# jac0626/Neighbor-Aware-Reinforcement-Learning-Fosters-Cooperation-in-Spatial-Public-Goods-Games-

Measured on AMD Instinct MI355X. Metric: agent-steps/sec (L×L×iters×replicas) + achieved HBM GB/s, L=200, higher is better.
Workload: dtype f64

## Files before the change

include/spgg_abi.h:

```cpp
#ifndef SPGG_ABI_H
#define SPGG_ABI_H

#include <stdint.h>

#ifdef __cplusplus
extern "C" {
#endif

#define SPGG_ABI_VERSION 17

#define SPGG_OK 0
#define SPGG_E_ARG (-1)
#define SPGG_E_STATE (-2)
#define SPGG_E_HIP (-3)

#define SPGG_GEN_ERR_SPIN 1u
#define SPGG_STEP_ERR_BARRIER 2u

#define SPGG_CLUSTERS_MAX_PASSES 32

#define SPGG_STATE_REPUTATION 0
#define SPGG_STATE_ACTION 1

#define SPGG_ALG_QLEARNING 0
#define SPGG_ALG_SARSA 1
#define SPGG_ALG_EXPECTED_SARSA 2
#define SPGG_ALG_DOUBLE_Q 3

#define SPGG_RNG_INJECT 0
#define SPGG_RNG_MT19937 1
#define SPGG_RNG_PHILOX 2

enum {
  SPGG_ST_NCOOP = 0,
  SPGG_ST_SUMP = 1,
  SPGG_ST_SUMP_C = 2,
  SPGG_ST_SUMP_D = 3,
  SPGG_ST_SUMR = 4,
  SPGG_ST_SW_CD = 5,
  SPGG_ST_SW_DC = 6,
  SPGG_ST_SUM_WPP = 7,
  SPGG_ST_SUM_WRR = 8,
  SPGG_ST_SUM_REW_C = 9,
  SPGG_ST_SUM_REW_D = 10,
  SPGG_ST_SUM_RATIO_C = 11,
  SPGG_ST_GC0 = 12,
  SPGG_ST_NMD_POS = 18,
  SPGG_ST_NMD_POS2 = 19,
  SPGG_ST_SUM_PCT = 20,
  SPGG_ST_SUMQ = 21,
  SPGG_ST_SUMQ_C = 25,
  SPGG_ST_SUMQ_D = 29,
  SPGG_ST_GMAX = 33,
  SPGG_NSTAT = 34
};

typedef struct spgg_ctx spgg_ctx;

typedef struct {
  int32_t device;
  int32_t n_rep;
  int32_t L;
  int32_t second_order;
  int32_t state_mode;
  int32_t rng_mode;
  int32_t iterations;
  int32_t rep_int8;
  int32_t algorithm;
  int32_t batch_reps;
} spgg_config;

typedef struct {
  double rc;
  double cost;
  double norm_min;
  double norm_den;
  double w_p;
  double w_rep;
  double alpha;
  double gamma;
  double diag_alpha;
  double diag_gamma;
  double kappa;
  double lambda_eps;
  double rep_gain_c;
  double neg_delta_r_d;
  double r_min;
  double r_max;
  uint64_t seed;
  uint64_t stream_id;
  double pay_c[6];
  double pay_d[6];
  double rep_unit;
  int32_t rk_gain, rk_loss, rk_min, rk_max;
  double norm_rcp;
} spgg_rep_params;

typedef struct {
  uint8_t* S[2];
  void* R[2];
  double* Q;
  double* pub[2];
  double* md;
  float* atd;
  uint32_t* draws;
  int64_t draw_slot_stride;
  uint32_t* mt_state;
  uint32_t* mt_snap;
  int64_t mt_snap_stride;
  double* eps;
  double* stats;
  int32_t* stop_iter;
} spgg_buffers;

int spgg_abi_version(void);
const char* spgg_build_id(void);
int spgg_draw_planes(int32_t algorithm);
const char* spgg_last_error(const spgg_ctx* ctx);

int spgg_create(spgg_ctx** out, const spgg_config* cfg);
int spgg_set_params(spgg_ctx* ctx, const spgg_rep_params* params);
int spgg_bind(spgg_ctx* ctx, const spgg_buffers* bufs);

int spgg_step(spgg_ctx* ctx, int32_t t0, int32_t n_steps, void* hip_stream);

int spgg_step_groups(spgg_ctx* const* ctxs, void* const* hip_streams, int32_t n_ctx, int32_t t0,
                     int32_t n_steps);

int spgg_flush(spgg_ctx* ctx, int32_t t_last, void* hip_stream);

int spgg_status(const spgg_ctx* ctx, uint32_t* flags);

int spgg_history_finalize(spgg_ctx* ctx, int32_t t_last, void* hip_stream);

int spgg_draw(spgg_ctx* ctx, int32_t t, void* hip_stream);
int spgg_draw_range(spgg_ctx* ctx, int32_t t0, int32_t t1, void* hip_stream);

int spgg_draw_layout(const spgg_ctx* ctx, int32_t* slots, int64_t* words_per_rep, int32_t* snap_slots);

int spgg_mt_chains(const spgg_ctx* ctx, int32_t* chains, int32_t* per_chain);

int spgg_mt_jump_poly(int64_t e, uint32_t* out624);

int spgg_stream_create(int32_t device, void** hip_stream);
int spgg_stream_destroy(void* hip_stream);

int spgg_set_draw_stream(spgg_ctx* ctx, void* hip_stream);

int spgg_payoff(spgg_ctx* ctx, int32_t t, double* out, void* hip_stream);

int spgg_clusters_max_side(const spgg_ctx* ctx, int32_t* side);
int spgg_clusters(spgg_ctx* ctx, int32_t t, int32_t periodic, int32_t* sizes, int32_t* rec,
                  int64_t rec_stride, void* hip_stream);

int spgg_pub_doubles(const spgg_ctx* ctx, int64_t* per_rep);

int spgg_stat_stripes(const spgg_ctx* ctx, int32_t* stripes);

int spgg_persistent(const spgg_ctx* ctx, int32_t* on, int32_t* capacity);

int spgg_tile_shape(const spgg_ctx* ctx, int32_t* tw, int32_t* th);

int spgg_destroy(spgg_ctx* ctx);

#ifdef __cplusplus
}
#endif
#endif
```

neighbor-aware-reinforcement-learning-fosters-cooperation-in-spatial-public-goods-games-_amd/_lib.py:

```python
from __future__ import annotations

import ctypes
import os
import threading

PKG_DIR = os.path.dirname(os.path.abspath(__file__))
LIB_PATH = os.path.join(PKG_DIR, "libspgg_hip.so")

ABI_VERSION = 17
OK, E_ARG, E_STATE, E_HIP = 0, -1, -2, -3
GEN_ERR_SPIN = 1
CLUSTERS_MAX_PASSES = 32
STATE_REPUTATION, STATE_ACTION = 0, 1
RNG_INJECT, RNG_MT19937, RNG_PHILOX = 0, 1, 2
RNG_MODES = {"inject": RNG_INJECT, "mt19937": RNG_MT19937, "philox": RNG_PHILOX}
ALG_QLEARNING, ALG_SARSA, ALG_EXPECTED_SARSA, ALG_DOUBLE_Q = 0, 1, 2, 3
ALGORITHMS = {"qlearning": ALG_QLEARNING, "sarsa": ALG_SARSA, "expected_sarsa": ALG_EXPECTED_SARSA,
              "double_qlearning": ALG_DOUBLE_Q}
DRAW_PLANES = {ALG_QLEARNING: 2, ALG_SARSA: 6, ALG_EXPECTED_SARSA: 2, ALG_DOUBLE_Q: 3}

ST_NCOOP, ST_SUMP, ST_SUMP_C, ST_SUMP_D, ST_SUMR = 0, 1, 2, 3, 4
ST_SW_CD, ST_SW_DC, ST_SUM_WPP, ST_SUM_WRR = 5, 6, 7, 8
ST_SUM_REW_C, ST_SUM_REW_D, ST_SUM_RATIO_C = 9, 10, 11
ST_GC0, ST_NMD_POS, ST_NMD_POS2, ST_SUM_PCT = 12, 18, 19, 20
ST_SUMQ, ST_SUMQ_C, ST_SUMQ_D, ST_GMAX = 21, 25, 29, 33
NSTAT = 34

EXPORTED = ("spgg_abi_version", "spgg_build_id", "spgg_last_error", "spgg_create", "spgg_set_params",
            "spgg_bind", "spgg_step", "spgg_step_groups", "spgg_flush", "spgg_draw", "spgg_payoff", "spgg_tile_shape",
            "spgg_destroy", "spgg_draw_planes", "spgg_pub_doubles", "spgg_stat_stripes",
            "spgg_history_finalize", "spgg_draw_layout", "spgg_set_draw_stream", "spgg_draw_range",
            "spgg_mt_chains", "spgg_mt_jump_poly", "spgg_stream_create", "spgg_stream_destroy",
            "spgg_status", "spgg_persistent", "spgg_clusters", "spgg_clusters_max_side")
TEST_EXPORTED = ("spgg_test_set_error",)


class Config(ctypes.Structure):
    _fields_ = [("device", ctypes.c_int32), ("n_rep", ctypes.c_int32), ("L", ctypes.c_int32),
                ("second_order", ctypes.c_int32), ("state_mode", ctypes.c_int32),
                ("rng_mode", ctypes.c_int32), ("iterations", ctypes.c_int32),
                ("rep_int8", ctypes.c_int32), ("algorithm", ctypes.c_int32),
                ("batch_reps", ctypes.c_int32)]


class RepParams(ctypes.Structure):
    _fields_ = [(name, ctypes.c_double) for name in (
        "rc", "cost", "norm_min", "norm_den", "w_p", "w_rep", "alpha", "gamma",
        "diag_alpha", "diag_gamma", "kappa", "lambda_eps", "rep_gain_c", "neg_delta_r_d",
        "r_min", "r_max")] + [("seed", ctypes.c_uint64), ("stream_id", ctypes.c_uint64),
                              ("pay_c", ctypes.c_double * 6), ("pay_d", ctypes.c_double * 6),
                              ("rep_unit", ctypes.c_double), ("rk_gain", ctypes.c_int32),
                              ("rk_loss", ctypes.c_int32), ("rk_min", ctypes.c_int32),
                              ("rk_max", ctypes.c_int32), ("norm_rcp", ctypes.c_double)]


class Buffers(ctypes.Structure):
    _fields_ = [("S", ctypes.c_void_p * 2), ("R", ctypes.c_void_p * 2), ("Q", ctypes.c_void_p),
                ("pub", ctypes.c_void_p * 2), ("md", ctypes.c_void_p), ("atd", ctypes.c_void_p),
                ("draws", ctypes.c_void_p), ("draw_slot_stride", ctypes.c_int64),
                ("mt_state", ctypes.c_void_p), ("mt_snap", ctypes.c_void_p), ("mt_snap_stride", ctypes.c_int64),
                ("eps", ctypes.c_void_p),
                ("stats", ctypes.c_void_p), ("stop_iter", ctypes.c_void_p)]


class SpggError(RuntimeError):
    pass


_libs = {}
_lock = threading.Lock()


def load(path: str | None = None):
    with _lock:
        p = path or os.environ.get("SPGG_LIB") or LIB_PATH
        if p in _libs:
            return _libs[p]
        if not os.path.exists(p):
            raise SpggError(f"{p} is not built; run `python -c 'import __graft_entry__ as g; g.build()'`")
        lib = ctypes.CDLL(p)
        vp, i32 = ctypes.c_void_p, ctypes.c_int32
        lib.spgg_abi_version.restype = ctypes.c_int
        lib.spgg_abi_version.argtypes = []
        lib.spgg_last_error.restype = ctypes.c_char_p
        lib.spgg_last_error.argtypes = [vp]
        lib.spgg_create.restype = ctypes.c_int
        lib.spgg_create.argtypes = [ctypes.POINTER(vp), ctypes.POINTER(Config)]
        lib.spgg_set_params.restype = ctypes.c_int
        lib.spgg_set_params.argtypes = [vp, ctypes.POINTER(RepParams)]
        lib.spgg_bind.restype = ctypes.c_int
        lib.spgg_bind.argtypes = [vp, ctypes.POINTER(Buffers)]
        lib.spgg_step.restype = ctypes.c_int
        lib.spgg_step.argtypes = [vp, i32, i32, vp]
        lib.spgg_step_groups.restype = ctypes.c_int
        lib.spgg_step_groups.argtypes = [ctypes.POINTER(vp), ctypes.POINTER(vp), i32, i32, i32]
        lib.spgg_flush.restype = ctypes.c_int
        lib.spgg_flush.argtypes = [vp, i32, vp]
        lib.spgg_history_finalize.restype = ctypes.c_int
        lib.spgg_history_finalize.argtypes = [vp, i32, vp]
        lib.spgg_draw.restype = ctypes.c_int
        lib.spgg_draw.argtypes = [vp, i32, vp]
        lib.spgg_draw_range.restype = ctypes.c_int
        lib.spgg_draw_range.argtypes = [vp, i32, i32, vp]
        lib.spgg_payoff.restype = ctypes.c_int
        lib.spgg_payoff.argtypes = [vp, i32, vp, vp]
        lib.spgg_tile_shape.restype = ctypes.c_int
        lib.spgg_tile_shape.argtypes = [vp, ctypes.POINTER(i32), ctypes.POINTER(i32)]
        lib.spgg_clusters.restype = ctypes.c_int
        lib.spgg_clusters.argtypes = [vp, i32, i32, vp, vp, ctypes.c_int64, vp]
        lib.spgg_clusters_max_side.restype = ctypes.c_int
        lib.spgg_clusters_max_side.argtypes = [vp, ctypes.POINTER(i32)]
        lib.spgg_persistent.restype = ctypes.c_int
        lib.spgg_persistent.argtypes = [vp, ctypes.POINTER(i32), ctypes.POINTER(i32)]
        lib.spgg_destroy.restype = ctypes.c_int
        lib.spgg_destroy.argtypes = [vp]
        lib.spgg_draw_planes.restype = ctypes.c_int
        lib.spgg_draw_planes.argtypes = [i32]
        lib.spgg_stat_stripes.restype = ctypes.c_int
        lib.spgg_stat_stripes.argtypes = [vp, ctypes.POINTER(ctypes.c_int32)]
        lib.spgg_pub_doubles.restype = ctypes.c_int
        lib.spgg_pub_doubles.argtypes = [vp, ctypes.POINTER(ctypes.c_int64)]
        lib.spgg_draw_layout.restype = ctypes.c_int
        lib.spgg_draw_layout.argtypes = [vp, ctypes.POINTER(i32), ctypes.POINTER(ctypes.c_int64), ctypes.POINTER(i32)]
        lib.spgg_mt_chains.restype = ctypes.c_int
        lib.spgg_mt_chains.argtypes = [vp, ctypes.POINTER(i32), ctypes.POINTER(i32)]
        lib.spgg_mt_jump_poly.restype = ctypes.c_int
        lib.spgg_mt_jump_poly.argtypes = [ctypes.c_int64, vp]
        lib.spgg_stream_create.restype = ctypes.c_int
        lib.spgg_stream_create.argtypes = [i32, ctypes.POINTER(vp)]
        lib.spgg_stream_destroy.restype = ctypes.c_int
        lib.spgg_stream_destroy.argtypes = [vp]
        lib.spgg_set_draw_stream.restype = ctypes.c_int
        lib.spgg_set_draw_stream.argtypes = [vp, vp]
        lib.spgg_status.restype = ctypes.c_int
        lib.spgg_status.argtypes = [vp, ctypes.POINTER(ctypes.c_uint32)]
        lib.spgg_test_set_error.restype = ctypes.c_int
        lib.spgg_test_set_error.argtypes = [vp, ctypes.c_uint32]
        lib.spgg_build_id.restype = ctypes.c_char_p
        lib.spgg_build_id.argtypes = []
        v = lib.spgg_abi_version()
        if v != ABI_VERSION:
            raise SpggError(f"libspgg_hip ABI {v} != expected {ABI_VERSION}")
        if p == LIB_PATH:
            from . import build as B
            if os.path.exists(B.SRC[0]):
                want, have = B.build_id(), lib.spgg_build_id().decode()
                if want != have:
                    raise SpggError(f"{p} was built from other sources (build id {have}, sources {want}); "
                                    "rebuild: python -c 'import __graft_entry__ as g; g.build()'")
        _libs[p] = lib
        return lib


def check(rc: int, ctx=None, what: str = "", lib=None):
    if rc != OK:
        lib = lib or load()
        detail = (lib.spgg_last_error(ctx) or b"").decode()
        raise SpggError(f"{what} failed (rc={rc}): {detail}")
```

neighbor-aware-reinforcement-learning-fosters-cooperation-in-spatial-public-goods-games-_amd/csrc/spgg_kernels.hip:

```cpp
#include <hip/hip_runtime.h>

#include <algorithm>
#include <numeric>
#include <type_traits>
#include <cstdio>
#include <cstdlib>
#include <cstring>
#include <new>
#include <string>
#include <thread>
#include <vector>

#include "spgg_abi.h"
#include "spgg_test.h"
#include "spgg_device.h"
#include "spgg_mt.h"
#include "spgg_clusters.h"

using namespace spgg;

#ifndef SPGG_ABLATE
#define SPGG_ABLATE 0
#endif
#ifndef SPGG_PRIO
#define SPGG_PRIO 0
#endif
#ifndef SPGG_QNT
#define SPGG_QNT 0
#endif
#ifndef SPGG_QSTORE
#define SPGG_QSTORE 0
#endif

#ifndef SPGG_TU
#define SPGG_TU (-1)
#endif
#define SPGG_TU_HAS_ALG(k) (SPGG_TU == -1 || SPGG_TU == (k))
#define SPGG_TU_HAS_HOST (SPGG_TU == -1 || SPGG_TU == 9)

namespace spgg_impl {

struct TileArgs {
  const uint8_t* S_in;
  uint8_t* S_out;
  const void* R_in;
  void* R_out;
  double* Q;
  double* md;
  const double* pub_in;
  double* pub_out;
  float* atd;
  const uint32_t* draws;
  int draw_words;
  int planes;
  const double* eps;
  double* stats;
  int* stop_iter;
  const spgg_rep_params* params;
  const int2* ring;
  int L, n, TW, TH, tiles_x, tiles_per_rep, n_rep, slots;
  int PB;
  int ring_max;
  int stripes;
  int rep_stride;
};

struct LaunchCfg {
  int m2, as, rq, rng, twc, total_tiles;
  int apt;
  size_t lds_bytes;
};

struct PersistArgs {
  uint8_t* S[2];
  void* R[2];
  double* pub[2];
  const uint32_t* draws0;
  long long draw_stride;
  int draw_slots;
  int t_end;
  uint32_t* bar;
  int shards;
  uint32_t base;
  uint32_t* err;
  uint32_t* err_host;
};
constexpr int kBarWords = 16;

template <int ALG>
void launch_alg(const LaunchCfg& lc, const TileArgs& a, int t, int fin, hipStream_t s,
                const PersistArgs* pa = nullptr);
template <int ALG>
int persist_blocks_per_cu(const LaunchCfg& lc);

constexpr int apt_of(int alg) { return (alg == SPGG_ALG_DOUBLE_Q ? 512 : 1024) / kBlock; }
constexpr int js_of(bool m2) { return kBlock == 256 ? (m2 ? 8 : 7) : 4; }
constexpr int jr_of() { return kBlock == 256 ? 6 : 3; }
constexpr int ring_per_thread(bool m2) { return kBlock == 256 && m2 ? 2 : 1; }
constexpr int qw_of(int alg) { return alg == SPGG_ALG_DOUBLE_Q ? 8 : 4; }
constexpr int pf_of(int alg) { return alg == SPGG_ALG_DOUBLE_Q ? 5 : 3; }

__host__ __device__ inline int pub_slots(int TW, int TH, int HA) {
  return 2 * HA * TW + (TH > 2 * HA ? (TH - 2 * HA) * 2 * HA : 0);
}
__host__ __device__ inline bool is_border(int r, int c, int th, int tw, int HA) {
  return r < HA || r >= th - HA || c < HA || c >= tw - HA;
}
__host__ __device__ inline int border_slot(int r, int c, int th, int tw, int HA) {
  if (r < HA) return r * tw + c;
  if (r >= th - HA) return (r - th + 2 * HA) * tw + c;
  const int cc = c < HA ? c : c - tw + 2 * HA;
  return 2 * HA * tw + (r - HA) * 2 * HA + cc;
}
__host__ __device__ inline int border_slot_or_none(int r, int c, int th, int tw, int HA) {
  const bool top = r < HA, bot = r >= th - HA;
  const bool left = c < HA, right = c >= tw - HA;
  const int band = (top ? r : r - th + 2 * HA) * tw + c;
  const int side = 2 * HA * tw + (r - HA) * 2 * HA + (left ? c : c - tw + 2 * HA);
  return (top || bot) ? band : ((left || right) ? side : -1);
}

__host__ __device__ inline void ring_cell(int k, int th, int tw, int HA, int* ay, int* ax) {
  const int aw = tw + 2 * HA, band = HA * aw;
  if (k < band) {
    *ay = k / aw;
    *ax = k - *ay * aw;
  } else if (k < 2 * band) {
    const int k2 = k - band;
    *ay = HA + th + k2 / aw;
    *ax = k2 - (k2 / aw) * aw;
  } else {
    const int k3 = k - 2 * band;
    *ay = HA + k3 / (2 * HA);
    const int cc = k3 - (k3 / (2 * HA)) * (2 * HA);
    *ax = cc < HA ? cc : tw + cc;
  }
}

}

using spgg_impl::TileArgs;

namespace {


struct LdsLayout {
  int sw, sh, aw, ah;
  int off_Rew, off_R, off_Rn, off_S, off_D, off_A, off_PC, off_DR, off_DP, bytes;
};

constexpr int kDrawSlots = 6;

constexpr int kPcPitch = 64;

__host__ __device__ inline LdsLayout lds_layout(int tw, int th, int HS, int HA, int rsz, bool dword_rows = false,
                                                bool draws = false) {
  LdsLayout l;
  l.sw = tw + 2 * HS; l.sh = th + 2 * HS;
  l.aw = tw + 2 * HA; l.ah = th + 2 * HA;
  if (dword_rows) l.sw = l.aw = (tw + 2 * HS + 3 + 3) / 4 * 4;
  const int na = l.aw * l.ah;
  int off = (12 + kWaves * 64) * 8;
  l.off_Rew = off;  off += ((na * 8 + 15) / 16) * 16;
  l.off_R = off;    off += ((na * rsz + 15) / 16) * 16;
  l.off_Rn = off;   off += ((na * rsz + 15) / 16) * 16;
  l.off_S = off;    off += ((l.sw * l.sh + 15) / 16) * 16;
  l.off_D = off;    off += ((l.sw * l.sh + kPcPitch + 15) / 16) * 16;
  l.off_A = off;    off += ((na + 15) / 16) * 16;
  l.off_PC = off;   off += (l.ah + 2) * kPcPitch;
  off = (off + 15) / 16 * 16;
  l.off_DR = off;   off += draws ? l.ah * kDrawSlots * 2 * 4 : 0;
  l.off_DP = off;   off += draws ? l.ah * 2 * 2 * 4 : 0;
  l.bytes = off;
  return l;
}

template <typename T>
__device__ __forceinline__ T* at(T* base, uint32_t i) {
  using B = typename std::conditional<std::is_const<T>::value, const char, char>::type;
  return reinterpret_cast<T*>(reinterpret_cast<B*>(base) + (size_t)(i * (uint32_t)sizeof(T)));
}

#ifndef SPGG_PERSIST_PLAIN
#define SPGG_PERSIST_PLAIN 0
#endif
#ifndef SPGG_PERSIST_STAGGER
#define SPGG_PERSIST_STAGGER 0
#endif
#ifndef SPGG_PERSIST_NORECOMP
#define SPGG_PERSIST_NORECOMP 0
#endif
template <bool SC1, typename T>
__device__ __forceinline__ T hload(const T* p) {
  if constexpr (SC1 && !SPGG_PERSIST_PLAIN) return __hip_atomic_load(const_cast<T*>(p), __ATOMIC_RELAXED, __HIP_MEMORY_SCOPE_AGENT);
  else return *p;
}
template <bool SC1, typename T>
__device__ __forceinline__ void hstore(T* p, T v) {
  if constexpr (SC1 && !SPGG_PERSIST_PLAIN) __hip_atomic_store(p, v, __ATOMIC_RELAXED, __HIP_MEMORY_SCOPE_AGENT);
  else *p = v;
}

template <bool RQ>
using RStore = typename std::conditional<RQ, int8_t, double>::type;
template <bool RQ>
using RVal = typename std::conditional<RQ, int, double>::type;

template <bool RQ, typename PT>
__device__ __forceinline__ RVal<RQ> rep_next(RVal<RQ> r, int act, const PT& p) {
  if constexpr (RQ) {
    const int k = r + (act == 0 ? p.rk_gain : -p.rk_loss);
    return min(max(k, p.rk_min), p.rk_max);
  } else {
    const double x = r + (act == 0 ? p.rep_gain_c : p.neg_delta_r_d);
    return fmin(fmax(x, p.r_min), p.r_max);
  }
}

template <bool M2>
__device__ __forceinline__ int rep_state_lds(const int8_t* R, int c, int w) {
  int acc = R[c] + R[c - w] + R[c + w] + R[c - 1] + R[c + 1];
  if constexpr (M2)
    acc += R[c - 2 * w] + R[c + 2 * w] + R[c - 2] + R[c + 2] + R[c - w - 1] + R[c - w + 1] + R[c + w - 1] +
           R[c + w + 1];
  return acc > 0 ? 1 : 0;
}

template <bool M2>
__device__ __forceinline__ int rep_state_lds(const double* R, int c, int w) {
  double acc = 0.0;
  acc += R[c];
  acc += R[c - w];
  acc += R[c + w];
  acc += R[c - 1];
  acc += R[c + 1];
  if constexpr (M2) {
    acc += R[c - 2 * w];
    acc += R[c + 2 * w];
    acc += R[c - 2];
    acc += R[c + 2];
    acc += R[c - w - 1];
    acc += R[c - w + 1];
    acc += R[c + w - 1];
    acc += R[c + w + 1];
  }
  return acc >= rep_threshold(M2) ? 1 : 0;
}

__device__ __forceinline__ double pending_nu(uint8_t b, double md, double kappa, double lam_den, double lam_rcp) {
  const double lam = div_uniform(kappa * md, lam_den, lam_rcp);
  return ((b >> 2) & 1) ? lam : -lam;
}

__device__ __forceinline__ int pending_entry(uint8_t b) { return ((b >> 1) & 1) * 2 + (b & 1); }

template <int K, typename T>
__device__ __forceinline__ void wave_partials(T (&v)[K], double* red, int base, int tid) {
  transpose_level<K, 32, K, T>(v, tid & 63);
  const int lane = tid & 63, wave = tid >> 6;
  constexpr int per = 64 / K;
  if ((lane & (per - 1)) == 0) red[wave * 64 + base + lane / per] = (double)v[0];
}

__device__ __forceinline__ int wrap1(int x, int L, bool tiny) {
  if (tiny) return wrap(x, L);
  x += x < 0 ? L : 0;
  x -= x >= L ? L : 0;
  return x;
}

template <typename T>
using StageReg = typename std::conditional<(sizeof(T) < 4), int, T>::type;

template <int J, typename T>
__device__ __forceinline__ void stage_region(T* dst, int pitch, const T* src, int h, int w, int y0, int x0,
                                             int L, bool tiny, uint8_t* dbit = nullptr) {
  const int total = h * w;
  const int tid = threadIdx.x;
  const int dr = kBlock / w, dc = kBlock - (kBlock / w) * w;
  int r = tid / w, c = tid - (tid / w) * w;
  StageReg<T> buf[J];
  int di[J];
#pragma unroll
  for (int j = 0; j < J; ++j) {
// ... 149 lines not shown
#define T_AT(t, o) (*reinterpret_cast<const double*>((t) + (o)))
__device__ __forceinline__ double payoff_pc(const uint8_t* pc, int ry, int rx, const double* tb, double norm_min,
                                            double norm_den, double norm_rcp) {
  const uint8_t* p = pc + ry * kPcPitch + rx + 1;
  const char* t = reinterpret_cast<const char*>(tb);
  const uint32_t x0 = p[kPcPitch], x1 = p[0], x2 = p[2 * kPcPitch], x3 = p[kPcPitch - 1], x4 = p[kPcPitch + 1];
  double tot = T_AT(t, x0);
  tot = tot + T_AT(t, x1);
  tot = tot + T_AT(t, x2);
  tot = tot + T_AT(t, x3);
  tot = tot + T_AT(t, x4);
  return div_uniform(tot - norm_min, norm_den, norm_rcp);
}

#undef T_AT

__device__ __forceinline__ double rcp_diag(double x) {
  double r = __builtin_amdgcn_rcp(x);
  r = __builtin_fma(r, __builtin_fma(-x, r, 1.0), r);
  r = __builtin_fma(r, __builtin_fma(-x, r, 1.0), r);
  return r;
}

constexpr uint64_t stat_bytes(int a, int b, int c, int d, int e, int f, int g, int h) {
  return (uint64_t)(uint8_t)a | (uint64_t)(uint8_t)b << 8 | (uint64_t)(uint8_t)c << 16 | (uint64_t)(uint8_t)d << 24 |
         (uint64_t)(uint8_t)e << 32 | (uint64_t)(uint8_t)f << 40 | (uint64_t)(uint8_t)g << 48 |
         (uint64_t)(uint8_t)h << 56;
}


enum { ALG_Q = SPGG_ALG_QLEARNING, ALG_SARSA = SPGG_ALG_SARSA, ALG_ES = SPGG_ALG_EXPECTED_SARSA,
       ALG_DQ = SPGG_ALG_DOUBLE_Q };

__device__ __forceinline__ int greedy2(double v0, double v1) { return v0 >= v1 ? 0 : 1; }

__device__ __forceinline__ double mean2(double x, double y) { return (x + y) * 0.5; }

__device__ __forceinline__ double expected_q(double v0, double v1, double eps) {
  const double po = eps * 0.5;
  const double pgr = (1.0 - eps) + po;
  const int g = greedy2(v0, v1);
  return (g == 0 ? pgr : po) * v0 + (g == 1 ? pgr : po) * v1;
}

__device__ __forceinline__ int draw_bit(const TileArgs& a, int rep, int g, int p) {
  const uint32_t w = *at(a.draws, (uint32_t)(rep * a.draw_words + (g >> 5) * a.planes + p));
  return (int)((w >> (g & 31)) & 1u);
}

template <int RNG>
__device__ __forceinline__ void draw_pair(const TileArgs& a, int rep, int g, int t, uint32_t key, uint64_t thr,
                                          int k, int* ex, int* rbt) {
  if constexpr (RNG == SPGG_RNG_PHILOX) {
#if SPGG_ABLATE & 1
    *ex = ((g * 2654435761u + t + k) >> 7) % 50 == 0; *rbt = (g ^ t ^ k) & 1;
#else
    philox_draw(g, t + (k << 26), key, thr, ex, rbt);
#endif
  } else {
    *ex = draw_bit(a, rep, g, 2 * k);
    *rbt = draw_bit(a, rep, g, 2 * k + 1);
  }
}

__device__ __forceinline__ void staged_draw(const uint2* sDP, int ry, int rx, int* ex, int* rbt) {
  const uint2 w = sDP[ry * 2 + (rx >> 5)];
  *ex = (int)((w.x >> (rx & 31)) & 1u);
  *rbt = (int)((w.y >> (rx & 31)) & 1u);
}

template <int RNG>
__device__ __forceinline__ int draw_table1(const TileArgs& a, int rep, int g, int t, uint32_t key) {
  if constexpr (RNG == SPGG_RNG_PHILOX) {
    int ex, rbt;
    philox_draw(g, t + (1 << 26), key, 1ull << 52, &ex, &rbt);
    return ex;
  } else {
    return draw_bit(a, rep, g, 2);
  }
}

typedef double vd2 __attribute__((ext_vector_type(2)));

template <int QB>
__device__ __forceinline__ void load_q(const double* Qr, uint32_t n, uint32_t agent, double (&q)[4],
                                       double (&qb)[QB ? 4 : 1]) {
  const vd2* q0 = at(reinterpret_cast<const vd2*>(Qr), agent * (QB ? 2 : 1));
  const vd2* q1 = at(reinterpret_cast<const vd2*>(Qr), (n + agent) * (QB ? 2 : 1));
#if SPGG_QNT & 1
  const vd2 q01 = __builtin_nontemporal_load(q0), q23 = __builtin_nontemporal_load(q1);
#else
  const vd2 q01 = q0[0], q23 = (SPGG_ABLATE & 4096) ? q01 : q1[0];
#endif
  q[0] = q01.x; q[1] = q01.y; q[2] = q23.x; q[3] = q23.y;
  if constexpr (QB) {
    const vd2 b01 = q0[1], b23 = q1[1];
    qb[0] = b01.x; qb[1] = b01.y; qb[2] = b23.x; qb[3] = b23.y;
  }
}

template <int QB>
__device__ __forceinline__ void store_q(double* Qr, uint32_t n, uint32_t agent, const double (&q)[4],
                                        const double (&qb)[QB ? 4 : 1], uint32_t rows = 3u) {
  vd2* q0 = at(reinterpret_cast<vd2*>(Qr), agent * (QB ? 2 : 1));
  vd2* q1 = at(reinterpret_cast<vd2*>(Qr), (n + agent) * (QB ? 2 : 1));
#if SPGG_QNT & 2
  if constexpr (!QB) {
    if (rows & 1u) __builtin_nontemporal_store(vd2{q[0], q[1]}, q0);
    if (rows & 2u) __builtin_nontemporal_store(vd2{q[2], q[3]}, q1);
    return;
  }
#endif
  if (rows & 1u) {
    q0[0] = vd2{q[0], q[1]};
    if constexpr (QB) q0[1] = vd2{qb[0], qb[1]};
  }
  if (rows & 2u) {
    q1[0] = vd2{q[2], q[3]};
    if constexpr (QB) q1[1] = vd2{qb[2], qb[3]};
  }
}

template <int QB>
__device__ __forceinline__ void select_row(const double (&q)[4], const double (&qb)[QB ? 4 : 1], int s,
                                           double* v0, double* v1) {
  if constexpr (QB) {
    const double m00 = mean2(q[0], qb[0]), m01 = mean2(q[1], qb[1]);
    const double m10 = mean2(q[2], qb[2]), m11 = mean2(q[3], qb[3]);
    *v0 = s ? m10 : m00;
    *v1 = s ? m11 : m01;
  } else {
    uint32_t a0, a1, b0, b1;
    asm("v_cmp_ne_u32_e32 vcc, 0, %4\n\t"
        "v_cndmask_b32_e32 %0, %5, %6, vcc\n\t"
        "v_cndmask_b32_e32 %1, %7, %8, vcc\n\t"
        "v_cndmask_b32_e32 %2, %9, %10, vcc\n\t"
        "v_cndmask_b32_e32 %3, %11, %12, vcc"
        : "=&v"(a0), "=&v"(a1), "=&v"(b0), "=&v"(b1)
        : "v"(s), "v"(__double2loint(q[0])), "v"(__double2loint(q[2])), "v"(__double2hiint(q[0])),
          "v"(__double2hiint(q[2])), "v"(__double2loint(q[1])), "v"(__double2loint(q[3])),
          "v"(__double2hiint(q[1])), "v"(__double2hiint(q[3]))
        : "vcc");
    *v0 = __hiloint2double((int)a1, (int)a0);
    *v1 = __hiloint2double((int)b1, (int)b0);
  }
}

template <typename PT>
__device__ __forceinline__ float diag_td_dq(const double (&q)[4], const double (&qb)[4], int e, int sn, double rew,
                                            const PT& pg) {
  const double m00 = mean2(q[0], qb[0]), m01 = mean2(q[1], qb[1]);
  const double m10 = mean2(q[2], qb[2]), m11 = mean2(q[3], qb[3]);
  const double m0 = sn ? m10 : m00, m1 = sn ? m11 : m01;
  const double td2 = (rew + pg.diag_gamma * max_f64(m0, m1)) - mean2(q_get(q, e), q_get(qb, e));
  return (float)fabs(pg.diag_alpha * td2);
}

template <int ALG, int RNG, typename PT>
__device__ __forceinline__ float td_update(const TileArgs& a, const PT& pg, int rep, int g, int t,
                                           uint32_t key, double eps, uint64_t eps53, bool diag, double rew,
                                           int so, int act, int sn, double (&q)[4],
                                           double (&qb)[ALG == ALG_DQ ? 4 : 1], double* rn0, double* rn1) {
  const double alpha = pg.alpha, gamma = pg.gamma, dgamma = pg.diag_gamma;
  const int e = so * 2 + act;
  if constexpr (ALG == ALG_DQ) {
    double x[4] = {q[0], q[1], q[2], q[3]}, y[4] = {qb[0], qb[1], qb[2], qb[3]};
    const int up1 = draw_table1<RNG>(a, rep, g, t, key);
    const double qc1 = q_get(x, e), qc2 = q_get(y, e);
    const double y0 = y[0], y1 = y[1], y2 = y[2], y3 = y[3];
// ... 98 lines not shown
  return v;
}

#ifndef SPGG_BAR_DEBUG
#define SPGG_BAR_DEBUG 0
#endif
constexpr uint32_t kBarrierPolls = 1u << 21;

__device__ __forceinline__ bool replica_barrier(const spgg_impl::PersistArgs& pa, int rep, int tile,
                                                int tiles_per_rep, uint32_t k,
                                                unsigned long long* arrive_stamp = nullptr) {
  __shared__ int bar_ok;
  asm volatile("s_waitcnt vmcnt(0)" ::: "memory");
  __syncthreads();
  if (arrive_stamp && threadIdx.x == 0) *arrive_stamp = __builtin_amdgcn_s_memrealtime();
  if (threadIdx.x < 64) {
    const int lane = threadIdx.x, S = pa.shards;
    uint32_t* ctr = pa.bar + (size_t)rep * S * spgg_impl::kBarWords;
    if (lane == 0)
      __hip_atomic_fetch_add(ctr + (tile % S) * spgg_impl::kBarWords, 1u, __ATOMIC_RELAXED,
                             __HIP_MEMORY_SCOPE_AGENT);
    const int j = lane < S ? lane : 0;
    const uint32_t want = (uint32_t)((tiles_per_rep - j + S - 1) / S) * (pa.base + k);
    bool ok = false;
    for (uint32_t poll = 0; poll < kBarrierPolls; ++poll) {
      const uint32_t have = __hip_atomic_load(ctr + j * spgg_impl::kBarWords, __ATOMIC_RELAXED,
                                              __HIP_MEMORY_SCOPE_AGENT);
      const uint32_t err = __hip_atomic_load(pa.err, __ATOMIC_RELAXED, __HIP_MEMORY_SCOPE_AGENT);
      if (__builtin_amdgcn_readfirstlane(err) != 0) break;
      if (__all((int32_t)(have - want) >= 0)) {
        ok = true;
        break;
      }
      __builtin_amdgcn_s_sleep(2);
    }
    if (!ok && lane == 0) {
      atomicOr(pa.err, (uint32_t)SPGG_STEP_ERR_BARRIER);
      __hip_atomic_fetch_or(pa.err_host, (uint32_t)SPGG_STEP_ERR_BARRIER, __ATOMIC_RELAXED, __HIP_MEMORY_SCOPE_SYSTEM);
    }
#if SPGG_BAR_DEBUG
    if (!ok) {
      const uint32_t have = __hip_atomic_load(ctr + j * spgg_impl::kBarWords, __ATOMIC_RELAXED, __HIP_MEMORY_SCOPE_AGENT);
      if ((int32_t)(have - want) < 0)
        printf("spgg barrier: rep %d tile %d k %u shard %d have %u want %u base %u\n", rep, tile, k, j, have, want,
               pa.base);
    }
#endif
    if (lane == 0) bar_ok = ok ? 1 : 0;
  }
  __syncthreads();
  return bar_ok != 0;
}

#ifndef SPGG_STAMPS
#define SPGG_STAMPS 0
#endif
#if SPGG_STAMPS
#ifndef SPGG_STAMP_T
#define SPGG_STAMP_T 30
#endif
constexpr int kStampWG = 8192, kStampSlots = 12;
__device__ unsigned long long spgg_stamps[kStampWG * kStampSlots];
#define STAMP(k)                                                                            \
  do {                                                                                      \
    if (t == SPGG_STAMP_T && tid == 0 && stamp_id < kStampWG)                               \
      spgg_stamps[stamp_id * kStampSlots + (k)] = __builtin_amdgcn_s_memrealtime();         \
  } while (0)
#else
#define STAMP(k) \
  do {           \
  } while (0)
#endif
constexpr int min_waves(bool m2, int rng, int twc, int alg) {
#ifdef SPGG_MIN_WAVES
  return SPGG_MIN_WAVES;
#else
#ifdef SPGG_MT_MIN_WAVES
  if (!m2 && rng == SPGG_RNG_MT19937 && twc > 0 && alg != SPGG_ALG_DOUBLE_Q) return SPGG_MT_MIN_WAVES;
#endif
  return (!m2 && rng == SPGG_RNG_PHILOX && twc > 0 && alg != SPGG_ALG_DOUBLE_Q) ? 4 : 1;
#endif
}

template <bool M2, bool AS, bool RQ, int RNG, int APT, int TWC, int ALG, bool PERSIST>
__device__ __forceinline__ void step_impl(const TileArgs& a0, const int t0, const int fin_only,
                                          const spgg_impl::PersistArgs& pa) {
  static_assert(!PERSIST || TWC > 0, "persistent launches use the compile-time-width kernels");
  using RT = RStore<RQ>;
  constexpr int HA = M2 ? 2 : 1;
  constexpr int HS = HA + 2;
  constexpr int QB = ALG == ALG_DQ ? 1 : 0;
  constexpr int QW = QB ? 8 : 4;
  constexpr int PF = spgg_impl::pf_of(ALG);
  constexpr bool RECOMP = ALG != ALG_SARSA && APT == spgg_impl::apt_of(ALG) && !(PERSIST && SPGG_PERSIST_NORECOMP);
  constexpr bool CARRY = PERSIST && !SPGG_PERSIST_NORECOMP;
  extern __shared__ __attribute__((aligned(16))) unsigned char smem[];

  const int total = a0.n_rep * a0.tiles_per_rep;
  const int per_xcd = (total + 7) / 8;
  const int logical = (blockIdx.x & 7) * per_xcd + (blockIdx.x >> 3);
  if (logical >= total) return;
  if (SPGG_ABLATE & 64) return;
  const int lrep = logical / a0.tiles_per_rep;
  const int tile = logical - lrep * a0.tiles_per_rep;
  const int rep = a0.rep_stride > 1 ? (int)(((uint32_t)lrep * (uint32_t)a0.rep_stride) % (uint32_t)a0.n_rep) : lrep;
#if SPGG_STAMPS
  const int stamp_id = (int)a0.params[rep].stream_id * a0.tiles_per_rep + tile;
#endif

  const int L = a0.L, n = a0.n;
  const bool tiny = TWC ? false : L < 8;
  const int tyi = tile / a0.tiles_x, txi = tile - (tile / a0.tiles_x) * a0.tiles_x;
  const int y0 = tyi * a0.TH, x0 = txi * a0.TW;
  const int th = min(a0.TH, L - y0), tw = TWC ? TWC : min(a0.TW, L - x0);
  constexpr bool DSTAGE = RNG != SPGG_RNG_PHILOX && TWC > 0;
  const LdsLayout ly = TWC ? lds_layout(TWC, a0.TH, HS, HA, (int)sizeof(RT), true, DSTAGE)
                           : lds_layout(tw, th, HS, HA, (int)sizeof(RT));
  double* tab = reinterpret_cast<double*>(smem);
  double* red = tab + 12;
  double* sRew = reinterpret_cast<double*>(smem + ly.off_Rew);
  RT* sR = reinterpret_cast<RT*>(smem + ly.off_R);
  RT* sRn = reinterpret_cast<RT*>(smem + ly.off_Rn);
  uint8_t* sS = smem + ly.off_S;
  uint8_t* sD = smem + ly.off_D;
  uint8_t* sA = smem + ly.off_A;
  uint8_t* sPC = smem + ly.off_PC;
  uint8_t* sPP = smem + ly.bytes;
  uint32_t* sDR = reinterpret_cast<uint32_t*>(smem + ly.off_DR);
  uint2* sDP = reinterpret_cast<uint2*>(smem + ly.off_DP);
  const size_t rb = (size_t)rep * n;
  double* Qr = a0.Q + rb * QW;
  double* mdr = a0.md + rb;
  float* atdr = a0.atd + rb;
  const int aw = tw + 2 * HA, ah = th + 2 * HA;

  int rc[APT];
  unsigned vbits = 0;
  double q[APT][4];
  double qb[APT][QB ? 4 : 1];
  double md_own[APT];
  float atd_own[APT];
  const int n_own = th * tw;
  const uint32_t g00 = (uint32_t)(y0 * L + x0);
  auto agent_of = [&](int rcu) { return g00 + __umul24((uint32_t)(rcu >> 16), (uint32_t)L) + ((rcu >> 8) & 0xff); };
  bool stored = false;
  int t = t0;
  for (;; ++t) {
  TileArgs a = a0;
  if constexpr (PERSIST) {
    const int cur = (t - 1) & 1, nxt = t & 1;
    a.S_in = pa.S[cur];
    a.S_out = pa.S[nxt];
    a.R_in = pa.R[cur];
    a.R_out = pa.R[nxt];
    a.pub_in = pa.pub[cur];
    a.pub_out = pa.pub[nxt];
    if (pa.draws0) a.draws = pa.draws0 + (size_t)((t - 1) % pa.draw_slots) * pa.draw_stride;
  }
  const bool first = !PERSIST || t == t0;
  int tid = threadIdx.x;
  if constexpr (PERSIST) asm volatile("" : "+v"(tid));
  const uint8_t* Sin = a.S_in + rb;
  uint8_t* Sout = a.S_out + rb;
  const RT* Rin = reinterpret_cast<const RT*>(a.R_in) + rb;
  RT* Rout = reinterpret_cast<RT*>(a.R_out) + rb;
  const bool pending = t > 1;
  STAMP(0);
#if SPGG_PRIO
  if constexpr (!PERSIST) __builtin_amdgcn_s_setprio(SPGG_PRIO);
#endif
#if SPGG_STAMPS
  if (t == SPGG_STAMP_T && tid == 0 && stamp_id < kStampWG) {
    unsigned hw, xcc;
    asm volatile("s_getreg_b32 %0, hwreg(HW_REG_HW_ID)" : "=s"(hw));
    asm volatile("s_getreg_b32 %0, hwreg(HW_REG_XCC_ID)" : "=s"(xcc));
    spgg_stamps[stamp_id * kStampSlots + 8] = hw;
    spgg_stamps[stamp_id * kStampSlots + 9] = xcc;
  }
#endif

  if (!first) {
#pragma unroll
    for (int u = 0; u < APT; ++u) rc[u] &= ~0xff;
  } else {
    const int dr = kBlock / tw, dc = kBlock - (kBlock / tw) * tw;
    int r = tid / tw, c = tid - (tid / tw) * tw;
#pragma unroll
    for (int u = 0; u < APT; ++u) {
      const int k = tid + u * kBlock;
      const bool own = k < n_own;
      rc[u] = own ? (r << 16) | (c << 8) : (TWC ? (tid & 1) << 8 : 0);
      vbits |= own ? 1u << u : 0u;
      const uint32_t g = own ? g00 + __umul24((uint32_t)r, (uint32_t)L) + (uint32_t)c : g00 + (TWC ? (tid & 1) : 0);
      if (SPGG_ABLATE & 512) {
#pragma unroll
        for (int k = 0; k < 4; ++k) q[u][k] = (double)((g + k) & 15) * 1e-3;
        if constexpr (QB) for (int k = 0; k < 4; ++k) qb[u][QB ? k : 0] = q[u][k];
        md_own[u] = 0.0;
        atd_own[u] = 0.f;
      } else {
        load_q<QB>(Qr, (uint32_t)n, g, q[u], qb[u]);
      }
      r += dr;
      c += dc;
      if (c >= tw) {
        c -= tw;
        ++r;
      }
    }
  }
  constexpr int RP = spgg_impl::ring_per_thread(M2);
  const int ring = aw * ah - n_own;
  int2 re[RP];
  {
    const int2* rtab = a.ring + (size_t)tile * a.ring_max;
#pragma unroll
    for (int j = 0; j < RP; ++j) re[j] = *at(rtab, (uint32_t)min(tid + j * kBlock, ring - 1));
  }
  constexpr int JRR = (25 + 2 * HA + kWaves - 1) / kWaves;
  constexpr int JSF = spgg_impl::js_of(M2), JRF = spgg_impl::jr_of();
  constexpr int DWS = (TWC + 2 * HS + 3 + 3) / 4, DWR = (TWC + 2 * HA + 3 + 3) / 4;
  constexpr int JSD = (25 + 2 * HS + kBlock / DWS - 1) / (kBlock / DWS);
  constexpr int JRD = (25 + 2 * HA + kBlock / DWR - 1) / (kBlock / DWR);
  const int soffS = TWC ? ((x0 - HS) & 3) : 0, soffR = TWC && RQ ? ((x0 - HA) & 3) : 0;
  uint8_t* sSv = sS + soffS;
  uint8_t* sDv = sD + soffS;
  RT* sRv = sR + soffR;
  DwordWindow<JSD, DWS> winS;
  DwordWindow<JRD, DWR> winRd;
  RowWindow<JRR, TWC + 2 * HA, RT> winR;
  if constexpr (TWC > 0) {
    winS.template load<PERSIST>(Sin, th + 2 * HS, y0 - HS, (x0 - HS) & ~3, L, tid);
    if constexpr (!AS) {
      if constexpr (RQ) winRd.template load<PERSIST>(Rin, ah, y0 - HA, (x0 - HA) & ~3, L, tid);
      else winR.template load<PERSIST>(Rin, ah, y0 - HA, x0 - HA, L, tid);
    }
  }

  if (!(SPGG_ABLATE & 512) && !RECOMP && (first || !CARRY)) {
    const bool ni_rec = __builtin_amdgcn_readfirstlane((int)(a.params[rep].kappa != 0.0)) != 0;
#pragma unroll
    for (int u = 0; u < APT; ++u) {
      const uint32_t g = ni_rec ? agent_of(rc[u]) : 0u;
      md_own[u] = (SPGG_ABLATE & 8192) ? 0.0 : *at(mdr, g);
      atd_own[u] = (SPGG_ABLATE & 256) ? 0.f : *at(atdr, g);
    }
  }
  const uint32_t xA = wrap_once(x0 - HA, L);
  const int a_len = min(aw, L - (int)xA);
  uint32_t dw0 = 0, dw1 = 0;
  if constexpr (DSTAGE) {
    const int i = min(tid, ah * kDrawSlots - 1), ry = i / kDrawSlots, sl = i - ry * kDrawSlots;
    const uint32_t gy = wrap_once(y0 - HA + ry, L);
    const uint32_t grp = min((gy * (uint32_t)L + (sl < 3 ? xA : 0u)) / 32u + (uint32_t)(sl % 3),
                             (uint32_t)(a.draw_words / a.planes - 1));
    const uint32_t wi = (uint32_t)rep * a.draw_words + grp * a.planes;
    dw0 = *at(a.draws, wi);
    dw1 = *at(a.draws, wi + 1);
  }
  const int st = first ? a.stop_iter[rep] : 0;
  const bool dead = st != 0 && st < t;
  const spgg_rep_params& pg = a.params[rep];
  __shared__ spgg_rep_params hps;
  static_assert(sizeof(spgg_rep_params) % 8 == 0, "spgg_rep_params: whole 8-byte words");
  constexpr int kParamWords = (int)(sizeof(spgg_rep_params) / 8);
  constexpr int kPayWord = (int)(offsetof(spgg_rep_params, pay_c) / 8);
  const uint64_t pword = *at(reinterpret_cast<const uint64_t*>(&pg),
                             (uint32_t)(tid < kParamWords ? tid
                                        : tid < kParamWords + 6 ? kPayWord + 5 - (tid - kParamWords)
                                        : kPayWord + 17 - min(tid - kParamWords, 11)));
  const spgg_rep_params& hp = hps;
  const double kappa = pg.kappa, w_p = pg.w_p, w_rep = pg.w_rep;
  const size_t stripe_len = (size_t)a.slots * SPGG_NSTAT;
  const double* rrow = a.stats + (size_t)rep * a.stripes * stripe_len;
  double* srow = a.stats + ((size_t)rep * a.stripes + tile % a.stripes) * stripe_len;
  bool stop_now = false;
  double gmax_prev = 0.0;
  if constexpr (PERSIST) {
    const int lane = tid & 63, k = lane < a.stripes ? lane : 0;
    const double ncv = hload<true>(rrow + k * stripe_len + (size_t)t * SPGG_NSTAT + SPGG_ST_NCOOP);
    const double gmv = pending ? hload<true>(rrow + k * stripe_len + (size_t)(t - 1) * SPGG_NSTAT + SPGG_ST_GMAX) : 0.0;
    const double nc = uniform_f64(wave_sum(lane < a.stripes ? ncv : 0.0));
    stop_now = (nc == 0.0) || (nc == (double)n);
    gmax_prev = uniform_f64(max_f64(wave_max(gmv), 0.0));
  } else {
    if (!fin_only) {
      double nc = 0.0;
      for (int k = 0; k < a.stripes; ++k) nc += rrow[k * stripe_len + (size_t)t * SPGG_NSTAT + SPGG_ST_NCOOP];
      stop_now = (nc == 0.0) || (nc == (double)n);
    }
    if (pending)
      for (int k = 0; k < a.stripes; ++k)
        gmax_prev = fmax(gmax_prev, rrow[k * stripe_len + (size_t)(t - 1) * SPGG_NSTAT + SPGG_ST_GMAX]);
  }
  const bool acting = !fin_only && !stop_now;
  const double lam_den = uniform_f64(pending ? gmax_prev + pg.lambda_eps : 1.0);
  const double lam_rcp = uniform_f64(1.0 / lam_den);
  const double eps_t = a.eps[(size_t)rep * a.slots + t];
  const double eps_prev = ALG == ALG_ES && pending ? a.eps[(size_t)rep * a.slots + t - 1] : 0.0;
  const uint64_t eps53 = uniform_u64(u53_threshold(eps_t));
  const uint32_t pkey = (uint32_t)pg.seed ^ (uint32_t)(pg.seed >> 32) * 0x85EBCA6Bu ^
                        (uint32_t)pg.stream_id * 0xC2B2AE35u;

  if (tid < kParamWords) reinterpret_cast<uint64_t*>(&hps)[tid] = pword;
  else if (tid < kParamWords + 12) reinterpret_cast<uint64_t*>(tab)[tid - kParamWords] = pword;
  if constexpr (TWC > 0) {
    winS.store(sS, ly.sw, th + 2 * HS, sD, tid);
    if constexpr (!AS) {
      if constexpr (RQ) winRd.store(reinterpret_cast<uint8_t*>(sR), ly.aw, ah, nullptr, tid);
      else winR.template store<(TWC + 2 * HS + 6) / 4 * 4>(sR, ah, nullptr, tid);
    }
  } else {
    stage_region<JSF>(sS, ly.sw, Sin, th + 2 * HS, tw + 2 * HS, y0 - HS, x0 - HS, L, tiny, sD);
    if (!AS) stage_region<JRF>(sR, ly.aw, Rin, ah, aw, y0 - HA, x0 - HA, L, tiny);
  }
  if constexpr (DSTAGE) {
    if (tid < ah * kDrawSlots) {
      sDR[tid * 2] = dw0;
      sDR[tid * 2 + 1] = dw1;
    }
  }
  if (dead) return;
  if (stop_now && tile == 0 && tid == 0) a.stop_iter[rep] = t;
  double rv[RP][PF];
  {
    const double* pin = a.pub_in + (size_t)rep * a.tiles_per_rep * PF * a.PB;
#pragma unroll
    for (int j = 0; j < RP; ++j)
#pragma unroll
      for (int f = 0; f < PF; ++f) rv[j][f] = hload<PERSIST>(at(pin, (uint32_t)(re[j].y + f * a.PB)));
  }
  __syncthreads();
  STAMP(1);
#if SPGG_PRIO
  if constexpr (!PERSIST) __builtin_amdgcn_s_setprio(0);
#endif
  if (SPGG_ABLATE & 128) {
#pragma unroll
    for (int u = 0; u < APT; ++u) {
      const int r = rc[u] >> 16, c = (rc[u] >> 8) & 0xff;
      store_q<QB>(Qr, (uint32_t)n, agent_of(rc[u]), q[u], qb[u]);
      if (!RECOMP) {
        *at(mdr, agent_of(rc[u])) = md_own[u];
        *at(atdr, agent_of(rc[u])) = atd_own[u];
      }
      *at(Sout, agent_of(rc[u])) = sSv[(r + HS) * ly.sw + (c + HS)];
      if (!AS) *at(Rout, agent_of(rc[u])) = sRv[(r + HA) * ly.aw + (c + HA)];
    }
    return;
  }
  if (!fin_only) {
    if constexpr (TWC > 0) build_plus_counts_dw<(TWC + 2 * HA + 2 + 3) / 4>(sPC, sD, ly.sw, ah + 2, soffS, tid);
    else build_plus_counts(sPC, sDv, ly.sw, ah + 2, tid);
  }
  const bool rec_prev = RECOMP && pending && kappa != 0.0;
  if (rec_prev) {
    if constexpr (TWC > 0) build_plus_counts_prev_dw<(TWC + 2 * HA + 2 + 3) / 4>(sPP, sS, ly.sw, ah + 2, soffS, tid);
    else build_plus_counts_prev(sPP, sSv, ly.sw, ah + 2, tid);
    __syncthreads();
    const int dr = kBlock / aw, dc = kBlock - (kBlock / aw) * aw;
    int ry = tid / aw, rx = tid - (tid / aw) * aw;
    for (int k = tid; k < aw * ah; k += kBlock) {
      const uint8_t b = sSv[(ry + (HS - HA)) * ly.sw + (rx + (HS - HA))];
      const double P = payoff_pc(sPP, ry, rx, tab + (((b >> 3) & 1) ? 6 : 0), hp.norm_min, hp.norm_den, hp.norm_rcp);
      const double rr = (b & 1) ? 0.0 : 0.5;
      const double wpp = w_p * P, wrr = w_rep * rr;
      sRew[ry * ly.aw + rx] = wpp + wrr;
      ry += dr;
      rx += dc;
      if (rx >= aw) {
        rx -= aw;
        ++ry;
      }
    }
    __syncthreads();
  }
  if constexpr (DSTAGE) {
    if (!fin_only && tid < ah * 2) {
      const int ry = tid >> 1, r0 = (tid & 1) * 32;
      const uint32_t gyL = wrap_once(y0 - HA + ry, L) * (uint32_t)L;
      const int offA = (int)((gyL + xA) & 31u), offB = (int)(gyL & 31u);
      const uint32_t* W = sDR + ry * kDrawSlots * 2;
      auto bits32 = [&](int slot0, int bitpos, int p) {
        const int w = bitpos >> 5;
        const uint32_t lo = W[(slot0 + min(w, 2)) * 2 + p], hi = W[(slot0 + min(w + 1, 2)) * 2 + p];
        return __builtin_amdgcn_alignbit(hi, lo, (uint32_t)(bitpos & 31));
      };
      uint32_t out[2] = {0u, 0u};
#pragma unroll
      for (int p = 0; p < 2; ++p) {
        if (r0 < a_len) out[p] = bits32(0, offA + r0, p);
        if (a_len < r0 + 32) {
          const int rs = max(r0, a_len), sh = rs - r0;
          const uint32_t mB = ~0u << sh;
          out[p] = (out[p] & ~mB) | ((bits32(3, offB + rs - a_len, p) << sh) & mB);
        }
      }
      sDP[ry * 2 + (r0 >> 5)] = make_uint2(out[0], out[1]);
    }
  }

  float pct_t1 = 0.f;
  uint32_t ni_rows = 0;
  {
    double v[8];
    float pct = 0.f;
#pragma unroll
    for (int k = 0; k < 8; ++k) v[k] = 0.0;
    uint8_t sb[APT];
#pragma unroll
    for (int u = 0; u < APT; ++u) {
      const int r = rc[u] >> 16, c = (rc[u] >> 8) & 0xff;
      sb[u] = sSv[(r + HS) * ly.sw + (c + HS)];
      rc[u] |= (AS ? 0 : ((sb[u] >> 4) & 1) << 1) | ((sb[u] & 1) << 3);
    }
    if (pending) {
#pragma unroll
      for (int u = 0; u < APT; ++u) {
        const double vmu = (vbits >> u) & 1 ? 1.0 : 0.0;
        const uint8_t b = sb[u];
        const int e = pending_entry(b);
        if (kappa != 0.0) {
          double mdp;
          float atdv;
          if constexpr (RECOMP) {
            const int r = rc[u] >> 16, c = (rc[u] >> 8) & 0xff;
            const int ca = (r + HA) * ly.aw + (c + HA);
            mdp = prev_max_diff<M2>(sRew, ca, ly.aw);
            atdv = prev_diag_td<ALG>(q[u], qb[u], e, (b >> 4) & 1, sRew[ca], hp, eps_prev);
          } else {
            mdp = md_own[u];
            atdv = atd_own[u];
          }
          const double nu = pending_nu(b, mdp, kappa, lam_den, lam_rcp);
#pragma unroll
          for (int k = 0; k < 4; ++k) {
            const double m = e == k ? 1.0 : 0.0;
            q[u][k] = __builtin_fma(m, nu, q[u][k]);
            if constexpr (QB) qb[u][k] = __builtin_fma(m, nu, qb[u][QB ? k : 0]);
          }
          ni_rows |= (1u << (e >> 1)) << (2 * u);
          const float anu = fabsf((float)nu);
          pct = (SPGG_ABLATE & 32768) ? 0.f : __builtin_fmaf(anu * __builtin_amdgcn_rcpf((atdv + anu) + 1e-8f), (float)vmu, pct);
        }
        const double cm = ((b >> 3) & 1) ? 0.0 : vmu;
#pragma unroll
        for (int e2 = 0; e2 < 4; ++e2) {
          const double qv = QB ? mean2(q[u][e2], qb[u][QB ? e2 : 0]) : q[u][e2];
          v[e2] = __builtin_fma(qv, vmu, v[e2]);
          v[4 + e2] = __builtin_fma(qv, cm, v[4 + e2]);
        }
      }
    }
    wave_partials<8>(v, red, 0, tid);
    pct_t1 = pct;
  }
  if (!acting) {
#pragma unroll
    for (int u = 0; u < APT; ++u) store_q<QB>(Qr, (uint32_t)n, agent_of(rc[u]), q[u], qb[u]);
    stored = true;
  }
  double* sRec = reinterpret_cast<double*>(smem + ly.bytes);
#pragma unroll
  for (int j = 0; j < RP; ++j) {
    const int k = tid + j * kBlock;
    if (k < ring) {
#pragma unroll
      for (int f = 0; f < PF; ++f) sRec[k * PF + f] = rv[j][f];
    }
  }
  STAMP(2);
  __syncthreads();

  uint32_t cw0 = 0, cw1 = 0;
  constexpr bool PAIRED = RNG == SPGG_RNG_PHILOX && TWC > 0 && APT % 2 == 0 && !(SPGG_ABLATE & 1);
  uint32_t pbits[APT];
  {
    double va[4] = {0.0, 0.0, 0.0, 0.0};
    RVal<RQ> rsum = 0;
#pragma unroll
    for (int u = 0; u < APT; ++u) {
      if (fin_only) continue;
      const int r = rc[u] >> 16, c = (rc[u] >> 8) & 0xff;
      const uint32_t one = (vbits >> u) & 1;
      const double vmu = one ? 1.0 : 0.0;
      const int cs = (r + HS) * ly.sw + (c + HS);
      const int ca = (r + HA) * ly.aw + (c + HA);
      const int s_t = (rc[u] >> 3) & 1;
      const double P = payoff_pc(sPC, r + HA, c + HA, tab + (s_t ? 6 : 0), hp.norm_min, hp.norm_den,
                                 hp.norm_rcp);
      const RVal<RQ> r_t = AS ? hload<PERSIST>(at(Rin, agent_of(rc[u]))) : sRv[ca];
      if constexpr (RQ) rsum += one ? r_t : 0;
      else rsum = __builtin_fma(r_t, vmu, rsum);
      if (!acting) continue;
      if constexpr (PAIRED) {
        if (u % 2 == 0) {
          const bool odd = tid & 1;
          const uint2 w = philox_block((int)agent_of(rc[odd ? u + 1 : u]), t, pkey);
          const uint32_t keep = odd ? w.y : w.x, recv = partner<1>(odd ? w.x : w.y);
          pbits[u] = odd ? recv : keep;
          pbits[u + 1] = odd ? keep : recv;
        }
      }
      int so;
      if constexpr (AS) so = s_t == 0 ? 1 : 0;
      else so = (rc[u] >> 1) & 1;
      int ex, rbt;
      if constexpr (PAIRED) philox_decide(pbits[u], eps53, &ex, &rbt);
      else if constexpr (DSTAGE) staged_draw(sDP, r + HA, c + HA, &ex, &rbt);
      else draw_pair<RNG>(a, rep, agent_of(rc[u]), t, pkey, eps53, 0, &ex, &rbt);
      double qs0, qs1;
      select_row<QB>(q[u], qb[u], so, &qs0, &qs1);
      const int act = ex ? rbt : greedy2(qs0, qs1);
      const RVal<RQ> rn = rep_next<RQ>(r_t, act, hp);
      const double rr = act == 0 ? 0.5 : 0.0;
      const double wpp = w_p * P, wrr = w_rep * rr;
      const double rew = wpp + wrr;
      sA[ca] = (uint8_t)act;
      sRn[ca] = (RT)rn;
      sRew[ca] = rew;
      rc[u] |= act | (AS ? so << 1 : 0);
      cw0 += (s_t == 0 && act == 1) ? one : 0u;
      cw1 += act == 0 ? one : 0u;
      const double am = act ? 0.0 : vmu;
      va[1] = __builtin_fma(rew, am, va[1]);
      if (w_rep != 0.0) va[2] = __builtin_fma(fabs(wrr) * rcp_diag(fabs(rew) + 1e-9), am, va[2]);
    }
    va[0] = (double)rsum;
    va[3] = (double)pct_t1;
    if (!(SPGG_ABLATE & (8 | 65536))) wave_partials<4>(va, red, 16, tid);
  }
  STAMP(3);

  if (acting && !(SPGG_ABLATE & 4)) {
#pragma unroll
    for (int j = 0; j < RP; ++j) {
      const int k = tid + j * kBlock;
      if (k >= ring) break;
      int ay, ax;
      spgg_impl::ring_cell(k, th, tw, HA, &ay, &ax);
      const int g = re[j].x;
      const int cs = (ay + (HS - HA)) * ly.sw + (ax + (HS - HA));
      const uint8_t b = sSv[cs];
      const double* rec = sRec + k * PF;
      double v0 = rec[0], v1 = rec[1], w0 = 0.0, w1 = 0.0;
      if constexpr (QB) {
        w0 = rec[QB ? 2 : 0];
        w1 = rec[QB ? 3 : 0];
      }
      if (pending && kappa != 0.0) {
        const int e = pending_entry(b);
        if ((e >> 1) == ((b >> 4) & 1)) {
          const double nu = pending_nu(b, rec[PF - 1], kappa, lam_den, lam_rcp);
          if (e & 1) v1 = v1 + nu; else v0 = v0 + nu;
          if constexpr (QB) {
            if (e & 1) w1 = w1 + nu; else w0 = w0 + nu;
          }
        }
      }
      const double P = payoff_pc(sPC, ay, ax, tab + ((b & 1) ? 6 : 0), hp.norm_min, hp.norm_den, hp.norm_rcp);
      const RVal<RQ> r_t = AS ? RVal<RQ>(0) : RVal<RQ>(sRv[ay * ly.aw + ax]);
      int ex, rbt;
      if constexpr (DSTAGE) staged_draw(sDP, ay, ax, &ex, &rbt);
      else draw_pair<RNG>(a, rep, g, t, pkey, eps53, 0, &ex, &rbt);
      const int act = ex ? rbt : (QB ? greedy2(mean2(v0, w0), mean2(v1, w1)) : greedy2(v0, v1));
      const RVal<RQ> rn = rep_next<RQ>(r_t, act, hp);
      const double rr = act == 0 ? 0.5 : 0.0;
      const int ca = ay * ly.aw + ax;
      sA[ca] = (uint8_t)act;
      sRn[ca] = (RT)rn;
      const double wpp = w_p * P, wrr = w_rep * rr;
      sRew[ca] = wpp + wrr;
    }
  }
  __syncthreads();
  STAMP(4);

  double bmax = 0.0;
  uint32_t gcn = 0, nmd2 = 0;
  if (acting) {
    double* pout = a.pub_out + (size_t)(rep * a.tiles_per_rep + tile) * PF * a.PB;
    const uint64_t bsw = *at(reinterpret_cast<const uint64_t*>(a.ring + (size_t)a.tiles_per_rep * a.ring_max),
                             (uint32_t)(((th != a.TH ? 2 : 0) + (tw != a.TW ? 1 : 0)) * kBlock + tid));
    const bool ni_on = __builtin_amdgcn_readfirstlane((int)(kappa != 0.0)) != 0;
    const bool diag_on = ni_on && !RECOMP;
#pragma unroll
    for (int u = 0; u < APT; ++u) {
      const int r = rc[u] >> 16, c = (rc[u] >> 8) & 0xff;
      const int ca = (r + HA) * ly.aw + (c + HA);
      const uint32_t one = (vbits >> u) & 1;
      const int act = rc[u] & 1, so = (rc[u] >> 1) & 1;
      const double rew = sRew[ca];
      int sn;
      if constexpr (AS) sn = act == 0 ? 1 : 0;
      else sn = rep_state_lds<M2>(sRn, ca, ly.aw);
      double rn0, rn1;
      const float atd = td_update<ALG, RNG>(a, hp, rep, agent_of(rc[u]), t, pkey, eps_t, eps53, diag_on, rew, so,
                                            act, sn, q[u], qb[u], &rn0, &rn1);
      if constexpr (CARRY) atd_own[u] = atd;
      else if (diag_on && !(SPGG_ABLATE & (256 | 2048))) *at(atdr, agent_of(rc[u])) = atd;
      if (!PERSIST && !(SPGG_ABLATE & 2048)) {
        uint32_t rows = ((ni_rows >> (2 * u)) & 3u) | (1u << so);
#if SPGG_QSTORE == 1
        rows = 3u;
#elif SPGG_QSTORE == 2
        rows |= (uint32_t)__shfl_xor((int)rows, 1);
        rows |= (uint32_t)__shfl_xor((int)rows, 2);
        rows |= (uint32_t)__shfl_xor((int)rows, 4);
#elif SPGG_QSTORE == 3
        if constexpr (TWC > 0 && TWC % 2 == 0) rows |= partner<1>(rows);
#elif SPGG_QSTORE == 4
        if constexpr (TWC > 0 && TWC % 8 == 0) {
          rows |= partner<1>(rows);
          rows |= partner<2>(rows);
          rows |= partner<4>(rows);
        }
#endif
        store_q<QB>(Qr, (uint32_t)n, agent_of(rc[u]), q[u], qb[u], rows);
      }
      const int w = ly.aw;
      constexpr int KN = M2 ? 12 : 4;
      const int nb[12] = {ca - w, ca + w, ca - 1, ca + 1,
                          ca - 2 * w, ca + 2 * w, ca - 2, ca + 2,
                          ca - w - 1, ca - w + 1, ca + w - 1, ca + w + 1};
      double rw[KN];
      int an[KN];
#pragma unroll
      for (int kk = 0; kk < KN; ++kk) {
        rw[kk] = sRew[nb[kk]];
        an[kk] = sA[nb[kk]];
      }
      double md = rw[0] - rew;
      int abest = an[0], ks = 0;
#pragma unroll
      for (int kk = 1; kk < KN; ++kk) {
        const double d = rw[kk] - rew;
        const bool better = d > md;
        md = max_f64(md, d);
        abest = better ? an[kk] : abest;
        if constexpr (M2) ks = better ? kk : ks;
      }
      const int dp = abest == act ? 1 : 0;
      const double mdp = max_f64(md, 0.0);
      bmax = max_f64(bmax, mdp);
      if constexpr (CARRY) md_own[u] = mdp;
      else if (ni_on && !RECOMP && !(SPGG_ABLATE & (2048 | 8192))) *at(mdr, agent_of(rc[u])) = mdp;
      hstore<PERSIST>(at(Sout, agent_of(rc[u])), (uint8_t)((rc[u] & 0xff) | (dp << 2) | (sn << 4)));
      hstore<PERSIST>(at(Rout, agent_of(rc[u])), (RT)sRn[ca]);
      const int bslot = (int)(int16_t)(uint16_t)(bsw >> (16 * u));
      if (bslot >= 0) {
        double* rec = pout + bslot;
        hstore<PERSIST>(rec, rn0);
        hstore<PERSIST>(rec + a.PB, rn1);
        if constexpr (QB) {
          hstore<PERSIST>(rec + 2 * a.PB, sn ? qb[u][QB ? 2 : 0] : qb[u][0]);
          hstore<PERSIST>(rec + 3 * a.PB, sn ? qb[u][QB ? 3 : 0] : qb[u][QB ? 1 : 0]);
        }
        if (ni_on) hstore<PERSIST>(rec + (PF - 1) * a.PB, mdp);
      }
      const int nd = act + an[0] + an[1] + an[2] + an[3];
      gcn += one << (4 * nd);
      if (md > 0.0) {
        cw1 += one << 16;
        if (M2 && ks >= 4) nmd2 += one;
      }
    }
  }
  STAMP(5);
  if (!(SPGG_ABLATE & (8 | 131072))) {
    uint32_t cw[8] = {cw0,
                      cw1,
                      nmd2 | ((gcn & 0xfu) << 16),
                      ((gcn >> 4) & 0xfu) | (((gcn >> 8) & 0xfu) << 16),
                      ((gcn >> 12) & 0xfu) | (((gcn >> 16) & 0xfu) << 16),
                      (gcn >> 20) & 0xfu,
                      0u,
                      0u};
    wave_partials<8>(cw, red, 24, tid);
  }
  {
    const double wm = wave_max(bmax);
    if ((tid & 63) == 0) red[(tid >> 6) * 64 + 12] = wm;
  }
  if (SPGG_ABLATE & 16) {
    if (tid == 0 && tile == 0 && acting) srow[(size_t)(t + 1) * SPGG_NSTAT] = n / 2;
    return;
  }
  __syncthreads();
  STAMP(6);

  if ((SPGG_ABLATE & (8 | 131072)) && tid == 0 && tile == 0 && acting) srow[(size_t)(t + 1) * SPGG_NSTAT] = n / 2;
  if ((SPGG_ABLATE & 16392) == 16392 && tid == 40 && acting) {
    double bm = 0.0;
#pragma unroll
    for (int w = 0; w < kWaves; ++w) bm = max_f64(bm, red[w * 64 + 12]);
    if (bm > 0.0)
      atomicMax(reinterpret_cast<unsigned long long*>(&srow[(size_t)t * SPGG_NSTAT + SPGG_ST_GMAX]),
                (unsigned long long)__double_as_longlong(bm));
  }
  if (tid < 64 && !(SPGG_ABLATE & 8)) {
    int slot = -1, k = -1, src = 12, src_c = -1;
    bool counter = false;
    if (tid < 13) {
      if (pending) {
        slot = t - 1;
        if (tid < 4) { k = SPGG_ST_SUMQ + tid; src = tid; }
        else if (tid < 8) { k = SPGG_ST_SUMQ_C + tid - 4; src = tid; }
        else if (tid == 8) { k = SPGG_ST_SUM_PCT; src = 16 + 3; }
        else { k = SPGG_ST_SUMQ_D + tid - 9; src = tid - 9; src_c = tid - 5; }
      }
    } else if (tid >= 16 && tid < 16 + 14 && !fin_only) {
      const int j = tid - 16;
      constexpr uint64_t km0 = stat_bytes(SPGG_ST_SUMR, SPGG_ST_SUM_REW_C, SPGG_ST_SUM_RATIO_C, SPGG_ST_SW_CD,
                                          -1, SPGG_ST_NCOOP, SPGG_ST_NMD_POS, SPGG_ST_NMD_POS2);
      constexpr uint64_t km1 = stat_bytes(SPGG_ST_GC0, SPGG_ST_GC0 + 1, SPGG_ST_GC0 + 2, SPGG_ST_GC0 + 3,
                                          SPGG_ST_GC0 + 4, SPGG_ST_GC0 + 5, -1, -1);
      k = (int)(int8_t)(uint8_t)((j < 8 ? km0 : km1) >> (8 * (j & 7)));
      counter = j >= 3;
      src = counter ? 24 + ((j - 3) >> 1) : 16 + j;
      const bool start_val = j == 0;
      if ((acting || start_val) && k >= 0) slot = (j == 5) ? t + 1 : t;
    }
    if ((SPGG_ABLATE & 131072) && tid >= 19 && tid <= 29) slot = -1;
    const int sc = src_c >= 0 ? src_c : src;
    double x[kWaves], y[kWaves];
#pragma unroll
    for (int w = 0; w < kWaves; ++w) {
      x[w] = red[w * 64 + src];
      y[w] = red[w * 64 + sc];
    }
    const double rep_unit = hp.rep_unit;
    if (tid == 40 && acting) {
      double bm = 0.0;
#pragma unroll
      for (int w = 0; w < kWaves; ++w) bm = max_f64(bm, x[w]);
      if (bm > 0.0)
        atomicMax(reinterpret_cast<unsigned long long*>(&srow[(size_t)t * SPGG_NSTAT + SPGG_ST_GMAX]),
                  (unsigned long long)__double_as_longlong(bm));
    }
    if (slot >= 0) {
      const int j = tid - 16;
      double tot0 = 0.0, tot1 = 0.0;
#pragma unroll
      for (int w = 0; w < kWaves; ++w) {
        tot0 += x[w];
        tot1 += y[w];
      }
      double val = src_c >= 0 ? tot0 - tot1 : tot0;
      if (counter) val = (double)(((unsigned long long)tot0 >> (16 * ((j - 3) & 1))) & 0xffffu);
      if (RQ && k == SPGG_ST_SUMR) val *= rep_unit;
      if (k == SPGG_ST_SUM_PCT || k == SPGG_ST_SUM_RATIO_C) val *= 100.0;
      if (val != 0.0 && (!(SPGG_ABLATE & 2) || k == SPGG_ST_NCOOP))
        atomicAdd(&srow[(size_t)slot * SPGG_NSTAT + k], val);
    }
  }
  STAMP(7);
  if constexpr (!PERSIST) {
    break;
  } else {
    if (!acting || t == pa.t_end) break;
    unsigned long long* arrive = nullptr;
#if SPGG_STAMPS
    if (t == SPGG_STAMP_T && stamp_id < kStampWG) arrive = &spgg_stamps[stamp_id * kStampSlots + 10];
#endif
    if (!replica_barrier(pa, rep, tile, a0.tiles_per_rep, (uint32_t)(t - t0 + 1), arrive)) {
      stored = true;
      break;
    }
    STAMP(11);
#if SPGG_PERSIST_STAGGER
    for (int z = 0; z < ((blockIdx.x >> 3) & 3) * SPGG_PERSIST_STAGGER; ++z) __builtin_amdgcn_s_sleep(16);
#endif
  }
  }
  if constexpr (PERSIST) {
    if (!stored) {
      const bool ni_rec = __builtin_amdgcn_readfirstlane((int)(a0.params[rep].kappa != 0.0)) != 0;
#pragma unroll
      for (int u = 0; u < APT; ++u) {
        store_q<QB>(Qr, (uint32_t)n, agent_of(rc[u]), q[u], qb[u]);
        if (CARRY && !RECOMP && ni_rec) {
          *at(mdr, agent_of(rc[u])) = md_own[u];
          *at(atdr, agent_of(rc[u])) = atd_own[u];
        }
      }
    }
  }
}

template <bool M2, bool AS, bool RQ, int RNG, int APT, int TWC, int ALG>
__global__ __launch_bounds__(kBlock, min_waves(M2, RNG, TWC, ALG)) void spgg_step_kernel(TileArgs a, int t,
                                                                                         int fin_only) {
  step_impl<M2, AS, RQ, RNG, APT, TWC, ALG, false>(a, t, fin_only, spgg_impl::PersistArgs{});
}

template <bool M2, bool AS, bool RQ, int RNG, int APT, int TWC, int ALG>
__global__ __launch_bounds__(kBlock, 4) void spgg_persist_kernel(TileArgs a, int t0, spgg_impl::PersistArgs pa) {
  step_impl<M2, AS, RQ, RNG, APT, TWC, ALG, true>(a, t0, 0, pa);
}

template <bool M2, bool AS, bool RQ, int ALG>
__global__ __launch_bounds__(kBlock) void spgg_publish_init_kernel(TileArgs a) {
  using RT = RStore<RQ>;
  constexpr int HA = M2 ? 2 : 1;
  constexpr int QB = ALG == ALG_DQ ? 1 : 0;
  constexpr int PF = spgg_impl::pf_of(ALG);
  const int rep = blockIdx.y;
  const int g = blockIdx.x * kBlock + threadIdx.x;
  const int L = a.L;
  const int y = g / L, x = g - (g / L) * L;
  const size_t rb = (size_t)rep * a.n;
  uint8_t* S = a.S_out;
  __shared__ int gc1[6];
  if (threadIdx.x < 6) gc1[threadIdx.x] = 0;
  __syncthreads();
  if (g < a.n) {
    const uint8_t* s = S + rb;
    const int d = (s[g] & 1) + (s[wrap(y - 1, L) * L + x] & 1) + (s[wrap(y + 1, L) * L + x] & 1) +
                  (s[y * L + wrap(x - 1, L)] & 1) + (s[y * L + wrap(x + 1, L)] & 1);
    atomicAdd(&gc1[d], 1);
  }
  __syncthreads();
  if (threadIdx.x < 6 && gc1[threadIdx.x] != 0)
    atomicAdd(&a.stats[(size_t)rep * a.stripes * a.slots * SPGG_NSTAT + SPGG_ST_GC0 + threadIdx.x],
              (double)gc1[threadIdx.x]);
  if (g >= a.n) return;
  int s1;
  if constexpr (AS) {
    s1 = (S[rb + g] & 1) ? 0 : 1;
  } else {
    const RT* R = reinterpret_cast<const RT*>(a.R_in) + rb;
    const int ym = wrap(y - 1, L), yp = wrap(y + 1, L), xm = wrap(x - 1, L), xp = wrap(x + 1, L);
    RT cell[13];
    cell[0] = R[y * L + x]; cell[1] = R[ym * L + x]; cell[2] = R[yp * L + x];
    cell[3] = R[y * L + xm]; cell[4] = R[y * L + xp];
    int nc = 5;
    if constexpr (M2) {
      const int yM = wrap(y - 2, L), yP = wrap(y + 2, L), xM = wrap(x - 2, L), xP = wrap(x + 2, L);
      cell[5] = R[yM * L + x]; cell[6] = R[yP * L + x]; cell[7] = R[y * L + xM]; cell[8] = R[y * L + xP];
      cell[9] = R[ym * L + xm]; cell[10] = R[ym * L + xp]; cell[11] = R[yp * L + xm]; cell[12] = R[yp * L + xp];
      nc = 13;
    }
    if constexpr (RQ) {
      int acc = 0;
      for (int i = 0; i < nc; ++i) acc += cell[i];
      s1 = acc > 0 ? 1 : 0;
    } else {
      double acc = 0.0;
      for (int i = 0; i < nc; ++i) acc += cell[i];
      s1 = acc >= rep_threshold(M2) ? 1 : 0;
    }
  }
  S[rb + g] = (uint8_t)((S[rb + g] & 0x0f) | (s1 << 4));
  const int ty = y / a.TH, tx = x / a.TW;
  const int r = y - ty * a.TH, c = x - tx * a.TW;
  const int th = min(a.TH, L - ty * a.TH), tw = min(a.TW, L - tx * a.TW);
  if (!spgg_impl::is_border(r, c, th, tw, HA)) return;
  constexpr int QH = QB ? 4 : 2;
  const double* Q = a.Q + rb * 2 * QH + ((size_t)s1 * a.n + g) * QH;
  double* rec = a.pub_out + (size_t)(rep * a.tiles_per_rep + ty * a.tiles_x + tx) * PF * a.PB +
                spgg_impl::border_slot(r, c, th, tw, HA);
  rec[0] = Q[0];
  rec[a.PB] = Q[1];
  if constexpr (QB) {
    rec[2 * a.PB] = Q[2];
    rec[3 * a.PB] = Q[3];
  }
  rec[(PF - 1) * a.PB] = 0.0;
}

}

namespace spgg_impl {

template <bool M2, bool AS, bool RQ, int RNG, int ALG>
const void* persist_fn_t(const LaunchCfg& lc) {
  constexpr int APT = apt_of(ALG);
  if constexpr (APT > 2) {
    if (lc.apt == 2 && lc.twc == 20)
      return reinterpret_cast<const void*>(&spgg_persist_kernel<M2, AS, RQ, RNG, 2, 20, ALG>);
  }
  if (lc.apt == APT && lc.twc == 40)
    return reinterpret_cast<const void*>(&spgg_persist_kernel<M2, AS, RQ, RNG, APT, 40, ALG>);
  return nullptr;
}

template <int ALG>
const void* persist_fn(const LaunchCfg& lc) {
  if (lc.rng == SPGG_RNG_INJECT) return nullptr;
  const bool ph = lc.rng == SPGG_RNG_PHILOX;
#define SPGG_PF(X, Y, Z)                                                                             \
  if (lc.m2 == X && lc.as == Y && lc.rq == Z)                                                        \
    return ph ? persist_fn_t<X, Y, Z, SPGG_RNG_PHILOX, ALG>(lc) : persist_fn_t<X, Y, Z, SPGG_RNG_MT19937, ALG>(lc);
  SPGG_PF(0, 0, 0) SPGG_PF(0, 0, 1) SPGG_PF(0, 1, 0) SPGG_PF(0, 1, 1)
  SPGG_PF(1, 0, 0) SPGG_PF(1, 0, 1) SPGG_PF(1, 1, 0) SPGG_PF(1, 1, 1)
#undef SPGG_PF
  return nullptr;
}

template <int ALG>
int persist_blocks_per_cu(const LaunchCfg& lc) {
  const void* f = persist_fn<ALG>(lc);
  int nb = 0;
  if (!f || hipOccupancyMaxActiveBlocksPerMultiprocessor(&nb, f, kBlock, lc.lds_bytes) != hipSuccess) return 0;
  return nb;
}

template <bool M2, bool AS, bool RQ, int RNG, int ALG>
void launch_t(const LaunchCfg& lc, const TileArgs& a, int t, int fin, hipStream_t s) {
  constexpr int APT = apt_of(ALG);
  const dim3 grid(((lc.total_tiles + 7) / 8) * 8);
  if (lc.apt == 1) {
    hipLaunchKernelGGL((spgg_step_kernel<M2, AS, RQ, RNG, 1, 0, ALG>), grid, dim3(kBlock), lc.lds_bytes, s, a, t,
                       fin);
    return;
  }
  if constexpr (APT > 2) {
    if (lc.apt == 2) {
      if (lc.twc == 20)
        hipLaunchKernelGGL((spgg_step_kernel<M2, AS, RQ, RNG, 2, 20, ALG>), grid, dim3(kBlock), lc.lds_bytes, s, a,
                           t, fin);
      else
        hipLaunchKernelGGL((spgg_step_kernel<M2, AS, RQ, RNG, 2, 0, ALG>), grid, dim3(kBlock), lc.lds_bytes, s, a,
                           t, fin);
      return;
    }
  }
#ifndef SPGG_NO_TWC
  if (lc.twc == 40)
    hipLaunchKernelGGL((spgg_step_kernel<M2, AS, RQ, RNG, APT, 40, ALG>), grid, dim3(kBlock), lc.lds_bytes, s, a,
                       t, fin);
  else
#endif
    hipLaunchKernelGGL((spgg_step_kernel<M2, AS, RQ, RNG, APT, 0, ALG>), grid, dim3(kBlock), lc.lds_bytes, s, a,
                       t, fin);
}

template <bool M2, bool AS, bool RQ, int ALG>
void launch_rng(const LaunchCfg& lc, const TileArgs& a, int t, int fin, hipStream_t s) {
  if (t == 0) {
    const dim3 grid((a.n + kBlock - 1) / kBlock, a.n_rep);
    hipLaunchKernelGGL((spgg_publish_init_kernel<M2, AS, RQ, ALG>), grid, dim3(kBlock), 0, s, a);
    return;
  }
  if (lc.rng == SPGG_RNG_PHILOX) launch_t<M2, AS, RQ, SPGG_RNG_PHILOX, ALG>(lc, a, t, fin, s);
  else launch_t<M2, AS, RQ, SPGG_RNG_MT19937, ALG>(lc, a, t, fin, s);
}

template <bool M2, bool AS, int ALG>
void launch_rq(const LaunchCfg& lc, const TileArgs& a, int t, int fin, hipStream_t s) {
  if (lc.rq) launch_rng<M2, AS, true, ALG>(lc, a, t, fin, s);
  else launch_rng<M2, AS, false, ALG>(lc, a, t, fin, s);
}

template <int ALG>
void launch_alg(const LaunchCfg& lc, const TileArgs& a, int t, int fin, hipStream_t s, const PersistArgs* pa) {
  if (pa) {
    const void* f = persist_fn<ALG>(lc);
    if (!f) return;
    TileArgs ka = a;
    int kt = t;
    PersistArgs kp = *pa;
    void* args[] = {&ka, &kt, &kp};
    (void)hipLaunchKernel(f, dim3(((lc.total_tiles + 7) / 8) * 8), dim3(kBlock), args, lc.lds_bytes, s);
    return;
  }
  if (lc.m2) {
    if (lc.as) launch_rq<true, true, ALG>(lc, a, t, fin, s);
    else launch_rq<true, false, ALG>(lc, a, t, fin, s);
  } else {
    if (lc.as) launch_rq<false, true, ALG>(lc, a, t, fin, s);
    else launch_rq<false, false, ALG>(lc, a, t, fin, s);
  }
}

#define SPGG_LAUNCH_INST(k, name)                                                                   \
  template void launch_alg<name>(const LaunchCfg&, const TileArgs&, int, int, hipStream_t, const PersistArgs*); \
  template int persist_blocks_per_cu<name>(const LaunchCfg&);
#define SPGG_LAUNCH_EXTERN(k, name)                                                                 \
  extern template void launch_alg<name>(const LaunchCfg&, const TileArgs&, int, int, hipStream_t,   \
                                        const PersistArgs*);                                        \
  extern template int persist_blocks_per_cu<name>(const LaunchCfg&);
#if SPGG_TU_HAS_ALG(0)
#if SPGG_STAMPS
}
extern "C" int spgg_stamps_read(void* dst, size_t bytes) {
  return (int)hipMemcpyFromSymbol(dst, HIP_SYMBOL(spgg_stamps), bytes < sizeof(spgg_stamps) ? bytes : sizeof(spgg_stamps));
}
namespace spgg_impl {
#endif
SPGG_LAUNCH_INST(0, SPGG_ALG_QLEARNING)
#else
SPGG_LAUNCH_EXTERN(0, SPGG_ALG_QLEARNING)
#endif
#if SPGG_TU_HAS_ALG(1)
SPGG_LAUNCH_INST(1, SPGG_ALG_SARSA)
#else
SPGG_LAUNCH_EXTERN(1, SPGG_ALG_SARSA)
#endif
#if SPGG_TU_HAS_ALG(2)
SPGG_LAUNCH_INST(2, SPGG_ALG_EXPECTED_SARSA)
#else
SPGG_LAUNCH_EXTERN(2, SPGG_ALG_EXPECTED_SARSA)
#endif
#if SPGG_TU_HAS_ALG(3)
SPGG_LAUNCH_INST(3, SPGG_ALG_DOUBLE_Q)
#else
SPGG_LAUNCH_EXTERN(3, SPGG_ALG_DOUBLE_Q)
#endif

}

#if SPGG_TU_HAS_HOST
namespace {

__device__ __forceinline__ uint32_t mt_temper(uint32_t y) {
  y ^= (y >> 11);
  y ^= (y << 7) & 0x9d2c5680u;
  y ^= (y << 15) & 0xefc60000u;
  y ^= (y >> 18);
  return y;
}

using spgg_mt::mt_next;

constexpr uint32_t kTemperBit0 = 0x20444009u;

__host__ __device__ inline int draw_planes(int alg) {
  return alg == SPGG_ALG_SARSA ? 6 : alg == SPGG_ALG_DOUBLE_Q ? 3 : 2;
}
__host__ __device__ inline int64_t draw_mt_words(int64_t n, int planes) { return n * (planes / 2 * 3 + (planes & 1) * 2); }
__host__ __device__ inline uint32_t plane_word0(uint32_t n, int p) { return n * (uint32_t)(p / 2 * 3 + (p & 1) * 2); }
__host__ __device__ inline int64_t draw_words_of(int n, int alg) {
  return (int64_t)((n + 63) / 64) * 2 * draw_planes(alg);
}

#ifndef SPGG_GEN_OUT
#define SPGG_GEN_OUT 3
#endif
constexpr int kGenOut = SPGG_GEN_OUT;
constexpr int kGenSPW = 4;
constexpr int kGenPub = 4;

constexpr int kGenU = 4;
constexpr int kGenThreads = 64 * (1 + kGenOut);
constexpr int kMtBlock = 227;
constexpr int kGenPitch = kMtBlock;
#ifndef SPGG_GEN_NB
#define SPGG_GEN_NB 16
#endif
constexpr int kGenNB = SPGG_GEN_NB;
static_assert(kGenNB == 16 || kGenNB == 8, "the block loop is unrolled kGenNB times");
static_assert(kGenNB % kGenPub == 0, "publication period divides the unrolled block loop");
static_assert(kGenU * kGenOut * 128 - 1 < (kGenNB - kGenPub) * kMtBlock + 1, "output waves' progress");
constexpr int kGenRingWords = kGenPitch * kGenNB;
constexpr int kGenRing = kGenRingWords + kGenPitch;
constexpr uint32_t kGenDoneAbort = (0xffffffffu - 624u) / kMtBlock;
constexpr uint32_t kGenSpinMax = 1u << 23;
#ifndef SPGG_GEN_SLEEP_OUT
#define SPGG_GEN_SLEEP_OUT 1
#endif
#ifndef SPGG_GEN_SLEEP_REC
#define SPGG_GEN_SLEEP_REC 2
#endif

__host__ __device__ constexpr int gen_slot_base(int s) { return s == 0 ? 0 : s == 1 ? 169 : s == 2 ? 58 : 122; }
__host__ __device__ constexpr int gen_slot_len(int s) { return s == 0 ? 58 : s == 1 ? 58 : s == 2 ? 64 : 47; }
__device__ __forceinline__ int gen_position(int s, int lane) {
  return gen_slot_base(s) + (lane < gen_slot_len(s) ? lane : lane - gen_slot_len(s));
}
// ... 176 lines not shown
      if (lane == 0) key[624] = key_pos;
    }
    return;
  }
  const int ow = wave - 1;
  const uint64_t thr_half = u53_threshold(0.5);
  const int nchunk = (g.n + 63) / 64;
  uint32_t kpos = pos0;
  uint32_t seen = 624;
  const uint32_t lane_off = (uint32_t)(((lane >> 1) * kGenOut * 2 + (lane & 1)) * planes);
  const uint64_t tail = (g.n & 63) ? (1ull << (g.n & 63)) - 1ull : ~0ull;
  for (int t = t0; t <= t1; ++t) {
    const uint64_t thr = u53_threshold(g.eps[(size_t)rep * g.eps_slots + t]);
    uint32_t* rec_out = g.draws + (size_t)((t - 1) % g.draw_slots) * g.draw_stride + (size_t)rep * g.draw_words;
    for (int p = 0; p < planes; ++p) {
      const bool dbl = (p & 1) == 0;
      const uint64_t th = (g.alg == SPGG_ALG_DOUBLE_Q && p == 2) ? thr_half : thr;
      const uint32_t th_hi = __builtin_amdgcn_readfirstlane((uint32_t)(th >> 26));
      const uint32_t th_lo = __builtin_amdgcn_readfirstlane((uint32_t)th & ((1u << 26) - 1u));
      const uint32_t base = kpos + plane_word0((uint32_t)g.n, p);
      auto chunks = [&](auto dbl_c) -> bool {
        constexpr bool dbl = decltype(dbl_c)::value;
        constexpr uint32_t wmul = dbl ? 2u : 1u;
        constexpr uint32_t cstep = 64u * wmul * kGenOut;
        static_assert(cstep * kGenU < (uint32_t)kGenRingWords, "a batch stays within one turn of the ring");
        const uint32_t wlane = wmul * (uint32_t)lane;
        uint32_t first = base + 64u * wmul * (uint32_t)ow;
        uint32_t rpos = gen_word_pos(first);
        for (int c = ow; c < nchunk; c += kGenOut * kGenU) {
          const int nb = min(kGenU, (nchunk - 1 - c) / kGenOut + 1);
          const int cl = c + (nb - 1) * kGenOut;
          const uint32_t last = first + cstep * (uint32_t)(nb - 1) + wmul * (uint32_t)min(64, g.n - 64 * cl) - 1u;
          LDS_ST(gen_need[ow][lane], first);
          if (seen <= last) {
            uint32_t spin = 0;
            for (; seen <= last && spin < kGenSpinMax; ++spin) {
              seen = 624u + kMtBlock * __builtin_amdgcn_readfirstlane(LDS_LD(gen_done[0]));
              if (seen <= last) __builtin_amdgcn_s_sleep(SPGG_GEN_SLEEP_OUT);
            }
            if (seen <= last) {
              gen_fail(g);
              LDS_ST(gen_need[ow][lane], 0xffffffffu);
              return false;
            }
          }
          GEN_FENCE();
          uint32_t rp[kGenU], x[kGenU];
#pragma unroll
          for (int u = 0; u < kGenU; ++u) {
            rp[u] = u == 0 ? rpos : rp[u - 1] + cstep;
            if (u > 0) rp[u] -= rp[u] >= (uint32_t)kGenRingWords ? (uint32_t)kGenRingWords : 0u;
            x[u] = ring[rp[u] + wlane];
          }
          uint32_t val = 0;
#pragma unroll
          for (int u = 0; u < kGenU; ++u) {
            if (u < nb) {
              bool flag;
              if (dbl) {
                const uint32_t ah = mt_temper(x[u]) >> 5;
                flag = ah < th_hi;
                if (ah == th_hi) flag = (mt_temper(ring[rp[u] + wlane + 1]) >> 6) < th_lo;
              } else {
                flag = (__builtin_popcount(x[u] & kTemperBit0) & 1) != 0;
              }
              const uint64_t bits = __builtin_amdgcn_ballot_w64(flag) & (c + u * kGenOut == nchunk - 1 ? tail : ~0ull);
              val = lane == 2 * u ? (uint32_t)bits : lane == 2 * u + 1 ? (uint32_t)(bits >> 32) : val;
            }
          }
          rpos += cstep * (uint32_t)nb;
          rpos -= rpos >= (uint32_t)kGenRingWords ? (uint32_t)kGenRingWords : 0u;
          if (lane < 2 * nb) *at(rec_out, (uint32_t)(2 * c * planes + p) + lane_off) = val;
          first += cstep * (uint32_t)nb;
        }
        return true;
      };
      if (!(dbl ? chunks(std::true_type{}) : chunks(std::false_type{}))) return;
    }
    kpos += W;
  }
  LDS_ST(gen_need[ow][lane], 0xffffffffu);
}

__global__ void spgg_set_err_kernel(uint32_t* err, uint32_t flags) {
  if (threadIdx.x == 0) atomicOr(err, flags);
}

__global__ void spgg_mt_final_kernel(GenArgs g, int t_last) {
  const int rep = blockIdx.x;
  const int st = g.stop_iter[rep];
  const int src = st ? st - 1 : t_last;
  const uint32_t* sn = g.snap + (size_t)(src % g.snap_slots) * g.snap_stride + (size_t)rep * 625;
  uint32_t* key = g.key_out + (size_t)rep * 625;
  for (int i = threadIdx.x; i < 625; i += blockDim.x) key[i] = sn[i];
}

__global__ __launch_bounds__(kBlock) void spgg_history_finalize_kernel(double* stats, const int* stop_iter,
                                                                       const spgg_rep_params* params, int n,
                                                                       int slots, int stripes, int t_last) {
  const int rep = blockIdx.y;
  const int t = blockIdx.x * kBlock + threadIdx.x + 1;
  const int st = stop_iter[rep];
  const int last = st ? st : t_last, m = st ? st - 1 : t_last;
  if (t > last || t + 1 >= slots) return;
  const size_t stripe_len = (size_t)slots * SPGG_NSTAT;
  const double* rec = stats + (size_t)rep * stripes * stripe_len;
  auto total = [&](int slot, int k) {
    double v = 0.0;
    for (int sp = 0; sp < stripes; ++sp) v += rec[sp * stripe_len + (size_t)slot * SPGG_NSTAT + k];
    return v;
  };
  const spgg_rep_params& p = params[rep];
  double praw = 0.0, praw_c = 0.0;
#pragma unroll
  for (int d = 0; d <= 5; ++d) {
    const double gc = total(t - 1, SPGG_ST_GC0 + d);
    praw_c += gc * ((5 - d) * p.pay_c[5 - d]);
    praw += gc * ((5 - d) * p.pay_c[5 - d] + d * p.pay_d[5 - d]);
  }
  const double nc = total(t, SPGG_ST_NCOOP);
  const double sump = (praw - n * p.norm_min) / p.norm_den;
  const double sump_c = (praw_c - nc * p.norm_min) / p.norm_den;
  double* out = stats + (size_t)rep * stripes * stripe_len + (size_t)t * SPGG_NSTAT;
  out[SPGG_ST_SUMP] = sump;
  out[SPGG_ST_SUMP_C] = sump_c;
  out[SPGG_ST_SUMP_D] = sump - sump_c;
  if (t <= m) {
    const double nc1 = total(t + 1, SPGG_ST_NCOOP);
    const double wpp = p.w_p * sump;
    const double wrr = nc1 * (p.w_rep * 0.5);
    out[SPGG_ST_SUM_WPP] = wpp;
    out[SPGG_ST_SUM_WRR] = wrr;
    out[SPGG_ST_SUM_REW_D] = (wpp + wrr) - total(t, SPGG_ST_SUM_REW_C);
    out[SPGG_ST_SW_DC] = total(t, SPGG_ST_SW_CD) + nc1 - nc;
  }
}

__global__ __launch_bounds__(kBlock) void spgg_payoff_kernel(const uint8_t* S, const spgg_rep_params* params,
                                                             double* out, int L, int n) {
  __shared__ double tab[12];
  const int rep = blockIdx.y;
  if (threadIdx.x < 12)
    tab[threadIdx.x] = threadIdx.x < 6 ? params[rep].pay_c[threadIdx.x] : params[rep].pay_d[threadIdx.x - 6];
  __syncthreads();
  const int idx = blockIdx.x * kBlock + threadIdx.x;
  if (idx >= n) return;
  const uint8_t* s = S + (size_t)rep * n;
  const int i = idx / L, j = idx - (idx / L) * L;
  const int im1 = wrap(i - 1, L), ip1 = wrap(i + 1, L), im2 = wrap(i - 2, L), ip2 = wrap(i + 2, L);
  const int jm1 = wrap(j - 1, L), jp1 = wrap(j + 1, L), jm2 = wrap(j - 2, L), jp2 = wrap(j + 2, L);
#define CO(r, c) ((s[(r) * L + (c)] & 1) ? 0 : 1)
  Cells13 c;
  c.c00 = CO(i, j); c.cm0 = CO(im1, j); c.cp0 = CO(ip1, j); c.c0m = CO(i, jm1); c.c0p = CO(i, jp1);
  c.cmm = CO(im1, jm1); c.cmp = CO(im1, jp1); c.cpm = CO(ip1, jm1); c.cpp = CO(ip1, jp1);
  c.cM0 = CO(im2, j); c.cP0 = CO(ip2, j); c.c0M = CO(i, jm2); c.c0P = CO(i, jp2);
#undef CO
  out[(size_t)rep * n + idx] = payoff13(c, tab, params[rep].norm_min, params[rep].norm_den, params[rep].norm_rcp);
}

}

struct spgg_ctx {
  spgg_config cfg{};
  spgg_buffers buf{};
  bool bound = false;
  bool params_set = false;
  int gen_chunk = 8, draw_slots = 16, snap_slots = 25;
  int chains = 1, per_chain = 8, jump_levels = 0;
  uint32_t* d_parts[2] = {nullptr, nullptr};
  uint32_t* d_keybuf[2] = {nullptr, nullptr};
  uint32_t* d_run_pos0 = nullptr;
  uint32_t* d_polys = nullptr;
  int64_t draw_words = 0;
  hipStream_t gen_stream = nullptr;
  bool own_gen_stream = false;
  hipEvent_t gen_done[2] = {nullptr, nullptr}, step_done[2] = {nullptr, nullptr}, gen_idle = nullptr;
  hipEvent_t caller_ready = nullptr;
  uint32_t* d_err = nullptr;
  volatile uint32_t* h_err = nullptr;
  int gen_upto = 0;
  std::vector<spgg_rep_params> params_host;
  bool params_moved = false;
  spgg_rep_params* d_params = nullptr;
  int2* d_ring = nullptr;
  int ring_max = 0;
  int n = 0;
  int TW = 0, TH = 0, tiles_x = 0, tiles_per_rep = 0, apt = 4, PB = 0;
  int stripes = 1;
  int rep_stride = 1;
  size_t lds_bytes = 0;
  bool persist = false;
  int persist_capacity = 0;
  uint32_t* d_bar = nullptr;
  uint32_t bar_base = 0;
  std::string err;
};

namespace {

int twc_of(const spgg_config& cfg, int TW, int TH) {
  if (TW == 40 && cfg.L % 40 == 0 && cfg.L >= 120 && TH <= 25) return 40;
  if (TW == 20 && cfg.L % 20 == 0 && cfg.L >= 60 && TH <= 25 && cfg.algorithm != SPGG_ALG_DOUBLE_Q) return 20;
  return 0;
}

thread_local std::string g_create_err;

int fail(spgg_ctx* c, int code, const std::string& msg) {
  if (c) c->err = msg;
  return code;
}

int create_fail(int code, const std::string& msg) {
  g_create_err = msg;
  return code;
}

int hip_check(spgg_ctx* c, hipError_t e, const char* what) {
  if (e == hipSuccess) return SPGG_OK;
  return fail(c, SPGG_E_HIP, std::string(what) + ": " + hipGetErrorString(e));
}

const char* tuning_env(const char* name) {
  const char* on = getenv("SPGG_TUNING");
  return on && !strcmp(on, "1") ? getenv(name) : nullptr;
}

constexpr long long kSmallBatchTiles = 128;
constexpr long long kTwoPerThreadTiles = 800;

constexpr double kGenRateMargin = 2.0;

void choose_mt_chains(spgg_ctx* c) {
  const spgg_config& cfg = c->cfg;
  const long long W = draw_mt_words(c->n, draw_planes(cfg.algorithm));
  int chains = 1, per = 8;
  const long long batch = cfg.batch_reps > 0 ? cfg.batch_reps : cfg.n_rep;
  if (W >= 4096) {
    const double gen_ns = W / 227.0 * 200.0;
    const double step_ns = std::max(8000.0, (double)batch * c->n * 0.015);
    const double need = kGenRateMargin * gen_ns / step_ns;
    while (chains < 256 && chains < need) chains *= 2;
    if (chains > 1)
      per = (int)std::max((1000000 + W - 1) / W, (long long)((128 + chains - 1) / chains));
    const double rec = draw_words_of(c->n, cfg.algorithm) * 4.0 * batch;
    while (chains > 1 && 2.0 * chains * per * rec > 512e6) {
      if (per > 1) per = std::max(1, per / 2);
      else chains /= 2;
    }
  }
  if (const char* e = tuning_env("SPGG_MT_CHAINS")) {
    int v = atoi(e), p2 = 1;
    while (p2 < 256 && p2 < v) p2 *= 2;
    chains = W >= 624 ? std::max(1, p2) : 1;
  }
  if (const char* e = tuning_env("SPGG_MT_PER_CHAIN")) per = std::max(1, std::min(4096, atoi(e)));
  if (chains == 1)
    if (const char* e = tuning_env("SPGG_MT_CHUNK")) per = std::max(1, std::min(256, atoi(e)));
  per = (int)std::max(1LL, std::min((long long)per, ((1LL << 31) - (1LL << 16)) / W));
  c->chains = chains;
  c->per_chain = per;
  c->gen_chunk = chains * per;
  c->jump_levels = 0;
  while ((1 << c->jump_levels) < chains) ++c->jump_levels;
  if (chains > 1) {
    const uint64_t D = (uint64_t)per * (uint64_t)W;
    const int J = c->jump_levels;
    try {
      std::thread([D, J] {
        uint32_t tmp[624];
        for (int j = 0; j <= J; ++j) spgg_mt::jump_poly((D << j) - 1, tmp);
      }).detach();
    } catch (...) {
    }
  }
}

// ... 63 lines not shown
  }
  if (rmax > spgg_impl::ring_per_thread(c->cfg.second_order != 0) * kBlock)
    return fail(c, SPGG_E_ARG, "tile ring exceeds the kernel's ring cells per thread");
  c->ring_max = rmax;
  int rc = hip_check(c, hipMalloc(&c->d_ring, tab.size() * sizeof(int2)), "hipMalloc(ring)");
  if (rc) return rc;
  return hip_check(c, hipMemcpy(c->d_ring, tab.data(), tab.size() * sizeof(int2), hipMemcpyHostToDevice),
                   "hipMemcpy(ring)");
}

TileArgs make_args(const spgg_ctx* c, int t) {
  TileArgs a{};
  if (t == 0) {
    a.S_out = c->buf.S[0];
    a.R_in = c->buf.R[0];
    a.pub_out = c->buf.pub[0];
  } else {
    const int cur = (t - 1) & 1, nxt = t & 1;
    a.S_in = c->buf.S[cur];    a.S_out = c->buf.S[nxt];
    a.R_in = c->buf.R[cur];    a.R_out = c->buf.R[nxt];
    a.pub_in = c->buf.pub[cur];  a.pub_out = c->buf.pub[nxt];
  }
  a.Q = c->buf.Q;
  a.md = c->buf.md;
  a.atd = c->buf.atd;
  a.draws = c->buf.draws ? c->buf.draws + (size_t)((t >= 1 ? t - 1 : 0) % c->draw_slots) * c->buf.draw_slot_stride
                         : nullptr;
  a.draw_words = (int)c->draw_words;
  a.planes = draw_planes(c->cfg.algorithm);
  a.eps = c->buf.eps;
  a.stats = c->buf.stats;
  a.stop_iter = c->buf.stop_iter;
  a.params = c->d_params;
  a.L = c->cfg.L;
  a.n = c->n;
  a.TW = c->TW;
  a.TH = c->TH;
  a.tiles_x = c->tiles_x;
  a.tiles_per_rep = c->tiles_per_rep;
  a.n_rep = c->cfg.n_rep;
  a.slots = c->cfg.iterations + 2;
  a.PB = c->PB;
  a.ring = c->d_ring;
  a.ring_max = c->ring_max;
  a.stripes = c->stripes;
  a.rep_stride = c->rep_stride;
  return a;
}

spgg_impl::LaunchCfg launch_cfg(const spgg_ctx* c) {
  spgg_impl::LaunchCfg lc;
  lc.m2 = c->cfg.second_order != 0;
  lc.as = c->cfg.state_mode == SPGG_STATE_ACTION;
  lc.rq = c->cfg.rep_int8 != 0;
  lc.rng = c->cfg.rng_mode;
  lc.twc = twc_of(c->cfg, c->TW, c->TH);
  lc.apt = c->apt;
  lc.total_tiles = c->cfg.n_rep * c->tiles_per_rep;
  lc.lds_bytes = c->lds_bytes;
  return lc;
}

void launch_step(const spgg_ctx* c, int t, int fin, hipStream_t s, const spgg_impl::PersistArgs* pa = nullptr) {
  const TileArgs a = make_args(c, t);
  const spgg_impl::LaunchCfg lc = launch_cfg(c);
  switch (c->cfg.algorithm) {
    case SPGG_ALG_SARSA: spgg_impl::launch_alg<SPGG_ALG_SARSA>(lc, a, t, fin, s, pa); break;
    case SPGG_ALG_EXPECTED_SARSA: spgg_impl::launch_alg<SPGG_ALG_EXPECTED_SARSA>(lc, a, t, fin, s, pa); break;
    case SPGG_ALG_DOUBLE_Q: spgg_impl::launch_alg<SPGG_ALG_DOUBLE_Q>(lc, a, t, fin, s, pa); break;
    default: spgg_impl::launch_alg<SPGG_ALG_QLEARNING>(lc, a, t, fin, s, pa); break;
  }
}

int persist_blocks(const spgg_ctx* c) {
  const spgg_impl::LaunchCfg lc = launch_cfg(c);
  switch (c->cfg.algorithm) {
    case SPGG_ALG_SARSA: return spgg_impl::persist_blocks_per_cu<SPGG_ALG_SARSA>(lc);
    case SPGG_ALG_EXPECTED_SARSA: return spgg_impl::persist_blocks_per_cu<SPGG_ALG_EXPECTED_SARSA>(lc);
    case SPGG_ALG_DOUBLE_Q: return spgg_impl::persist_blocks_per_cu<SPGG_ALG_DOUBLE_Q>(lc);
    default: return spgg_impl::persist_blocks_per_cu<SPGG_ALG_QLEARNING>(lc);
  }
}

int err_word_init(spgg_ctx* c) {
  int rc = SPGG_OK;
  if (!c->d_err) {
    rc = hip_check(c, hipMalloc(&c->d_err, 4), "hipMalloc(err)");
    if (!rc) rc = hip_check(c, hipMemset(c->d_err, 0, 4), "hipMemset(err)");
  }
  if (!rc && !c->h_err) {
    void* h = nullptr;
    rc = hip_check(c, hipHostMalloc(&h, 4, hipHostMallocMapped), "hipHostMalloc(err)");
    if (!rc) {
      c->h_err = static_cast<volatile uint32_t*>(h);
      *c->h_err = 0;
    }
  }
  return rc;
}

int persist_lazy_init(spgg_ctx* c) {
  int rc = err_word_init(c);
  if (rc || c->d_bar) return rc;
  const size_t bytes = (size_t)c->cfg.n_rep * c->stripes * spgg_impl::kBarWords * 4;
  rc = hip_check(c, hipMalloc(&c->d_bar, bytes), "hipMalloc(barrier counters)");
  if (!rc) rc = hip_check(c, hipMemset(c->d_bar, 0, bytes), "hipMemset(barrier counters)");
  return rc;
}

void launch_persist(spgg_ctx* c, int t, int t1, hipStream_t s) {
  if (t == 1) {
    (void)hipMemsetAsync(c->d_bar, 0, (size_t)c->cfg.n_rep * c->stripes * spgg_impl::kBarWords * 4, s);
    c->bar_base = 0;
  }
  spgg_impl::PersistArgs pa{};
  for (int i = 0; i < 2; ++i) {
    pa.S[i] = c->buf.S[i];
    pa.R[i] = c->buf.R[i];
    pa.pub[i] = c->buf.pub[i];
  }
  pa.draws0 = c->cfg.rng_mode == SPGG_RNG_PHILOX ? nullptr : c->buf.draws;
  pa.draw_stride = c->buf.draw_slot_stride;
  pa.draw_slots = c->draw_slots;
  pa.t_end = t1;
  pa.bar = c->d_bar;
  pa.shards = c->stripes;
  pa.base = c->bar_base;
  pa.err = c->d_err;
  void* hd = nullptr;
  pa.err_host = hipHostGetDevicePointer(&hd, (void*)c->h_err, 0) == hipSuccess ? static_cast<uint32_t*>(hd)
                                                                                 : const_cast<uint32_t*>(c->h_err);
  launch_step(c, t, 0, s, &pa);
  c->bar_base += (uint32_t)(t1 - t);
}

GenArgs gen_args(const spgg_ctx* c, int q = -1) {
  GenArgs g{};
  g.key_in = q <= 0 ? c->buf.mt_state : c->d_keybuf[q & 1];
  g.key_out = q < 0 ? c->buf.mt_state : c->d_keybuf[(q + 1) & 1];
  g.parts = q < 0 ? nullptr : c->d_parts[q & 1];
  g.run_pos0 = c->d_run_pos0;
  g.chains = q < 0 ? 1 : c->chains;
  g.per_chain = q < 0 ? c->gen_chunk : c->per_chain;
  g.snap = c->buf.mt_snap;
  g.snap_stride = c->buf.mt_snap_stride;
  g.snap_slots = c->snap_slots;
  g.draws = c->buf.draws;
  g.draw_stride = c->buf.draw_slot_stride;
  g.draw_slots = c->draw_slots;
  g.draw_words = (int)c->draw_words;
  g.eps = c->buf.eps;
  g.eps_slots = c->cfg.iterations + 2;
  g.stop_iter = c->buf.stop_iter;
  g.err = c->d_err;
  g.n = c->n;
  g.alg = c->cfg.algorithm;
  return g;
}

void launch_gen(const spgg_ctx* c, int t0, int t1, int skip_stopped, hipStream_t s, int q = -1) {
  const GenArgs g = gen_args(c, q);
  hipLaunchKernelGGL(spgg_mt_gen_kernel, dim3(c->cfg.n_rep * g.chains), dim3(kGenThreads), 0, s, g, t0, t1,
                     skip_stopped);
}

hipError_t make_stream(hipStream_t* s, bool gen) {
  const char* e = tuning_env(gen ? "SPGG_GEN_STREAM_MODE" : "SPGG_STREAM_MODE");
  const int mode = e ? atoi(e) : gen ? 0 : 2;
  if (mode == 1 || mode == 4) {
    int lo = 0, hi = 0;
    if (hipDeviceGetStreamPriorityRange(&lo, &hi) == hipSuccess)
      return hipStreamCreateWithPriority(s, hipStreamNonBlocking, mode == 1 ? hi : lo);
  } else if (mode == 2 || mode == 3) {
    int dev = 0, cus = 0;
    hipError_t r = hipGetDevice(&dev);
    if (r == hipSuccess) r = hipDeviceGetAttribute(&cus, hipDeviceAttributeMultiprocessorCount, dev);
    if (r == hipSuccess && cus > 0) {
      const char* st = tuning_env("SPGG_GEN_CU_STRIDE");
      const int stride = std::max(2, st ? atoi(st) : 8);
      std::vector<uint32_t> mask((cus + 31) / 32, 0u);
      for (int i = 0; i < cus; ++i)
        if (mode == 2 || ((i % stride == 0) == gen)) mask[i / 32] |= 1u << (i % 32);
      return hipExtStreamCreateWithCUMask(s, (uint32_t)mask.size(), mask.data());
    }
  }
  return hipStreamCreateWithFlags(s, hipStreamNonBlocking);
}

int mt_lazy_init(spgg_ctx* c) {
  if (c->gen_done[0] && c->h_err) return SPGG_OK;
  int rc = SPGG_OK;
  if (!c->gen_stream) {
    rc = hip_check(c, make_stream(&c->gen_stream, true), "hipStreamCreate(gen)");
    if (rc) return rc;
    c->own_gen_stream = true;
  }
  for (int i = 0; i < 2 && !rc; ++i) {
    rc = hip_check(c, hipEventCreateWithFlags(&c->gen_done[i], hipEventDisableTiming), "hipEventCreate");
    if (!rc) rc = hip_check(c, hipEventCreateWithFlags(&c->step_done[i], hipEventDisableTiming), "hipEventCreate");
  }
  if (!rc) rc = hip_check(c, hipEventCreateWithFlags(&c->gen_idle, hipEventDisableTiming), "hipEventCreate");
  if (!rc) rc = hip_check(c, hipEventCreateWithFlags(&c->caller_ready, hipEventDisableTiming), "hipEventCreate");
  if (!rc) rc = err_word_init(c);
  if (rc || c->chains == 1) return rc;
  const size_t R = c->cfg.n_rep, win = R * c->chains * spgg_mt::kSplits * 624;
  for (int i = 0; i < 2 && !rc; ++i) {
    rc = hip_check(c, hipMalloc(&c->d_parts[i], win * 4), "hipMalloc(mt parts)");
    if (!rc) rc = hip_check(c, hipMalloc(&c->d_keybuf[i], R * 625 * 4), "hipMalloc(mt keys)");
  }
  if (!rc) rc = hip_check(c, hipMalloc(&c->d_run_pos0, R * 4), "hipMalloc(mt pos)");
  if (!rc) rc = hip_check(c, hipMalloc(&c->d_polys, (size_t)(c->jump_levels + 1) * 624 * 4), "hipMalloc(mt polys)");
  if (rc) return rc;
  const uint64_t W = (uint64_t)draw_mt_words(c->n, draw_planes(c->cfg.algorithm));
  std::vector<uint32_t> polys((size_t)(c->jump_levels + 1) * 624);
  for (int j = 0; j <= c->jump_levels; ++j) {
    spgg_mt::jump_poly(((uint64_t)c->per_chain * W << j) - 1, polys.data() + (size_t)j * 624);
    bool nz = false;
    for (int i = 0; i < 624; ++i) nz |= polys[(size_t)j * 624 + i] != 0;
    if (!nz) return fail(c, SPGG_E_STATE, "MT19937 jump polynomial unavailable");
  }
  return hip_check(c, hipMemcpy(c->d_polys, polys.data(), polys.size() * 4, hipMemcpyHostToDevice),
                   "hipMemcpy(mt polys)");
}

void enqueue_gen_chunk(spgg_ctx* c, int q) {
  const int K = c->gen_chunk;
  const int t0 = q * K + 1, t1 = std::min((q + 1) * K, c->cfg.iterations);
  const int J = c->jump_levels, R = c->cfg.n_rep;
  if (q >= 2) (void)hipStreamWaitEvent(c->gen_stream, c->step_done[q & 1], 0);
  if (c->chains > 1 && q == 0) {
    spgg_mt::launch_seed(c->buf.mt_state, c->d_run_pos0, c->d_parts[J & 1], R, c->chains, c->gen_stream);
    for (int j = 0; j < J; ++j)
      spgg_mt::launch_jump(c->d_parts[(J - j) & 1], c->d_parts[(J - j - 1) & 1], c->d_polys + (size_t)j * 624, R,
                           c->chains, j, nullptr, c->gen_stream);
  }
  launch_gen(c, t0, t1, 1, c->gen_stream, c->chains > 1 ? q : -1);
  (void)hipEventRecord(c->gen_done[q & 1], c->gen_stream);
  (void)hipMemcpyAsync((void*)c->h_err, c->d_err, 4, hipMemcpyDeviceToHost, c->gen_stream);
  if (c->chains > 1 && t1 < c->cfg.iterations)
    spgg_mt::launch_jump(c->d_parts[q & 1], c->d_parts[(q + 1) & 1], c->d_polys + (size_t)J * 624, R, c->chains, -1,
                         c->buf.stop_iter, c->gen_stream);
  c->gen_upto = t1;
}

}

#ifndef SPGG_TIMING
#define SPGG_TIMING 0
#endif

#ifndef SPGG_BUILD_ID
#define SPGG_BUILD_ID "unversioned"
#endif

extern "C" {

int spgg_abi_version(void) { return SPGG_ABI_VERSION; }

static const char kBuildTag[] = "spgg-build:" SPGG_BUILD_ID;
const char* spgg_build_id(void) { return kBuildTag + 11; }

int spgg_draw_planes(int32_t algorithm) {
  if (algorithm < SPGG_ALG_QLEARNING || algorithm > SPGG_ALG_DOUBLE_Q) return SPGG_E_ARG;
  return draw_planes(algorithm);
}

const char* spgg_last_error(const spgg_ctx* ctx) { return ctx ? ctx->err.c_str() : g_create_err.c_str(); }

int spgg_create(spgg_ctx** out, const spgg_config* cfg) {
  if (!out || !cfg) return create_fail(SPGG_E_ARG, "spgg_create: null argument");
  *out = nullptr;
  g_create_err.clear();
  if (cfg->n_rep < 1 || cfg->L < 1 || cfg->iterations < 0 || (long long)cfg->L * cfg->L > (1LL << 30))
    return create_fail(SPGG_E_ARG, "spgg_create: n_rep >= 1, 1 <= L <= 32768, iterations >= 0 required");
  if (cfg->state_mode != SPGG_STATE_REPUTATION && cfg->state_mode != SPGG_STATE_ACTION)
    return create_fail(SPGG_E_ARG, "spgg_create: unknown state_mode");
  if (cfg->rng_mode < SPGG_RNG_INJECT || cfg->rng_mode > SPGG_RNG_PHILOX)
    return create_fail(SPGG_E_ARG, "spgg_create: unknown rng_mode");
  if (cfg->algorithm < SPGG_ALG_QLEARNING || cfg->algorithm > SPGG_ALG_DOUBLE_Q)
    return create_fail(SPGG_E_ARG, "spgg_create: unknown algorithm");
  if (cfg->iterations >= (1 << 26))
    return create_fail(SPGG_E_ARG, "spgg_create: iterations >= 2^26");
  if (cfg->batch_reps != 0 && cfg->batch_reps < cfg->n_rep)
    return create_fail(SPGG_E_ARG, "spgg_create: batch_reps < n_rep");
  if ((long long)cfg->n_rep * cfg->L * cfg->L > (1LL << 31) - 1)
    return create_fail(SPGG_E_ARG, "spgg_create: n_rep * L * L >= 2^31");
  if ((long long)cfg->L * cfg->L * spgg_impl::qw_of(cfg->algorithm) * 8 > 0xFFFFFFFFLL)
    return create_fail(SPGG_E_ARG, "spgg_create: a replica's Q table exceeds 4 GiB (32-bit offsets)");
  const int apt_max = spgg_impl::apt_of(cfg->algorithm);
  int apt = apt_max;
  {
    int tw4, th4;
    choose_tile(cfg->L, kBlock * apt_max, &tw4, &th4);
    const long long reps = cfg->batch_reps > 0 ? cfg->batch_reps : cfg->n_rep;
    const long long tiles4 = reps * ((cfg->L + tw4 - 1) / tw4) * ((cfg->L + th4 - 1) / th4);
    if (const char* e = tuning_env("SPGG_APT")) {
      if (!strcmp(e, "max") || atoi(e) == apt_max) apt = apt_max;
      else if (!strcmp(e, "1")) apt = 1;
      else if (!strcmp(e, "2")) apt = 2;
      else
        return create_fail(SPGG_E_ARG, std::string("SPGG_APT=") + e + ": expected 1, 2 or max (" +
                                           std::to_string(apt_max) + " agents per thread for this operator)");
    } else if (tiles4 < kTwoPerThreadTiles && apt_max > 2 && cfg->L % 20 == 0 && cfg->L >= 60) {
      apt = 2;
    } else if (tiles4 < kSmallBatchTiles) {
      apt = 1;
    }
  }
  spgg_ctx* c = new (std::nothrow) spgg_ctx();
  if (!c) return create_fail(SPGG_E_ARG, "spgg_create: out of host memory");
  c->cfg = *cfg;
  c->n = cfg->L * cfg->L;
  c->apt = apt;
  if (cfg->rng_mode == SPGG_RNG_MT19937) choose_mt_chains(c);
  c->draw_slots = 2 * c->gen_chunk;
  c->snap_slots = 3 * c->gen_chunk + 1;
  c->draw_words = draw_words_of(c->n, cfg->algorithm);
  choose_tile(cfg->L, kBlock * c->apt, &c->TW, &c->TH);
  if (c->apt == 2 && c->apt < spgg_impl::apt_of(cfg->algorithm) && cfg->L % 20 == 0 && cfg->L >= 60) {
    c->TW = 20;
    c->TH = 25;
  }
  if (const char* e = tuning_env("SPGG_TILE")) {
    int w = 0, h = 0;
    if (sscanf(e, "%dx%d", &w, &h) == 2 && w >= 1 && h >= 1 && w <= std::min(cfg->L, 56) &&
        h <= std::min(cfg->L, 64) && w * h <= kBlock * c->apt) {
      c->TW = w;
      c->TH = h;
    }
  }
  c->tiles_x = (cfg->L + c->TW - 1) / c->TW;
  c->tiles_per_rep = c->tiles_x * ((cfg->L + c->TH - 1) / c->TH);
  int tiles_per_stripe = kTilesPerStripe;
  if (const char* e = tuning_env("SPGG_TILES_PER_STRIPE")) tiles_per_stripe = std::max(1, atoi(e));
  while (c->stripes < 32 && (c->tiles_per_rep + c->stripes - 1) / c->stripes > tiles_per_stripe) c->stripes *= 2;
  const int HA = cfg->second_order ? 2 : 1;
  const bool twc = twc_of(*cfg, c->TW, c->TH) > 0;
  const LdsLayout ly = lds_layout(c->TW, c->TH, HA + 2, HA, cfg->rep_int8 ? 1 : 8, twc,
                                  twc && cfg->rng_mode != SPGG_RNG_PHILOX);
  c->lds_bytes = (size_t)ly.bytes;
  c->PB = spgg_impl::pub_slots(c->TW, c->TH, HA);
  const int js = spgg_impl::js_of(cfg->second_order != 0), jr = spgg_impl::jr_of();
  if (c->lds_bytes > 160 * 1024 || ly.sw * ly.sh > js * kBlock || ly.aw * ly.ah > jr * kBlock) {
    delete c;
    return create_fail(SPGG_E_ARG, "spgg_create: tile windows exceed the kernel's LDS / staging budget");
  }
  int rc = hip_check(c, hipSetDevice(cfg->device), "hipSetDevice");
  if (!rc) rc = build_ring_table(c);
  if (!rc) {
    c->lds_bytes += std::max((size_t)c->ring_max * spgg_impl::pf_of(cfg->algorithm) * sizeof(double),
                             (size_t)(ly.ah + 2) * kPcPitch);
    if (c->lds_bytes > 160 * 1024) rc = fail(c, SPGG_E_ARG, "tile LDS footprint exceeds 160 KB");
  }
  if (!rc && cfg->rng_mode != SPGG_RNG_INJECT) {
    const char* e = tuning_env("SPGG_PERSIST");
    const int nb = (e && !strcmp(e, "1")) ? persist_blocks(c) : 0;
    int cus = 0;
    if (nb > 0 && hipDeviceGetAttribute(&cus, hipDeviceAttributeMultiprocessorCount, cfg->device) == hipSuccess) {
      const long long reps = cfg->batch_reps > 0 ? cfg->batch_reps : cfg->n_rep;
      c->persist_capacity = (nb - (cfg->rng_mode == SPGG_RNG_MT19937 ? 1 : 0)) * cus;
      c->persist = reps * c->tiles_per_rep <= (long long)c->persist_capacity;
    }
  }
  if (rc) {
    g_create_err = c->err;
    spgg_destroy(c);
    return rc;
  }
  *out = c;
  return SPGG_OK;
}

static int rep_stride_for(const spgg_ctx* c, const spgg_rep_params* params) {
  const int R = c->cfg.n_rep, tiles = c->tiles_per_rep;
  if (R < 3 || tiles < 1) return 1;
  if (const char* e = tuning_env("SPGG_REP_STRIDE")) {
    const int st = atoi(e) % R;
    return st > 1 && std::gcd(st, R) == 1 ? st : 1;
  }
  const long long total = (long long)R * tiles, per = (total + 7) / 8;
  auto busiest = [&](int stride) {
    double load[8] = {0, 0, 0, 0, 0, 0, 0, 0};
    for (int j = 0; j < R; ++j) {
      const int r = (int)(((long long)j * stride) % R);
      const double w = params[r].kappa == 0.0 ? 0.82 : 1.0;
      for (long long k = (long long)j * tiles; k < (long long)(j + 1) * tiles;) {
        const int x = (int)(k / per);
        const long long k1 = std::min((long long)(j + 1) * tiles, (x + 1) * per);
        load[x] += w * (double)(k1 - k);
        k = k1;
      }
    }
    return *std::max_element(load, load + 8);
  };
  const double base = busiest(1);
  int best = 1;
  double best_load = base;
  for (int st = 2; st < R; ++st) {
    if (std::gcd(st, R) != 1) continue;
    const double l = busiest(st);
    if (l < best_load - 1e-9) { best_load = l; best = st; }
  }
  return best_load <= 0.99 * base ? best : 1;
}

int spgg_set_params(spgg_ctx* c, const spgg_rep_params* params) {
  if (!c || !params) return fail(c, SPGG_E_ARG, "null argument");
  int rc = hip_check(c, hipSetDevice(c->cfg.device), "hipSetDevice");
  if (rc) return rc;
  const size_t bytes = sizeof(spgg_rep_params) * c->cfg.n_rep;
  if (!c->d_params) {
    rc = hip_check(c, hipMalloc(&c->d_params, bytes), "hipMalloc(params)");
    if (rc) return rc;
  }
  rc = hip_check(c, hipMemcpy(c->d_params, params, bytes, hipMemcpyHostToDevice), "hipMemcpy(params)");
  if (rc) return rc;
  if (c->params_host.size() == (size_t)c->cfg.n_rep)
    c->params_moved |= memcmp(c->params_host.data(), params, bytes) != 0;
  c->params_host.assign(params, params + c->cfg.n_rep);
  c->rep_stride = rep_stride_for(c, params);
  c->params_set = true;
  return SPGG_OK;
}

int spgg_bind(spgg_ctx* c, const spgg_buffers* b) {
  if (!c || !b) return fail(c, SPGG_E_ARG, "null argument");
  for (int i = 0; i < 2; ++i)
    if (!b->S[i] || !b->R[i] || !b->pub[i])
      return fail(c, SPGG_E_ARG, "spgg_bind: an S / R / border-record buffer is null");
  if (!b->Q || !b->md || !b->atd || !b->eps || !b->stats || !b->stop_iter)
    return fail(c, SPGG_E_ARG, "spgg_bind: a required buffer is null");
  if (c->cfg.rng_mode != SPGG_RNG_PHILOX &&
      (!b->draws || b->draw_slot_stride < (int64_t)c->cfg.n_rep * c->draw_words))
    return fail(c, SPGG_E_ARG, "spgg_bind: draw records (spgg_draw_layout slots, stride >= n_rep*words) required "
                               "for INJECT/MT19937");
  if (c->cfg.rng_mode == SPGG_RNG_MT19937 &&
      (!b->mt_state || !b->mt_snap || b->mt_snap_stride < (int64_t)c->cfg.n_rep * 625))
    return fail(c, SPGG_E_ARG, "spgg_bind: mt_state and mt_snap (stride >= n_rep*625) required for MT19937");
  if ((reinterpret_cast<uintptr_t>(b->Q) & 15) != 0)
    return fail(c, SPGG_E_ARG, "spgg_bind: the Q buffer must be 16-byte aligned");
  c->buf = *b;
  c->bound = true;
  return SPGG_OK;
}

static int step_check(spgg_ctx* c, int32_t t0, int32_t n_steps) {
  if (!c) return SPGG_E_ARG;
  if (!c->bound || !c->params_set) return fail(c, SPGG_E_STATE, "spgg_step before bind/set_params");
  if (t0 < 1 || n_steps < 0 || (long long)t0 + n_steps - 1 > c->cfg.iterations)
    return fail(c, SPGG_E_ARG, "spgg_step: iteration range outside [1, iterations]");
  if (c->cfg.rng_mode == SPGG_RNG_INJECT && n_steps > 1)
    return fail(c, SPGG_E_ARG, "spgg_step: INJECT mode steps one iteration per call");
  if (t0 != 1 && c->params_moved)
    return fail(c, SPGG_E_STATE, "spgg_step: replica parameters changed mid-run (spgg_set_params after "
                                 "iteration 1: e.g. a kappa woken from 0 has no pending NI record)");
  return SPGG_OK;
}

static int step_setup(spgg_ctx* c) {
  int rc = SPGG_OK;
  if (c->cfg.rng_mode == SPGG_RNG_MT19937) rc = mt_lazy_init(c);
  if (!rc && c->persist) rc = persist_lazy_init(c);
  return rc;
}

static int step_begin(spgg_ctx* c, int32_t t0, int32_t n_steps, hipStream_t s) {
  if (t0 == 1) c->params_moved = false;
  const bool mt = c->cfg.rng_mode == SPGG_RNG_MT19937;
  int rc = step_setup(c);
  if (rc) return rc;
  if (mt && t0 == 1) c->gen_upto = 0;
  if (t0 == 1 && n_steps > 0) launch_step(c, 0, 0, s);
  if (mt && n_steps > 0 && c->gen_upto == 0) {
    (void)hipEventRecord(c->caller_ready, s);
    (void)hipStreamWaitEvent(c->gen_stream, c->caller_ready, 0);
  }
  return SPGG_OK;
}

static int seg_end(const spgg_ctx* c, int t, int end) {
  if (!c->persist) return t;
  int t1 = end - 1;
  if (c->cfg.rng_mode == SPGG_RNG_MT19937) t1 = std::min(t1, ((t - 1) / c->gen_chunk + 1) * c->gen_chunk);
  return t1;
}

static void step_seg(spgg_ctx* c, int t, int t1, int32_t t0, hipStream_t s) {
  const bool mt = c->cfg.rng_mode == SPGG_RNG_MT19937;
  const int K = c->gen_chunk, T = c->cfg.iterations;
  constexpr int timing = SPGG_TIMING;
  if (mt) {
    const int q = (t - 1) / K;
    while (timing != 2 && c->gen_upto < std::min(T, (q + 2) * K)) enqueue_gen_chunk(c, c->gen_upto / K);
    if (timing != 2 && (t == q * K + 1 || t == t0)) (void)hipStreamWaitEvent(s, c->gen_done[q & 1], 0);
  }
  if (timing != 1) {
    if (t1 > t) launch_persist(c, t, t1, s);
    else launch_step(c, t, 0, s);
  }
  if (mt && (t1 % K == 0 || t1 == T)) (void)hipEventRecord(c->step_done[((t1 - 1) / K) & 1], s);
}

int spgg_step(spgg_ctx* c, int32_t t0, int32_t n_steps, void* stream) {
  int rc = step_check(c, t0, n_steps);
  if (rc) return rc;
  hipStream_t s = reinterpret_cast<hipStream_t>(stream);
  if ((rc = step_begin(c, t0, n_steps, s))) return rc;
  const int end = t0 + n_steps;
  for (int t = t0; t < end;) {
    const int t1 = seg_end(c, t, end);
    step_seg(c, t, t1, t0, s);
    t = t1 + 1;
  }
  return hip_check(c, hipGetLastError(), "spgg_step launch");
}

int spgg_step_groups(spgg_ctx* const* ctxs, void* const* streams, int32_t n_ctx, int32_t t0, int32_t n_steps) {
  if (!ctxs || !streams || n_ctx < 1) return SPGG_E_ARG;
  for (int i = 0; i < n_ctx; ++i) {
    if (!ctxs[i]) return SPGG_E_ARG;
    for (int j = 0; j < i; ++j)
      if (ctxs[j] == ctxs[i]) return fail(ctxs[i], SPGG_E_ARG, "spgg_step_groups: a context listed twice");
    if (ctxs[i]->cfg.rng_mode == SPGG_RNG_INJECT)
      return fail(ctxs[i], SPGG_E_ARG, "spgg_step_groups: INJECT mode steps through spgg_step");
    int rc = step_check(ctxs[i], t0, n_steps);
    if (!rc) rc = step_setup(ctxs[i]);
    if (rc) {
      if (i > 0) fail(ctxs[0], rc, "spgg_step_groups: context " + std::to_string(i) + ": " + ctxs[i]->err);
      return rc;
    }
  }
  for (int i = 0; i < n_ctx; ++i) {
    int rc = step_begin(ctxs[i], t0, n_steps, reinterpret_cast<hipStream_t>(streams[i]));
    if (rc) return rc;
  }
  bool same = true;
  for (int i = 1; i < n_ctx; ++i)
    same &= ctxs[i]->persist == ctxs[0]->persist && ctxs[i]->gen_chunk == ctxs[0]->gen_chunk &&
            ctxs[i]->cfg.rng_mode == ctxs[0]->cfg.rng_mode;
  const int end = t0 + n_steps;
  for (int t = t0; t < end;) {
    int t1 = same ? seg_end(ctxs[0], t, end) : t;
    for (int i = 0; i < n_ctx; ++i)
      step_seg(ctxs[i], t, ctxs[i]->persist ? t1 : t, t0, reinterpret_cast<hipStream_t>(streams[i]));
    t = t1 + 1;
  }
  const int rc = hip_check(ctxs[0], hipGetLastError(), "spgg_step_groups launch");
  for (int i = 1; i < n_ctx && rc; ++i) ctxs[i]->err = ctxs[0]->err;
  return rc;
}

int spgg_flush(spgg_ctx* c, int32_t t_last, void* stream) {
  if (!c) return SPGG_E_ARG;
  if (!c->bound || !c->params_set) return fail(c, SPGG_E_STATE, "spgg_flush before bind/set_params");
  if (t_last < 1 || t_last > c->cfg.iterations) return fail(c, SPGG_E_ARG, "spgg_flush: bad t_last");
  if (c->params_moved)
    return fail(c, SPGG_E_STATE, "spgg_flush: replica parameters changed mid-run (e.g. a kappa woken "
                                 "from 0 has no pending NI record)");
  hipStream_t s = reinterpret_cast<hipStream_t>(stream);
  if (c->cfg.rng_mode == SPGG_RNG_MT19937 && c->gen_done[0]) {
    (void)hipMemcpyAsync((void*)c->h_err, c->d_err, 4, hipMemcpyDeviceToHost, c->gen_stream);
    (void)hipEventRecord(c->gen_idle, c->gen_stream);
    (void)hipStreamWaitEvent(s, c->gen_idle, 0);
    c->gen_upto = 0;
    int rc = hip_check(c, hipEventSynchronize(c->gen_idle), "spgg_flush: generator");
    if (rc) return rc;
    if (*c->h_err)
      return fail(c, SPGG_E_STATE, "spgg_flush: the MT19937 draw generator failed (error word " +
                                       std::to_string(*c->h_err) + "): a wait between its waves ran out of "
                                       "its bound, so this run's draws are not the reference's");
    hipLaunchKernelGGL(spgg_mt_final_kernel, dim3(c->cfg.n_rep), dim3(256), 0, s, gen_args(c), t_last);
  }
  launch_step(c, t_last + 1, 1, s);
  return hip_check(c, hipGetLastError(), "spgg_flush launch");
}

int spgg_history_finalize(spgg_ctx* c, int32_t t_last, void* stream) {
  if (!c) return SPGG_E_ARG;
  if (!c->bound || !c->params_set) return fail(c, SPGG_E_STATE, "spgg_history_finalize before bind/set_params");
  if (t_last < 0 || t_last > c->cfg.iterations) return fail(c, SPGG_E_ARG, "spgg_history_finalize: bad t_last");
  const int slots = c->cfg.iterations + 2;
  const dim3 grid((slots + kBlock - 1) / kBlock, c->cfg.n_rep);
  hipLaunchKernelGGL(spgg_history_finalize_kernel, grid, dim3(kBlock), 0, reinterpret_cast<hipStream_t>(stream),
                     c->buf.stats, c->buf.stop_iter, c->d_params, c->n, slots, c->stripes, t_last);
  return hip_check(c, hipGetLastError(), "spgg_history_finalize launch");
}

int spgg_draw(spgg_ctx* c, int32_t t, void* stream) { return spgg_draw_range(c, t, t, stream); }

int spgg_draw_range(spgg_ctx* c, int32_t t0, int32_t t1, void* stream) {
  if (!c) return SPGG_E_ARG;
  if (!c->bound || c->cfg.rng_mode != SPGG_RNG_MT19937)
    return fail(c, SPGG_E_STATE, "spgg_draw needs a bound MT19937 context");
  if (t0 < 1 || t1 < t0 || t1 > c->cfg.iterations || t1 - t0 + 1 > c->gen_chunk ||
      (long long)(t1 - t0 + 2) * draw_mt_words(c->n, draw_planes(c->cfg.algorithm)) >= (1LL << 31))
    return fail(c, SPGG_E_ARG, "spgg_draw_range: 1 <= t0 <= t1 <= iterations, t1 - t0 < gen chunk, < 2^31 words");
  const int rc = mt_lazy_init(c);
  if (rc) return rc;
  launch_gen(c, t0, t1, 0, reinterpret_cast<hipStream_t>(stream));
  return hip_check(c, hipGetLastError(), "spgg_draw launch");
}

int spgg_payoff(spgg_ctx* c, int32_t t, double* out, void* stream) {
  if (!c || !out) return fail(c, SPGG_E_ARG, "null argument");
  if (!c->bound || !c->params_set) return fail(c, SPGG_E_STATE, "spgg_payoff before bind/set_params");
  if (t < 1) return fail(c, SPGG_E_ARG, "spgg_payoff: bad t");
  const dim3 grid((c->n + kBlock - 1) / kBlock, c->cfg.n_rep);
  hipLaunchKernelGGL(spgg_payoff_kernel, grid, dim3(kBlock), 0, reinterpret_cast<hipStream_t>(stream),
                     c->buf.S[(t - 1) & 1], c->d_params, out, c->cfg.L, c->n);
  return hip_check(c, hipGetLastError(), "spgg_payoff launch");
}

int spgg_clusters_max_side(const spgg_ctx* c, int32_t* side) {
  if (!c || !side) return SPGG_E_ARG;
  *side = spgg_cl::kMaxSide;
  return SPGG_OK;
}

int spgg_clusters(spgg_ctx* c, int32_t t, int32_t periodic, int32_t* sizes, int32_t* rec, int64_t rec_stride,
                  void* stream) {
  if (!c || !rec) return fail(c, SPGG_E_ARG, "null argument");
  if (!c->bound) return fail(c, SPGG_E_STATE, "spgg_clusters before bind");
  if (t < 1) return fail(c, SPGG_E_ARG, "spgg_clusters: bad t");
  if (c->cfg.L > spgg_cl::kMaxSide)
    return fail(c, SPGG_E_ARG, "spgg_clusters: L = " + std::to_string(c->cfg.L) + " exceeds the supported side " +
                                   std::to_string(spgg_cl::kMaxSide) + " (the lattice is labelled in LDS)");
  spgg_cl::launch(c->buf.S[0], c->buf.S[1], c->buf.stop_iter, c->cfg.n_rep, c->cfg.L, t, periodic, sizes, rec,
                        rec_stride, reinterpret_cast<hipStream_t>(stream));
  return hip_check(c, hipGetLastError(), "spgg_clusters launch");
}

int spgg_status(const spgg_ctx* c, uint32_t* flags) {
  if (!c || !flags) return SPGG_E_ARG;
  *flags = c->h_err ? *c->h_err : 0u;
  return SPGG_OK;
}

int spgg_test_set_error(spgg_ctx* c, uint32_t flags) {
  if (!c) return SPGG_E_ARG;
  if (c->cfg.rng_mode != SPGG_RNG_MT19937) return fail(c, SPGG_E_STATE, "spgg_test_set_error: MT19937 only");
  int rc = hip_check(c, hipSetDevice(c->cfg.device), "hipSetDevice");
  if (!rc) rc = mt_lazy_init(c);
  if (rc) return rc;
  hipLaunchKernelGGL(spgg_set_err_kernel, dim3(1), dim3(64), 0, c->gen_stream, c->d_err, flags);
  return hip_check(c, hipGetLastError(), "spgg_test_set_error launch");
}

int spgg_pub_doubles(const spgg_ctx* c, int64_t* per_rep) {
  if (!c || !per_rep) return SPGG_E_ARG;
  *per_rep = (int64_t)c->tiles_per_rep * spgg_impl::pf_of(c->cfg.algorithm) * c->PB;
  return SPGG_OK;
}

int spgg_stat_stripes(const spgg_ctx* c, int32_t* stripes) {
  if (!c || !stripes) return SPGG_E_ARG;
  *stripes = c->stripes;
  return SPGG_OK;
}

int spgg_persistent(const spgg_ctx* c, int32_t* on, int32_t* capacity) {
  if (!c || !on || !capacity) return SPGG_E_ARG;
  *on = c->persist ? 1 : 0;
  *capacity = c->persist_capacity;
  return SPGG_OK;
}

int spgg_tile_shape(const spgg_ctx* c, int32_t* tw, int32_t* th) {
  if (!c || !tw || !th) return SPGG_E_ARG;
  *tw = c->TW;
  *th = c->TH;
  return SPGG_OK;
}

int spgg_draw_layout(const spgg_ctx* c, int32_t* slots, int64_t* words_per_rep, int32_t* snap_slots) {
  if (!c || !slots || !words_per_rep || !snap_slots) return SPGG_E_ARG;
  *slots = c->draw_slots;
  *words_per_rep = c->draw_words;
  *snap_slots = c->snap_slots;
  return SPGG_OK;
}

int spgg_mt_chains(const spgg_ctx* c, int32_t* chains, int32_t* per_chain) {
  if (!c || !chains || !per_chain) return SPGG_E_ARG;
  const bool mt = c->cfg.rng_mode == SPGG_RNG_MT19937;
  *chains = mt ? c->chains : 1;
  *per_chain = mt ? c->per_chain : 1;
  return SPGG_OK;
}

int spgg_stream_create(int32_t device, void** stream) {
  if (!stream) return SPGG_E_ARG;
  *stream = nullptr;
  if (hipSetDevice(device) != hipSuccess) return SPGG_E_HIP;
  hipStream_t s = nullptr;
  if (make_stream(&s, false) != hipSuccess) return SPGG_E_HIP;
  *stream = s;
  return SPGG_OK;
}

int spgg_stream_destroy(void* stream) {
  if (!stream) return SPGG_E_ARG;
  return hipStreamDestroy(reinterpret_cast<hipStream_t>(stream)) == hipSuccess ? SPGG_OK : SPGG_E_HIP;
}

int spgg_set_draw_stream(spgg_ctx* c, void* stream) {
  if (!c) return SPGG_E_ARG;
  if (c->cfg.rng_mode != SPGG_RNG_MT19937) return fail(c, SPGG_E_STATE, "spgg_set_draw_stream: MT19937 only");
  if (c->gen_done[0] || c->gen_stream) return fail(c, SPGG_E_STATE, "spgg_set_draw_stream: set it before spgg_step");
  c->gen_stream = reinterpret_cast<hipStream_t>(stream);
  c->own_gen_stream = false;
  return SPGG_OK;
}

int spgg_destroy(spgg_ctx* c) {
  if (!c) return SPGG_OK;
  if (c->d_params || c->d_ring || c->gen_stream || c->gen_done[0] || c->d_err || c->d_bar) {
    (void)hipSetDevice(c->cfg.device);
    if (c->gen_stream) (void)hipStreamSynchronize(c->gen_stream);
    if (c->d_params) (void)hipFree(c->d_params);
    if (c->d_ring) (void)hipFree(c->d_ring);
    for (int i = 0; i < 2; ++i) {
      if (c->gen_done[i]) (void)hipEventDestroy(c->gen_done[i]);
      if (c->step_done[i]) (void)hipEventDestroy(c->step_done[i]);
    }
    if (c->gen_idle) (void)hipEventDestroy(c->gen_idle);
    if (c->caller_ready) (void)hipEventDestroy(c->caller_ready);
    if (c->d_err) (void)hipFree(c->d_err);
    if (c->h_err) (void)hipHostFree((void*)c->h_err);
    for (int i = 0; i < 2; ++i) {
      if (c->d_parts[i]) (void)hipFree(c->d_parts[i]);
      if (c->d_keybuf[i]) (void)hipFree(c->d_keybuf[i]);
    }
    if (c->d_run_pos0) (void)hipFree(c->d_run_pos0);
    if (c->d_bar) (void)hipFree(c->d_bar);
    if (c->d_polys) (void)hipFree(c->d_polys);
    if (c->own_gen_stream) (void)hipStreamDestroy(c->gen_stream);
  }
  delete c;
  return SPGG_OK;
}

}
#endif
```

neighbor-aware-reinforcement-learning-fosters-cooperation-in-spatial-public-goods-games-_amd/engine.py:

```python
from __future__ import annotations

import atexit
import ctypes
import dataclasses
import math
import os
from typing import Callable, Optional, Sequence

import numpy as np
import torch

from . import _lib as C
from .algorithms import canonical_name

SNAPSHOT_ITERS = (1, 10, 100, 1000, 5000, 10000, 20000, 30000, 40000)


def tuning_env(name: str, default: Optional[str] = None) -> Optional[str]:
    if os.environ.get("SPGG_TUNING") != "1":
        return default
    return os.environ.get(name, default)
PNG_ITERS = set(SNAPSHOT_ITERS) | {5000}


# ... 293 lines not shown
            key = (p.epsilon, p.epsilon_decay, p.epsilon_min)
            if key not in cache:
                cache[key] = epsilon_table(*key, T + 1)
            eps[k] = cache[key]
        self.eps_host = eps
        self.eps = torch.from_numpy(eps).to(d)
        self._ncoop0 = (S0 == 0).sum(axis=1).astype(np.float64)
        self.stop_iter = torch.zeros(R, dtype=torch.int32, device=d)
        self.P_buf = torch.zeros((R, n), dtype=f64, device=d)

    def _create(self):
        cfg = C.Config(device=self.dev.index, n_rep=self.R, L=self.L, second_order=int(self.M2),
                       state_mode=C.STATE_ACTION if self.state_rep == "action" else C.STATE_REPUTATION,
                       rng_mode=C.RNG_MODES[self.rng], iterations=self.T, rep_int8=int(self.rep_int8),
                       algorithm=self.alg, batch_reps=self.R)
        params = [p.to_c() for p in self.reps]
        for k, p in enumerate(params):
            p.stream_id = self.replica_offset + k
        self.groups = []
        self._own_streams = []
        if self.G == 1:
            streams = [torch.cuda.current_stream(self.dev)]
        elif tuning_env("SPGG_OWN_STREAMS", "1") == "1":
            for _ in range(self.resident):
                self._own_streams.append(_take_stream(self.lib, self.dev.index))
            streams = [torch.cuda.ExternalStream(h, device=self.dev) for h in self._own_streams]
        else:
            streams = [torch.cuda.Stream(self.dev) for _ in range(self.resident)]
        bounds = np.linspace(0, self.R, self.G + 1).round().astype(int)
        for g in range(self.G):
            r0, r1 = int(bounds[g]), int(bounds[g + 1])
            cfg.n_rep = r1 - r0
            ctx = ctypes.c_void_p()
            C.check(self.lib.spgg_create(ctypes.byref(ctx), cfg), None, "spgg_create")
            self.groups.append(dict(r0=r0, r1=r1, ctx=ctx, stream=streams[g % len(streams)], live=True))
            arr = (C.RepParams * (r1 - r0))(*params[r0:r1])
            C.check(self.lib.spgg_set_params(ctx, arr), ctx, "spgg_set_params")
            layout = self._layout(ctx) + (self._draw_layout(ctx), self._mt_chains(ctx))
            if g == 0:
                self.layout = layout
                tile, per, self.stripes = layout[:3]
                self.pub = torch.zeros((2, self.R, max(1, per)), dtype=torch.float64, device=self.dev)
                self.stats = torch.zeros((self.R, self.stripes, self.T + 2, C.NSTAT), dtype=torch.float64,
                                         device=self.dev)
                self.stats[:, 0, 1, C.ST_NCOOP] = torch.from_numpy(self._ncoop0).to(self.dev)
                slots, words, snaps = self._draw_layout(ctx)
                self.draw_slots, self.draw_words = slots, words
                rngd = self.rng != "philox"
                self.draws = torch.zeros((slots, self.R, words) if rngd else (1, 1, 1), dtype=torch.int32,
                                         device=self.dev)
                self.mt_snap = torch.zeros((snaps, self.R, 625) if self.rng == "mt19937" else (1, 1, 1),
                                           dtype=torch.int32, device=self.dev)
            elif layout != self.layout:
                raise C.SpggError(f"replica group {g} got layout {layout} != group 0's {self.layout} "
                                  "(tile, border-record doubles, stripes, draw ring, MT chains): shared buffer "
                                  "strides would disagree")
            b = C.Buffers()
            for i in range(2):
                b.S[i], b.R[i] = self.S[i][r0].data_ptr(), self.Rep[i][r0].data_ptr()
                b.pub[i] = self.pub[i][r0].data_ptr()
            b.Q, b.md, b.atd = self.Qb[r0].data_ptr(), self.md[r0].data_ptr(), self.atd[r0].data_ptr()
            b.draws = self.draws[0, min(r0, self.draws.shape[1] - 1)].data_ptr()
            b.draw_slot_stride = self.draws.shape[1] * self.draws.shape[2]
            b.mt_state = self.mt_state[r0].data_ptr()
            b.mt_snap = self.mt_snap[0, min(r0, self.mt_snap.shape[1] - 1)].data_ptr()
            b.mt_snap_stride = self.mt_snap.shape[1] * self.mt_snap.shape[2]
            b.eps, b.stats = self.eps[r0].data_ptr(), self.stats[r0].data_ptr()
            b.stop_iter = self.stop_iter[r0].data_ptr()
            C.check(self.lib.spgg_bind(ctx, b), ctx, "spgg_bind")
            self.groups[-1]["bufs"] = b
        self.streams = streams
        self._draw_stream = None
        if self.rng == "mt19937" and self.G > 1 and tuning_env("SPGG_SHARED_DRAW_STREAM", "1") == "1":
            self._draw_stream = torch.cuda.Stream(self.dev)
            for gr in self.groups:
                C.check(self.lib.spgg_set_draw_stream(gr["ctx"], ctypes.c_void_p(self._draw_stream.cuda_stream)),
                        gr["ctx"], "spgg_set_draw_stream")
        self.ctx = self.groups[0]["ctx"]
        self.tile = self.layout[0]
        self.mt_layout = self.layout[4]
        on, cap = ctypes.c_int32(), ctypes.c_int32()
        C.check(self.lib.spgg_persistent(self.ctx, ctypes.byref(on), ctypes.byref(cap)), self.ctx, "spgg_persistent")
        self.persistent, self.persist_capacity = bool(on.value), int(cap.value)
        side = ctypes.c_int32()
        C.check(self.lib.spgg_clusters_max_side(self.ctx, ctypes.byref(side)), self.ctx, "spgg_clusters_max_side")
        self.clusters_max_side = int(side.value)

    def _draw_layout(self, ctx):
        slots, snaps, words = ctypes.c_int32(), ctypes.c_int32(), ctypes.c_int64()
        C.check(self.lib.spgg_draw_layout(ctx, ctypes.byref(slots), ctypes.byref(words), ctypes.byref(snaps)),
                ctx, "spgg_draw_layout")
        return int(slots.value), int(words.value), int(snaps.value)

    def _mt_chains(self, ctx):
        ch, per = ctypes.c_int32(), ctypes.c_int32()
        C.check(self.lib.spgg_mt_chains(ctx, ctypes.byref(ch), ctypes.byref(per)), ctx, "spgg_mt_chains")
        return int(ch.value), int(per.value)

    def check_status(self):
        for g in self.groups:
            f = ctypes.c_uint32()
            C.check(self.lib.spgg_status(g["ctx"], ctypes.byref(f)), g["ctx"], "spgg_status")
            if f.value:
                raise C.SpggError(f"replica group {self.groups.index(g)}: the MT19937 draw generator failed "
                                  f"(error word {f.value}); the run's draws are not the reference's")

    def draw_record(self, t):
        x = self.draws[(t - 1) % self.draw_slots].cpu().numpy().view(np.uint32)
        x = x.reshape(self.R, -1, self.n_planes).transpose(0, 2, 1)
        bits = np.unpackbits(np.ascontiguousarray(x).view(np.uint8), axis=-1, bitorder="little")
        return np.ascontiguousarray(bits[..., :self.n].transpose(1, 0, 2))

    def _layout(self, ctx):
        tw, th = ctypes.c_int32(), ctypes.c_int32()
        C.check(self.lib.spgg_tile_shape(ctx, ctypes.byref(tw), ctypes.byref(th)), ctx, "spgg_tile_shape")
        per = ctypes.c_int64()
        C.check(self.lib.spgg_pub_doubles(ctx, ctypes.byref(per)), ctx, "spgg_pub_doubles")
        ns = ctypes.c_int32()
        C.check(self.lib.spgg_stat_stripes(ctx, ctypes.byref(ns)), ctx, "spgg_stat_stripes")
        return (tw.value, th.value), int(per.value), int(ns.value)

    def _enqueue(self, fn, rounds=(None,)):
        cur = torch.cuda.current_stream(self.dev)
        call = (lambda g, s, r: fn(g, s)) if rounds == (None,) else fn
        if self.G == 1:
            for r in rounds:
                call(self.groups[0], cur.cuda_stream, r)
            return
        for st in self.streams:
            st.wait_stream(cur)
        for r in rounds:
            for g in self.groups:
                call(g, g["stream"].cuda_stream, r)
        for st in self.streams:
            cur.wait_stream(st)

    def close(self):
        for g in getattr(self, "groups", []):
            if g.get("ctx"):
                self.lib.spgg_destroy(g["ctx"])
                g["ctx"] = None
        self.groups = []
        self.ctx = None
        if getattr(self, "_own_streams", None):
            torch.cuda.synchronize(self.dev)
            self.streams = []
            _give_streams(self._own_streams)
            self._own_streams = []
            self._loop = None

    def __del__(self):
        try:
            self.close()
        except Exception:
            pass

    @property
    def stream(self):
        return torch.cuda.current_stream(self.dev).cuda_stream

    def _inject(self, t):
        ncoop = self.stats[:, :, t, C.ST_NCOOP].sum(dim=1).cpu().numpy()
        stop = self.stop_iter.cpu().numpy()
        planes = np.zeros((self.n_planes, self.R, self.n), dtype=np.uint8)
        L = self.L
        for k, s in enumerate(self.init):
            if stop[k] != 0 or ncoop[k] == 0 or ncoop[k] == self.n:
                continue
            e = self.eps_host[k, t]
            selects = 3 if self.alg == C.ALG_SARSA else 1
            for j in range(selects):
                planes[2 * j, k] = s.rs.rand(L, L).reshape(-1) < e
                planes[2 * j + 1, k] = s.rs.randint(0, 2, size=(L, L)).reshape(-1)
            if self.double_q:
                planes[2, k] = s.rs.rand(L, L).reshape(-1) < 0.5
        nwords = self.draw_words // self.n_planes
        pad = np.zeros((self.n_planes, self.R, nwords * 32), dtype=np.uint8)
        pad[:, :, :self.n] = planes
        words = np.packbits(pad, axis=-1, bitorder="little").view(np.uint32)
        rec = np.ascontiguousarray(words.transpose(1, 2, 0)).reshape(self.R, -1)
        self.draws[(t - 1) % self.draw_slots].copy_(torch.from_numpy(rec.view(np.int32)))

    def launch_streams(self):
        if self.G == 1:
            return [torch.cuda.current_stream(self.dev)]
        return list(self.streams)

    def step(self, n_steps: int, ordered: bool = True):
# ... 312 lines not shown
```

Before: 83.83 billion.

## Chain several iterations into one launch with per-tile dependency counters

Adds a chained launch mode: one grid holds blocks for several consecutive iterations. Each block waits on atomic arrival counters from the tiles it depends on before proceeding, which replaces per-iteration kernel launch boundaries with fine-grained cross-block synchronization. Stores and Q loads use coherent (SC1/agent-scope) paths only when a replica spans several XCDs. The aim is to cut launch overhead and tail idle time between iterations when the persistent mode is off. In exchange it adds spin-waits with a timeout, a new error bit, and a host sync in flush, and it risks deadlock if later-iteration blocks occupy the GPU before earlier ones.

```diff
diff --git a/include/spgg_abi.h b/include/spgg_abi.h
--- a/include/spgg_abi.h
+++ b/include/spgg_abi.h
@@ -7,7 +7,7 @@
 extern "C" {
 #endif
 
-#define SPGG_ABI_VERSION 17
+#define SPGG_ABI_VERSION 18
 
 #define SPGG_OK 0
 #define SPGG_E_ARG (-1)
@@ -159,6 +159,8 @@
 
 int spgg_persistent(const spgg_ctx* ctx, int32_t* on, int32_t* capacity);
 
+int spgg_chain(const spgg_ctx* ctx, int32_t* iterations);
+
 int spgg_tile_shape(const spgg_ctx* ctx, int32_t* tw, int32_t* th);
 
 int spgg_destroy(spgg_ctx* ctx);
diff --git a/neighbor-aware-reinforcement-learning-fosters-cooperation-in-spatial-public-goods-games-_amd/_lib.py b/neighbor-aware-reinforcement-learning-fosters-cooperation-in-spatial-public-goods-games-_amd/_lib.py
--- a/neighbor-aware-reinforcement-learning-fosters-cooperation-in-spatial-public-goods-games-_amd/_lib.py
+++ b/neighbor-aware-reinforcement-learning-fosters-cooperation-in-spatial-public-goods-games-_amd/_lib.py
@@ -7,9 +7,10 @@
 PKG_DIR = os.path.dirname(os.path.abspath(__file__))
 LIB_PATH = os.path.join(PKG_DIR, "libspgg_hip.so")
 
-ABI_VERSION = 17
+ABI_VERSION = 18
 OK, E_ARG, E_STATE, E_HIP = 0, -1, -2, -3
 GEN_ERR_SPIN = 1
+STEP_ERR_BARRIER = 2
 CLUSTERS_MAX_PASSES = 32
 STATE_REPUTATION, STATE_ACTION = 0, 1
 RNG_INJECT, RNG_MT19937, RNG_PHILOX = 0, 1, 2
@@ -31,8 +32,8 @@
             "spgg_destroy", "spgg_draw_planes", "spgg_pub_doubles", "spgg_stat_stripes",
             "spgg_history_finalize", "spgg_draw_layout", "spgg_set_draw_stream", "spgg_draw_range",
             "spgg_mt_chains", "spgg_mt_jump_poly", "spgg_stream_create", "spgg_stream_destroy",
-            "spgg_status", "spgg_persistent", "spgg_clusters", "spgg_clusters_max_side")
-TEST_EXPORTED = ("spgg_test_set_error",)
+            "spgg_status", "spgg_persistent", "spgg_clusters", "spgg_clusters_max_side", "spgg_chain")
+TEST_EXPORTED = ("spgg_test_set_error", "spgg_test_chain_map")
 
 
 class Config(ctypes.Structure):
@@ -112,6 +113,10 @@
         lib.spgg_clusters_max_side.argtypes = [vp, ctypes.POINTER(i32)]
         lib.spgg_persistent.restype = ctypes.c_int
         lib.spgg_persistent.argtypes = [vp, ctypes.POINTER(i32), ctypes.POINTER(i32)]
+        lib.spgg_chain.restype = ctypes.c_int
+        lib.spgg_chain.argtypes = [vp, ctypes.POINTER(i32)]
+        lib.spgg_test_chain_map.restype = ctypes.c_int
+        lib.spgg_test_chain_map.argtypes = [i32, i32, i32, i32] + [ctypes.POINTER(i32)] * 4
         lib.spgg_destroy.restype = ctypes.c_int
         lib.spgg_destroy.argtypes = [vp]
         lib.spgg_draw_planes.restype = ctypes.c_int
diff --git a/neighbor-aware-reinforcement-learning-fosters-cooperation-in-spatial-public-goods-games-_amd/csrc/spgg_kernels.hip b/neighbor-aware-reinforcement-learning-fosters-cooperation-in-spatial-public-goods-games-_amd/csrc/spgg_kernels.hip
--- a/neighbor-aware-reinforcement-learning-fosters-cooperation-in-spatial-public-goods-games-_amd/csrc/spgg_kernels.hip
+++ b/neighbor-aware-reinforcement-learning-fosters-cooperation-in-spatial-public-goods-games-_amd/csrc/spgg_kernels.hip
@@ -84,6 +84,7 @@
   uint32_t base;
   uint32_t* err;
   uint32_t* err_host;
+  int chain_blocks;
 };
 constexpr int kBarWords = 16;
 
@@ -92,6 +93,8 @@
                 const PersistArgs* pa = nullptr);
 template <int ALG>
 int persist_blocks_per_cu(const LaunchCfg& lc);
+template <int ALG>
+bool chain_available(const LaunchCfg& lc);
 
 constexpr int apt_of(int alg) { return (alg == SPGG_ALG_DOUBLE_Q ? 512 : 1024) / kBlock; }
 constexpr int js_of(bool m2) { return kBlock == 256 ? (m2 ? 8 : 7) : 4; }
@@ -135,6 +138,37 @@
     const int cc = k3 - (k3 / (2 * HA)) * (2 * HA);
     *ax = cc < HA ? cc : tw + cc;
   }
+}
+
+struct TileWork {
+  int rep, tile;
+  int lrep;
+};
+__host__ __device__ inline TileWork tile_work(int block, int n_rep, int tiles_per_rep, int rep_stride) {
+  const int total = n_rep * tiles_per_rep;
+  const int per_xcd = (total + 7) / 8;
+  const int logical = (block & 7) * per_xcd + (block >> 3);
+  if (logical >= total) return TileWork{-1, -1, -1};
+  const int lrep = logical / tiles_per_rep;
+  const int tile = logical - lrep * tiles_per_rep;
+  const int rep = rep_stride > 1 ? (int)(((uint32_t)lrep * (uint32_t)rep_stride) % (uint32_t)n_rep) : lrep;
+  return TileWork{rep, tile, lrep};
+}
+__host__ __device__ inline bool rep_spans_xcds(int lrep, int n_rep, int tiles_per_rep) {
+  const int per_xcd = (n_rep * tiles_per_rep + 7) / 8;
+  const int first = lrep * tiles_per_rep;
+  return first / per_xcd != (first + tiles_per_rep - 1) / per_xcd;
+}
+__host__ __device__ inline int chain_blocks_of(int total_tiles) { return (total_tiles + 7) / 8 * 8; }
+__host__ __device__ inline int chain_block(int b, int chain_blocks);
+__host__ __device__ inline TileWork chain_work(int block, int chain_blocks, int n_rep, int tiles_per_rep,
+                                               int rep_stride, int* iter) {
+  *iter = block / chain_blocks;
+  return tile_work(chain_block(block - *iter * chain_blocks, chain_blocks), n_rep, tiles_per_rep, rep_stride);
+}
+__host__ __device__ inline int chain_block(int b, int chain_blocks) {
+  if (b & 1) b = chain_blocks - 8 + (b & 7) - (b & ~7);
+  return b;
 }
 
 }
@@ -200,6 +234,15 @@
   if constexpr (SC1 && !SPGG_PERSIST_PLAIN) __hip_atomic_store(p, v, __ATOMIC_RELAXED, __HIP_MEMORY_SCOPE_AGENT);
   else *p = v;
 }
+template <bool SC1, typename T>
+__device__ __forceinline__ void hstore(bool wide, T* p, T v) {
+  if constexpr (SC1) {
+    if (wide) hstore<true>(p, v);
+    else *p = v;
+  } else {
+    *p = v;
+  }
+}
 
 template <bool RQ>
 using RStore = typename std::conditional<RQ, int8_t, double>::type;
@@ -515,9 +558,24 @@
 
 typedef double vd2 __attribute__((ext_vector_type(2)));
 
-template <int QB>
+typedef uint32_t vu4 __attribute__((ext_vector_type(4)));
+template <int QB, bool SC1 = false>
 __device__ __forceinline__ void load_q(const double* Qr, uint32_t n, uint32_t agent, double (&q)[4],
                                        double (&qb)[QB ? 4 : 1]) {
+  if constexpr (SC1) {
+    constexpr int kSc1 = 16;
+    const __amdgpu_buffer_rsrc_t rs = __builtin_amdgcn_make_buffer_rsrc(const_cast<double*>(Qr), 0, -1, 0x00027000);
+    const uint32_t o0 = agent * (QB ? 32u : 16u), o1 = (n + agent) * (QB ? 32u : 16u);
+    const vd2 q01 = __builtin_bit_cast(vd2, __builtin_amdgcn_raw_buffer_load_b128(rs, (int)o0, 0, kSc1));
+    const vd2 q23 = __builtin_bit_cast(vd2, __builtin_amdgcn_raw_buffer_load_b128(rs, (int)o1, 0, kSc1));
+    q[0] = q01.x; q[1] = q01.y; q[2] = q23.x; q[3] = q23.y;
+    if constexpr (QB) {
+      const vd2 b01 = __builtin_bit_cast(vd2, __builtin_amdgcn_raw_buffer_load_b128(rs, (int)(o0 + 16u), 0, kSc1));
+      const vd2 b23 = __builtin_bit_cast(vd2, __builtin_amdgcn_raw_buffer_load_b128(rs, (int)(o1 + 16u), 0, kSc1));
+      qb[0] = b01.x; qb[1] = b01.y; qb[2] = b23.x; qb[3] = b23.y;
+    }
+    return;
+  }
   const vd2* q0 = at(reinterpret_cast<const vd2*>(Qr), agent * (QB ? 2 : 1));
   const vd2* q1 = at(reinterpret_cast<const vd2*>(Qr), (n + agent) * (QB ? 2 : 1));
 #if SPGG_QNT & 1
@@ -782,10 +840,12 @@
 #endif
 }
 
-template <bool M2, bool AS, bool RQ, int RNG, int APT, int TWC, int ALG, bool PERSIST>
+constexpr int MODE_LAUNCH = 0, MODE_PERSIST = 1, MODE_CHAIN = 2;
+template <bool M2, bool AS, bool RQ, int RNG, int APT, int TWC, int ALG, int MODE>
 __device__ __forceinline__ void step_impl(const TileArgs& a0, const int t0, const int fin_only,
                                           const spgg_impl::PersistArgs& pa) {
-  static_assert(!PERSIST || TWC > 0, "persistent launches use the compile-time-width kernels");
+  constexpr bool HANDOFF = MODE != MODE_LAUNCH, PERSIST = MODE == MODE_PERSIST, CHAIN = MODE == MODE_CHAIN;
+  static_assert(!HANDOFF || TWC > 0, "multi-iteration launches use the compile-time-width kernels");
   using RT = RStore<RQ>;
   constexpr int HA = M2 ? 2 : 1;
   constexpr int HS = HA + 2;
@@ -794,16 +854,23 @@
   constexpr int PF = spgg_impl::pf_of(ALG);
   constexpr bool RECOMP = ALG != ALG_SARSA && APT == spgg_impl::apt_of(ALG) && !(PERSIST && SPGG_PERSIST_NORECOMP);
   constexpr bool CARRY = PERSIST && !SPGG_PERSIST_NORECOMP;
+  static_assert(!CHAIN || RECOMP, "chained launches: the instances that recompute the pending NI record");
   extern __shared__ __attribute__((aligned(16))) unsigned char smem[];
 
+  int chain_k = 0, bidx = (int)blockIdx.x;
+  if constexpr (CHAIN) {
+    chain_k = bidx / pa.chain_blocks;
+    bidx = spgg_impl::chain_block(bidx - chain_k * pa.chain_blocks, pa.chain_blocks);
+  }
   const int total = a0.n_rep * a0.tiles_per_rep;
   const int per_xcd = (total + 7) / 8;
-  const int logical = (blockIdx.x & 7) * per_xcd + (blockIdx.x >> 3);
+  const int logical = (bidx & 7) * per_xcd + (bidx >> 3);
   if (logical >= total) return;
   if (SPGG_ABLATE & 64) return;
   const int lrep = logical / a0.tiles_per_rep;
   const int tile = logical - lrep * a0.tiles_per_rep;
   const int rep = a0.rep_stride > 1 ? (int)(((uint32_t)lrep * (uint32_t)a0.rep_stride) % (uint32_t)a0.n_rep) : lrep;
+  const bool wide = CHAIN ? spgg_impl::rep_spans_xcds(lrep, a0.n_rep, a0.tiles_per_rep) : true;
 #if SPGG_STAMPS
   const int stamp_id = (int)a0.params[rep].stream_id * a0.tiles_per_rep + tile;
 #endif
@@ -844,10 +911,10 @@
   const uint32_t g00 = (uint32_t)(y0 * L + x0);
   auto agent_of = [&](int rcu) { return g00 + __umul24((uint32_t)(rcu >> 16), (uint32_t)L) + ((rcu >> 8) & 0xff); };
   bool stored = false;
-  int t = t0;
+  int t = t0 + chain_k;
   for (;; ++t) {
   TileArgs a = a0;
-  if constexpr (PERSIST) {
+  if constexpr (HANDOFF) {
     const int cur = (t - 1) & 1, nxt = t & 1;
     a.S_in = pa.S[cur];
     a.S_out = pa.S[nxt];
@@ -899,7 +966,7 @@
         md_own[u] = 0.0;
         atd_own[u] = 0.f;
       } else {
-        load_q<QB>(Qr, (uint32_t)n, g, q[u], qb[u]);
+        load_q<QB, CHAIN>(Qr, (uint32_t)n, g, q[u], qb[u]);
       }
       r += dr;
       c += dc;
@@ -930,10 +997,10 @@
   DwordWindow<JRD, DWR> winRd;
   RowWindow<JRR, TWC + 2 * HA, RT> winR;
   if constexpr (TWC > 0) {
-    winS.template load<PERSIST>(Sin, th + 2 * HS, y0 - HS, (x0 - HS) & ~3, L, tid);
+    winS.template load<HANDOFF>(Sin, th + 2 * HS, y0 - HS, (x0 - HS) & ~3, L, tid);
     if constexpr (!AS) {
-      if constexpr (RQ) winRd.template load<PERSIST>(Rin, ah, y0 - HA, (x0 - HA) & ~3, L, tid);
-      else winR.template load<PERSIST>(Rin, ah, y0 - HA, x0 - HA, L, tid);
+      if constexpr (RQ) winRd.template load<HANDOFF>(Rin, ah, y0 - HA, (x0 - HA) & ~3, L, tid);
+      else winR.template load<HANDOFF>(Rin, ah, y0 - HA, x0 - HA, L, tid);
     }
   }
 
@@ -958,7 +1025,9 @@
     dw0 = *at(a.draws, wi);
     dw1 = *at(a.draws, wi + 1);
   }
-  const int st = first ? a.stop_iter[rep] : 0;
+  const int st = CHAIN   ? __builtin_amdgcn_readfirstlane(hload<true>(a.stop_iter + rep))
+                 : first ? a.stop_iter[rep]
+                         : 0;
   const bool dead = st != 0 && st < t;
   const spgg_rep_params& pg = a.params[rep];
   __shared__ spgg_rep_params hps;
@@ -976,7 +1045,7 @@
   double* srow = a.stats + ((size_t)rep * a.stripes + tile % a.stripes) * stripe_len;
   bool stop_now = false;
   double gmax_prev = 0.0;
-  if constexpr (PERSIST) {
+  if constexpr (HANDOFF) {
     const int lane = tid & 63, k = lane < a.stripes ? lane : 0;
     const double ncv = hload<true>(rrow + k * stripe_len + (size_t)t * SPGG_NSTAT + SPGG_ST_NCOOP);
     const double gmv = pending ? hload<true>(rrow + k * stripe_len + (size_t)(t - 1) * SPGG_NSTAT + SPGG_ST_GMAX) : 0.0;
@@ -1021,14 +1090,14 @@
     }
   }
   if (dead) return;
-  if (stop_now && tile == 0 && tid == 0) a.stop_iter[rep] = t;
+  if (stop_now && tile == 0 && tid == 0) hstore<CHAIN>(a.stop_iter + rep, t);
   double rv[RP][PF];
   {
     const double* pin = a.pub_in + (size_t)rep * a.tiles_per_rep * PF * a.PB;
 #pragma unroll
     for (int j = 0; j < RP; ++j)
 #pragma unroll
-      for (int f = 0; f < PF; ++f) rv[j][f] = hload<PERSIST>(at(pin, (uint32_t)(re[j].y + f * a.PB)));
+      for (int f = 0; f < PF; ++f) rv[j][f] = hload<HANDOFF>(at(pin, (uint32_t)(re[j].y + f * a.PB)));
   }
   __syncthreads();
   STAMP(1);
@@ -1189,7 +1258,7 @@
       const int s_t = (rc[u] >> 3) & 1;
       const double P = payoff_pc(sPC, r + HA, c + HA, tab + (s_t ? 6 : 0), hp.norm_min, hp.norm_den,
                                  hp.norm_rcp);
-      const RVal<RQ> r_t = AS ? hload<PERSIST>(at(Rin, agent_of(rc[u]))) : sRv[ca];
+      const RVal<RQ> r_t = AS ? hload<HANDOFF>(at(Rin, agent_of(rc[u]))) : sRv[ca];
       if constexpr (RQ) rsum += one ? r_t : 0;
       else rsum = __builtin_fma(r_t, vmu, rsum);
       if (!acting) continue;
@@ -1345,18 +1414,18 @@
       bmax = max_f64(bmax, mdp);
       if constexpr (CARRY) md_own[u] = mdp;
       else if (ni_on && !RECOMP && !(SPGG_ABLATE & (2048 | 8192))) *at(mdr, agent_of(rc[u])) = mdp;
-      hstore<PERSIST>(at(Sout, agent_of(rc[u])), (uint8_t)((rc[u] & 0xff) | (dp << 2) | (sn << 4)));
-      hstore<PERSIST>(at(Rout, agent_of(rc[u])), (RT)sRn[ca]);
+      hstore<HANDOFF>(wide, at(Sout, agent_of(rc[u])), (uint8_t)((rc[u] & 0xff) | (dp << 2) | (sn << 4)));
+      hstore<HANDOFF>(wide, at(Rout, agent_of(rc[u])), (RT)sRn[ca]);
       const int bslot = (int)(int16_t)(uint16_t)(bsw >> (16 * u));
       if (bslot >= 0) {
         double* rec = pout + bslot;
-        hstore<PERSIST>(rec, rn0);
-        hstore<PERSIST>(rec + a.PB, rn1);
+        hstore<HANDOFF>(wide, rec, rn0);
+        hstore<HANDOFF>(wide, rec + a.PB, rn1);
         if constexpr (QB) {
-          hstore<PERSIST>(rec + 2 * a.PB, sn ? qb[u][QB ? 2 : 0] : qb[u][0]);
-          hstore<PERSIST>(rec + 3 * a.PB, sn ? qb[u][QB ? 3 : 0] : qb[u][QB ? 1 : 0]);
+          hstore<HANDOFF>(wide, rec + 2 * a.PB, sn ? qb[u][QB ? 2 : 0] : qb[u][0]);
+          hstore<HANDOFF>(wide, rec + 3 * a.PB, sn ? qb[u][QB ? 3 : 0] : qb[u][QB ? 1 : 0]);
         }
-        if (ni_on) hstore<PERSIST>(rec + (PF - 1) * a.PB, mdp);
+        if (ni_on) hstore<HANDOFF>(wide, rec + (PF - 1) * a.PB, mdp);
       }
       const int nd = act + an[0] + an[1] + an[2] + an[3];
       gcn += one << (4 * nd);
@@ -1491,12 +1560,79 @@
 template <bool M2, bool AS, bool RQ, int RNG, int APT, int TWC, int ALG>
 __global__ __launch_bounds__(kBlock, min_waves(M2, RNG, TWC, ALG)) void spgg_step_kernel(TileArgs a, int t,
                                                                                          int fin_only) {
-  step_impl<M2, AS, RQ, RNG, APT, TWC, ALG, false>(a, t, fin_only, spgg_impl::PersistArgs{});
+  step_impl<M2, AS, RQ, RNG, APT, TWC, ALG, MODE_LAUNCH>(a, t, fin_only, spgg_impl::PersistArgs{});
 }
 
 template <bool M2, bool AS, bool RQ, int RNG, int APT, int TWC, int ALG>
 __global__ __launch_bounds__(kBlock, 4) void spgg_persist_kernel(TileArgs a, int t0, spgg_impl::PersistArgs pa) {
-  step_impl<M2, AS, RQ, RNG, APT, TWC, ALG, true>(a, t0, 0, pa);
+  step_impl<M2, AS, RQ, RNG, APT, TWC, ALG, MODE_PERSIST>(a, t0, 0, pa);
+}
+
+#ifndef SPGG_CHAIN_STATS
+#define SPGG_CHAIN_STATS 0
+#endif
+#if SPGG_CHAIN_STATS
+__device__ unsigned long long spgg_chain_stats[4];
+#endif
+constexpr unsigned long long kChainWaitTicks = 5000000ull;
+
+__device__ __forceinline__ bool chain_wait(const spgg_impl::PersistArgs& pa, const uint32_t* ctr, uint32_t want) {
+  __shared__ int chain_ok;
+  if (threadIdx.x < 64) {
+    bool ok = false, timed_out = false;
+    uint32_t polls = 0;
+    const unsigned long long start = __builtin_amdgcn_s_memrealtime();
+    for (;;) {
+      const uint32_t have = __hip_atomic_load(const_cast<uint32_t*>(ctr), __ATOMIC_RELAXED, __HIP_MEMORY_SCOPE_AGENT);
+      const uint32_t err = __hip_atomic_load(pa.err, __ATOMIC_RELAXED, __HIP_MEMORY_SCOPE_AGENT);
+      if (__builtin_amdgcn_readfirstlane(err) != 0) break;
+      if ((int32_t)(__builtin_amdgcn_readfirstlane(have) - want) >= 0) {
+        ok = true;
+        break;
+      }
+      if (__builtin_amdgcn_s_memrealtime() - start > kChainWaitTicks) {
+        timed_out = true;
+        break;
+      }
+      ++polls;
+      __builtin_amdgcn_s_sleep(8);
+    }
+    if (threadIdx.x == 0) {
+      if (timed_out) {
+        atomicOr(pa.err, (uint32_t)SPGG_STEP_ERR_BARRIER);
+        __hip_atomic_fetch_or(pa.err_host, (uint32_t)SPGG_STEP_ERR_BARRIER, __ATOMIC_RELAXED, __HIP_MEMORY_SCOPE_SYSTEM);
+      }
+#if SPGG_CHAIN_STATS
+      atomicAdd(&spgg_chain_stats[0], 1ull);
+      if (polls) {
+        atomicAdd(&spgg_chain_stats[1], 1ull);
+        atomicAdd(&spgg_chain_stats[2], (unsigned long long)polls);
+      }
+#endif
+      chain_ok = ok ? 1 : 0;
+    }
+  }
+  __syncthreads();
+  return chain_ok != 0;
+}
+
+__device__ __forceinline__ void chain_arrive(uint32_t* ctr) {
+  asm volatile("s_waitcnt vmcnt(0)" ::: "memory");
+  __syncthreads();
+  if (threadIdx.x == 0) __hip_atomic_fetch_add(ctr, 1u, __ATOMIC_RELAXED, __HIP_MEMORY_SCOPE_AGENT);
+}
+
+template <bool M2, bool AS, bool RQ, int RNG, int APT, int TWC, int ALG>
+__global__ __launch_bounds__(kBlock, min_waves(M2, RNG, TWC, ALG)) void spgg_chain_kernel(TileArgs a, int t0,
+                                                                                          spgg_impl::PersistArgs pa) {
+  int k;
+  const spgg_impl::TileWork w =
+      spgg_impl::chain_work((int)blockIdx.x, pa.chain_blocks, a.n_rep, a.tiles_per_rep, a.rep_stride, &k);
+  if (w.tile < 0) return;
+  uint32_t* ctr = pa.bar + (size_t)w.rep * pa.shards * spgg_impl::kBarWords;
+  const bool ok = k == 0 || chain_wait(pa, ctr, (uint32_t)a.tiles_per_rep * (pa.base + (uint32_t)k));
+  if (ok) step_impl<M2, AS, RQ, RNG, APT, TWC, ALG, MODE_CHAIN>(a, t0, 0, pa);
+  chain_arrive(ctr);
 }
 
 template <bool M2, bool AS, bool RQ, int ALG>
@@ -1599,6 +1735,27 @@
 }
 
 template <int ALG>
+const void* chain_fn(const LaunchCfg& lc) {
+  if constexpr (ALG == SPGG_ALG_SARSA) {
+    return nullptr;
+  } else {
+    if (lc.rng != SPGG_RNG_PHILOX || lc.apt != apt_of(ALG) || lc.twc != 40) return nullptr;
+#define SPGG_CF(X, Y, Z)                                     \
+  if (lc.m2 == X && lc.as == Y && lc.rq == Z)                \
+    return reinterpret_cast<const void*>(&spgg_chain_kernel<X, Y, Z, SPGG_RNG_PHILOX, apt_of(ALG), 40, ALG>);
+    SPGG_CF(0, 0, 0) SPGG_CF(0, 0, 1) SPGG_CF(0, 1, 0) SPGG_CF(0, 1, 1)
+    SPGG_CF(1, 0, 0) SPGG_CF(1, 0, 1) SPGG_CF(1, 1, 0) SPGG_CF(1, 1, 1)
+#undef SPGG_CF
+    return nullptr;
+  }
+}
+
+template <int ALG>
+bool chain_available(const LaunchCfg& lc) {
+  return chain_fn<ALG>(lc) != nullptr;
+}
+
+template <int ALG>
 int persist_blocks_per_cu(const LaunchCfg& lc) {
   const void* f = persist_fn<ALG>(lc);
   int nb = 0;
@@ -1656,13 +1813,16 @@
 template <int ALG>
 void launch_alg(const LaunchCfg& lc, const TileArgs& a, int t, int fin, hipStream_t s, const PersistArgs* pa) {
   if (pa) {
-    const void* f = persist_fn<ALG>(lc);
+    const bool chained = pa->chain_blocks > 0;
+    const void* f = chained ? chain_fn<ALG>(lc) : persist_fn<ALG>(lc);
     if (!f) return;
     TileArgs ka = a;
     int kt = t;
     PersistArgs kp = *pa;
     void* args[] = {&ka, &kt, &kp};
-    (void)hipLaunchKernel(f, dim3(((lc.total_tiles + 7) / 8) * 8), dim3(kBlock), args, lc.lds_bytes, s);
+    const unsigned blocks = chained ? (unsigned)pa->chain_blocks * (unsigned)(pa->t_end - t + 1)
+                                    : (unsigned)((lc.total_tiles + 7) / 8) * 8;
+    (void)hipLaunchKernel(f, dim3(blocks), dim3(kBlock), args, lc.lds_bytes, s);
     return;
   }
   if (lc.m2) {
@@ -1676,16 +1836,25 @@
 
 #define SPGG_LAUNCH_INST(k, name)                                                                   \
   template void launch_alg<name>(const LaunchCfg&, const TileArgs&, int, int, hipStream_t, const PersistArgs*); \
-  template int persist_blocks_per_cu<name>(const LaunchCfg&);
+  template int persist_blocks_per_cu<name>(const LaunchCfg&);                                       \
+  template bool chain_available<name>(const LaunchCfg&);
 #define SPGG_LAUNCH_EXTERN(k, name)                                                                 \
   extern template void launch_alg<name>(const LaunchCfg&, const TileArgs&, int, int, hipStream_t,   \
                                         const PersistArgs*);                                        \
-  extern template int persist_blocks_per_cu<name>(const LaunchCfg&);
+  extern template int persist_blocks_per_cu<name>(const LaunchCfg&);                                \
+  extern template bool chain_available<name>(const LaunchCfg&);
 #if SPGG_TU_HAS_ALG(0)
 #if SPGG_STAMPS
 }
 extern "C" int spgg_stamps_read(void* dst, size_t bytes) {
   return (int)hipMemcpyFromSymbol(dst, HIP_SYMBOL(spgg_stamps), bytes < sizeof(spgg_stamps) ? bytes : sizeof(spgg_stamps));
+}
+namespace spgg_impl {
+#endif
+#if SPGG_CHAIN_STATS
+}
+extern "C" int spgg_chain_stats_read(unsigned long long* dst) {
+  return (int)hipMemcpyFromSymbol(dst, HIP_SYMBOL(spgg_chain_stats), sizeof(spgg_chain_stats));
 }
 namespace spgg_impl {
 #endif
@@ -2028,8 +2197,18 @@
   LDS_ST(gen_need[ow][lane], 0xffffffffu);
 }
 
-__global__ void spgg_set_err_kernel(uint32_t* err, uint32_t flags) {
-  if (threadIdx.x == 0) atomicOr(err, flags);
+__global__ void spgg_set_err_kernel(uint32_t* err, uint32_t* err_host, uint32_t flags) {
+  if (threadIdx.x == 0) {
+    atomicOr(err, flags);
+    __hip_atomic_fetch_or(err_host, flags, __ATOMIC_RELAXED, __HIP_MEMORY_SCOPE_SYSTEM);
+  }
+}
+
+__global__ void spgg_merge_err_kernel(uint32_t* err, uint32_t* err_host) {
+  if (threadIdx.x == 0) {
+    const uint32_t v = __hip_atomic_load(err, __ATOMIC_RELAXED, __HIP_MEMORY_SCOPE_AGENT);
+    if (v) __hip_atomic_fetch_or(err_host, v, __ATOMIC_RELAXED, __HIP_MEMORY_SCOPE_SYSTEM);
+  }
 }
 
 __global__ void spgg_mt_final_kernel(GenArgs g, int t_last) {
@@ -2124,6 +2303,7 @@
   hipEvent_t caller_ready = nullptr;
   uint32_t* d_err = nullptr;
   volatile uint32_t* h_err = nullptr;
+  uint32_t* h_err_dev = nullptr;
   int gen_upto = 0;
   std::vector<spgg_rep_params> params_host;
   bool params_moved = false;
@@ -2139,6 +2319,7 @@
   int persist_capacity = 0;
   uint32_t* d_bar = nullptr;
   uint32_t bar_base = 0;
+  int chain = 0;
   std::string err;
 };
 
@@ -2368,6 +2549,18 @@
   }
 }
 
+bool chain_instance(const spgg_ctx* c) {
+  const spgg_impl::LaunchCfg lc = launch_cfg(c);
+  switch (c->cfg.algorithm) {
+    case SPGG_ALG_SARSA: return spgg_impl::chain_available<SPGG_ALG_SARSA>(lc);
+    case SPGG_ALG_EXPECTED_SARSA: return spgg_impl::chain_available<SPGG_ALG_EXPECTED_SARSA>(lc);
+    case SPGG_ALG_DOUBLE_Q: return spgg_impl::chain_available<SPGG_ALG_DOUBLE_Q>(lc);
+    default: return spgg_impl::chain_available<SPGG_ALG_QLEARNING>(lc);
+  }
+}
+constexpr int kChainDefault = 0;
+constexpr int kChainMax = 64;
+
 int err_word_init(spgg_ctx* c) {
   int rc = SPGG_OK;
   if (!c->d_err) {
@@ -2380,6 +2573,9 @@
     if (!rc) {
       c->h_err = static_cast<volatile uint32_t*>(h);
       *c->h_err = 0;
+      void* hd = nullptr;
+      c->h_err_dev = hipHostGetDevicePointer(&hd, h, 0) == hipSuccess ? static_cast<uint32_t*>(hd)
+                                                                      : static_cast<uint32_t*>(h);
     }
   }
   return rc;
@@ -2395,10 +2591,6 @@
 }
 
 void launch_persist(spgg_ctx* c, int t, int t1, hipStream_t s) {
-  if (t == 1) {
-    (void)hipMemsetAsync(c->d_bar, 0, (size_t)c->cfg.n_rep * c->stripes * spgg_impl::kBarWords * 4, s);
-    c->bar_base = 0;
-  }
   spgg_impl::PersistArgs pa{};
   for (int i = 0; i < 2; ++i) {
     pa.S[i] = c->buf.S[i];
@@ -2413,11 +2605,10 @@
   pa.shards = c->stripes;
   pa.base = c->bar_base;
   pa.err = c->d_err;
-  void* hd = nullptr;
-  pa.err_host = hipHostGetDevicePointer(&hd, (void*)c->h_err, 0) == hipSuccess ? static_cast<uint32_t*>(hd)
-                                                                                 : const_cast<uint32_t*>(c->h_err);
+  pa.err_host = c->h_err_dev;
+  pa.chain_blocks = c->persist ? 0 : spgg_impl::chain_blocks_of(c->cfg.n_rep * c->tiles_per_rep);
   launch_step(c, t, 0, s, &pa);
-  c->bar_base += (uint32_t)(t1 - t);
+  c->bar_base += (uint32_t)(c->persist ? t1 - t : t1 - t + 1);
 }
 
 GenArgs gen_args(const spgg_ctx* c, int q = -1) {
@@ -2522,7 +2713,7 @@
   }
   launch_gen(c, t0, t1, 1, c->gen_stream, c->chains > 1 ? q : -1);
   (void)hipEventRecord(c->gen_done[q & 1], c->gen_stream);
-  (void)hipMemcpyAsync((void*)c->h_err, c->d_err, 4, hipMemcpyDeviceToHost, c->gen_stream);
+  hipLaunchKernelGGL(spgg_merge_err_kernel, dim3(1), dim3(64), 0, c->gen_stream, c->d_err, c->h_err_dev);
   if (c->chains > 1 && t1 < c->cfg.iterations)
     spgg_mt::launch_jump(c->d_parts[q & 1], c->d_parts[(q + 1) & 1], c->d_polys + (size_t)J * 624, R, c->chains, -1,
                          c->buf.stop_iter, c->gen_stream);
@@ -2648,6 +2839,10 @@
       c->persist = reps * c->tiles_per_rep <= (long long)c->persist_capacity;
     }
   }
+  if (!rc && !c->persist && chain_instance(c) && (cfg->batch_reps > 0 ? cfg->batch_reps : cfg->n_rep) > 1) {
+    c->chain = kChainDefault;
+    if (const char* e = tuning_env("SPGG_CHAIN")) c->chain = std::max(0, std::min(atoi(e), kChainMax));
+  }
   if (rc) {
     g_create_err = c->err;
     spgg_destroy(c);
@@ -2746,7 +2941,7 @@
 static int step_setup(spgg_ctx* c) {
   int rc = SPGG_OK;
   if (c->cfg.rng_mode == SPGG_RNG_MT19937) rc = mt_lazy_init(c);
-  if (!rc && c->persist) rc = persist_lazy_init(c);
+  if (!rc && (c->persist || c->chain > 1)) rc = persist_lazy_init(c);
   return rc;
 }
 
@@ -2756,6 +2951,10 @@
   int rc = step_setup(c);
   if (rc) return rc;
   if (mt && t0 == 1) c->gen_upto = 0;
+  if (t0 == 1 && c->d_bar) {
+    (void)hipMemsetAsync(c->d_bar, 0, (size_t)c->cfg.n_rep * c->stripes * spgg_impl::kBarWords * 4, s);
+    c->bar_base = 0;
+  }
   if (t0 == 1 && n_steps > 0) launch_step(c, 0, 0, s);
   if (mt && n_steps > 0 && c->gen_upto == 0) {
     (void)hipEventRecord(c->caller_ready, s);
@@ -2765,6 +2964,7 @@
 }
 
 static int seg_end(const spgg_ctx* c, int t, int end) {
+  if (c->chain > 1) return std::min(end - 1, t + c->chain - 1);
   if (!c->persist) return t;
   int t1 = end - 1;
   if (c->cfg.rng_mode == SPGG_RNG_MT19937) t1 = std::min(t1, ((t - 1) / c->gen_chunk + 1) * c->gen_chunk);
@@ -2823,12 +3023,13 @@
   bool same = true;
   for (int i = 1; i < n_ctx; ++i)
     same &= ctxs[i]->persist == ctxs[0]->persist && ctxs[i]->gen_chunk == ctxs[0]->gen_chunk &&
-            ctxs[i]->cfg.rng_mode == ctxs[0]->cfg.rng_mode;
+            ctxs[i]->chain == ctxs[0]->chain && ctxs[i]->cfg.rng_mode == ctxs[0]->cfg.rng_mode;
   const int end = t0 + n_steps;
   for (int t = t0; t < end;) {
     int t1 = same ? seg_end(ctxs[0], t, end) : t;
     for (int i = 0; i < n_ctx; ++i)
-      step_seg(ctxs[i], t, ctxs[i]->persist ? t1 : t, t0, reinterpret_cast<hipStream_t>(streams[i]));
+      step_seg(ctxs[i], t, ctxs[i]->persist || ctxs[i]->chain > 1 ? t1 : t, t0,
+               reinterpret_cast<hipStream_t>(streams[i]));
     t = t1 + 1;
   }
   const int rc = hip_check(ctxs[0], hipGetLastError(), "spgg_step_groups launch");
@@ -2845,7 +3046,7 @@
                                  "from 0 has no pending NI record)");
   hipStream_t s = reinterpret_cast<hipStream_t>(stream);
   if (c->cfg.rng_mode == SPGG_RNG_MT19937 && c->gen_done[0]) {
-    (void)hipMemcpyAsync((void*)c->h_err, c->d_err, 4, hipMemcpyDeviceToHost, c->gen_stream);
+    hipLaunchKernelGGL(spgg_merge_err_kernel, dim3(1), dim3(64), 0, c->gen_stream, c->d_err, c->h_err_dev);
     (void)hipEventRecord(c->gen_idle, c->gen_stream);
     (void)hipStreamWaitEvent(s, c->gen_idle, 0);
     c->gen_upto = 0;
@@ -2856,6 +3057,14 @@
                                        std::to_string(*c->h_err) + "): a wait between its waves ran out of "
                                        "its bound, so this run's draws are not the reference's");
     hipLaunchKernelGGL(spgg_mt_final_kernel, dim3(c->cfg.n_rep), dim3(256), 0, s, gen_args(c), t_last);
+  }
+  if (c->h_err) {
+    int rc = hip_check(c, hipStreamSynchronize(s), "spgg_flush: step stream");
+    if (rc) return rc;
+    if (*c->h_err & SPGG_STEP_ERR_BARRIER)
+      return fail(c, SPGG_E_STATE, "spgg_flush: a step launch's barrier wait ran out of its bound (error word " +
+                                       std::to_string(*c->h_err) + "): a tile of a multi-iteration launch never "
+                                       "arrived, so this run's state is not the reference's");
   }
   launch_step(c, t_last + 1, 1, s);
   return hip_check(c, hipGetLastError(), "spgg_flush launch");
@@ -2924,12 +3133,29 @@
 
 int spgg_test_set_error(spgg_ctx* c, uint32_t flags) {
   if (!c) return SPGG_E_ARG;
-  if (c->cfg.rng_mode != SPGG_RNG_MT19937) return fail(c, SPGG_E_STATE, "spgg_test_set_error: MT19937 only");
+  const bool mt = c->cfg.rng_mode == SPGG_RNG_MT19937;
+  if (!mt && !c->persist && c->chain <= 1)
+    return fail(c, SPGG_E_STATE, "spgg_test_set_error: a context with an error word (MT19937, persistent or "
+                                 "chained launches)");
   int rc = hip_check(c, hipSetDevice(c->cfg.device), "hipSetDevice");
-  if (!rc) rc = mt_lazy_init(c);
+  if (!rc) rc = mt ? mt_lazy_init(c) : err_word_init(c);
   if (rc) return rc;
-  hipLaunchKernelGGL(spgg_set_err_kernel, dim3(1), dim3(64), 0, c->gen_stream, c->d_err, flags);
+  hipLaunchKernelGGL(spgg_set_err_kernel, dim3(1), dim3(64), 0, mt ? c->gen_stream : nullptr, c->d_err, c->h_err_dev,
+                     flags);
   return hip_check(c, hipGetLastError(), "spgg_test_set_error launch");
+}
+
+int spgg_test_chain_map(int32_t block, int32_t n_rep, int32_t tiles_per_rep, int32_t rep_stride, int32_t* chain_blocks,
+                        int32_t* iter, int32_t* rep, int32_t* tile) {
+  if (block < 0 || n_rep < 1 || tiles_per_rep < 1 || rep_stride < 1 || !chain_blocks || !iter || !rep || !tile)
+    return SPGG_E_ARG;
+  *chain_blocks = spgg_impl::chain_blocks_of(n_rep * tiles_per_rep);
+  int k = 0;
+  const spgg_impl::TileWork w = spgg_impl::chain_work(block, *chain_blocks, n_rep, tiles_per_rep, rep_stride, &k);
+  *iter = k;
+  *rep = w.rep;
+  *tile = w.tile;
+  return SPGG_OK;
 }
 
 int spgg_pub_doubles(const spgg_ctx* c, int64_t* per_rep) {
@@ -2948,6 +3174,12 @@
   if (!c || !on || !capacity) return SPGG_E_ARG;
   *on = c->persist ? 1 : 0;
   *capacity = c->persist_capacity;
+  return SPGG_OK;
+}
+
+int spgg_chain(const spgg_ctx* c, int32_t* iterations) {
+  if (!c || !iterations) return SPGG_E_ARG;
+  *iterations = c->chain > 1 ? c->chain : 0;
   return SPGG_OK;
 }
 
diff --git a/neighbor-aware-reinforcement-learning-fosters-cooperation-in-spatial-public-goods-games-_amd/engine.py b/neighbor-aware-reinforcement-learning-fosters-cooperation-in-spatial-public-goods-games-_amd/engine.py
--- a/neighbor-aware-reinforcement-learning-fosters-cooperation-in-spatial-public-goods-games-_amd/engine.py
+++ b/neighbor-aware-reinforcement-learning-fosters-cooperation-in-spatial-public-goods-games-_amd/engine.py
@@ -399,6 +399,9 @@
         on, cap = ctypes.c_int32(), ctypes.c_int32()
         C.check(self.lib.spgg_persistent(self.ctx, ctypes.byref(on), ctypes.byref(cap)), self.ctx, "spgg_persistent")
         self.persistent, self.persist_capacity = bool(on.value), int(cap.value)
+        ch = ctypes.c_int32()
+        C.check(self.lib.spgg_chain(self.ctx, ctypes.byref(ch)), self.ctx, "spgg_chain")
+        self.chain = int(ch.value)
         side = ctypes.c_int32()
         C.check(self.lib.spgg_clusters_max_side(self.ctx, ctypes.byref(side)), self.ctx, "spgg_clusters_max_side")
         self.clusters_max_side = int(side.value)
@@ -418,9 +421,18 @@
         for g in self.groups:
             f = ctypes.c_uint32()
             C.check(self.lib.spgg_status(g["ctx"], ctypes.byref(f)), g["ctx"], "spgg_status")
-            if f.value:
-                raise C.SpggError(f"replica group {self.groups.index(g)}: the MT19937 draw generator failed "
-                                  f"(error word {f.value}); the run's draws are not the reference's")
+            if not f.value:
+                continue
+            parts = []
+            if f.value & C.GEN_ERR_SPIN:
+                parts.append("the MT19937 draw generator failed: the run's draws are not the reference's")
+            if f.value & C.STEP_ERR_BARRIER:
+                parts.append("a step launch's barrier wait ran out of its bound: a tile of a multi-iteration "
+                             "launch never arrived and the run's state is wrong")
+            if f.value & ~(C.GEN_ERR_SPIN | C.STEP_ERR_BARRIER):
+                parts.append("unknown error bits")
+            raise C.SpggError(f"replica group {self.groups.index(g)}: " + "; ".join(parts) +
+                              f" (error word {f.value})")
 
     def draw_record(self, t):
         x = self.draws[(t - 1) % self.draw_slots].cpu().numpy().view(np.uint32)
```

Measured after the change: 83.88 billion, median of 3. About the same (+0.1%).
